# bytedance/particle-sfm

Hardware: AMD Instinct MI355X
Metric: trajectory-points/s (higher is better)
Workload: dtype f32 sampling + f64 positions; 1 GPU; configs[1]: synthetic 100x(1920x1080) flow pairs, sample_ratio=2, flow_check + chaining + occlusion + id assignment, 1 sequence per GPU; frames=101, height=1080, width=1920, trajectories=2073277, parallelism=sequence-per-gpu x1, world_size=1

## Files before the change

include/psfm.h:

```cpp
#ifndef PSFM_H_
#define PSFM_H_

#include <stddef.h>
#include <stdint.h>

#ifdef __cplusplus
extern "C" {
#endif

#define PSFM_VERSION 141

typedef enum psfm_status {
    PSFM_OK = 0,
    PSFM_ERR_ARG = 1,
    PSFM_ERR_HIP = 2,
    PSFM_ERR_CAPACITY = 3,
    PSFM_ERR_SOLVER = 4
} psfm_status;

typedef struct psfm_ctx psfm_ctx;

enum {
    PSFM_TERM_FUNCTION_TOL = 0,
    PSFM_TERM_PARAMETER_TOL = 1,
    PSFM_TERM_GRADIENT_TOL = 2,
    PSFM_TERM_MAX_ITER = 3,
    PSFM_TERM_MIN_RADIUS = 4,
    PSFM_TERM_FAILURE = 5
};

typedef struct psfm_solve_stats {
    int32_t iterations;
    int32_t successful_steps;
    int32_t termination;
    int32_t dogleg_nonGN;
    double initial_cost;
    double final_cost;
} psfm_solve_stats;

typedef struct psfm_track_info {
    int64_t n_traj;
    int64_t n_points;
    int64_t n_lanes_peak;
    int64_t lane_capacity;
    int64_t solver_iterations;
    int32_t n_solves;
    int32_t chain_mode;
} psfm_track_info;

const char* psfm_last_error(void);
int psfm_version(void);

int psfm_device_count(void);

psfm_status psfm_ctx_create(int device, psfm_ctx** out);
psfm_status psfm_ctx_destroy(psfm_ctx* ctx);

psfm_status psfm_ctx_set_capacity(psfm_ctx* ctx, double lane_factor, double traj_factor);

psfm_status psfm_ctx_set_chain_mode(psfm_ctx* ctx, int mode);

psfm_status psfm_ctx_set_motion_boundary(psfm_ctx* ctx, int enable, float thres);

psfm_status psfm_motion_boundary(psfm_ctx* ctx, const float* flows, int n, int h, int w, float thres, uint8_t* mb_out, void* stream);

psfm_status psfm_kill_map(psfm_ctx* ctx, const float* flows, const uint8_t* occ, int n, int h, int w, float thres, uint8_t* kill_out,
                          void* stream);

psfm_status psfm_ctx_set_solver(psfm_ctx* ctx, int mode, int k);
psfm_status psfm_solver_counters(psfm_ctx* ctx, int64_t* fused, int64_t* fused_redone, int64_t* chain, int32_t* k_now);

psfm_status psfm_ctx_set_resident_budget(psfm_ctx* ctx, int blocks);
psfm_status psfm_resident_capacity(psfm_ctx* ctx, int32_t* blocks);

psfm_status psfm_solver_launches(psfm_ctx* ctx, int64_t* resident, int64_t* giveups, int64_t* iterations);

psfm_status psfm_flow_check(psfm_ctx* ctx, const float* flows_f, const float* flows_b, int n_pairs, int h,
                            int w, float thres, uint8_t* occ_out, float* err_out, void* stream);

psfm_status psfm_load_flo_stack(psfm_ctx* ctx, const char* const* paths_host, int n, int h, int w, float* dst, int n_threads, void* stream);

psfm_status psfm_grid_sample(psfm_ctx* ctx, const float* map_hwc, int c, int h, int w, const double* xy,
                             int64_t n, float* out, void* stream);

psfm_status psfm_optimize_location(psfm_ctx* ctx, const double* uv12, const double* ref1, const double* ref2,
                                   const double* scale, const float* flow12, int64_t n, int w, int h,
                                   double* out, psfm_solve_stats* stats_host, void* stream);

psfm_status psfm_path_consistency_eval(psfm_ctx* ctx, const double* uv12, const double* ref1, const double* ref2,
                                       const double* scale, const float* flow12, int64_t n, int w, int h,
                                       double* residuals, double* jacobians, void* stream);

psfm_status psfm_sort_records(psfm_ctx* ctx, uint32_t* keys, int32_t* values, int64_t n, int end_bit, void* stream);

psfm_status psfm_sort_records64(psfm_ctx* ctx, uint64_t* keys, int32_t* values, int64_t n, int end_bit, void* stream);

psfm_status psfm_ctx_get_finalize_forms(psfm_ctx* ctx, int* sort_form, int* offsets_form);

psfm_status psfm_track(psfm_ctx* ctx, const float* flows, const uint8_t* occ, const float* flows_f2,
                       const uint8_t* occ_s2, int n_flows, int h, int w, int sample_ratio,
                       psfm_track_info* info_host, void* stream);

psfm_status psfm_connect(psfm_ctx* ctx, const float* flows_f, const float* flows_b, const float* flows_f2,
                         const float* flows_b2, int n_flows, int h, int w, float thres, int sample_ratio,
                         uint8_t* occ, uint8_t* occ_s2, psfm_track_info* info_host, void* stream);

psfm_status psfm_track_queries(psfm_ctx* ctx, const float* flows_f, const uint8_t* occ_f, const float* flows_b, const uint8_t* occ_b,
                               int n_flows, int h, int w, const double* q_xy, const int32_t* q_t, int64_t n_q,
                               psfm_track_info* info_host, void* stream);

psfm_status psfm_track_queries_optimize(psfm_ctx* ctx, const float* flows_f, const uint8_t* occ_f, const float* flows_f2,
                                        const uint8_t* occ_f2, const float* flows_b, const uint8_t* occ_b, const float* flows_b2,
                                        const uint8_t* occ_b2, int n_flows, int h, int w, const double* q_xy, const int32_t* q_t,
                                        int64_t n_q, psfm_track_info* info_host, void* stream);

psfm_status psfm_connect_batch(psfm_ctx* const* ctxs, int n_seq, const float* const* flows_f, const float* const* flows_b,
                               const float* const* flows_f2, const float* const* flows_b2, const int* n_flows, int h, int w,
                               float thres, int sample_ratio, psfm_track_info* infos_host, void* stream);

psfm_status psfm_result_device(psfm_ctx* ctx, const int32_t** birth, const int32_t** len,
                               const int64_t** off, const double** xy);

psfm_status psfm_result_copy(psfm_ctx* ctx, int32_t* birth_host, int32_t* len_host, int64_t* off_host,
                             double* xy_host, void* stream);

psfm_status psfm_result_solve_stats(psfm_ctx* ctx, psfm_solve_stats* stats_host, int32_t max_n,
                                    int32_t* n_out);

psfm_status psfm_result_filter(psfm_ctx* ctx, int traj_min_len, int64_t* n_traj_host, int64_t* n_points_host, void* stream);
psfm_status psfm_result_filtered_copy(psfm_ctx* ctx, int32_t* ids_host, int32_t* birth_host, int32_t* len_host,
                                      int64_t* off_host, double* xy_host, void* stream);

psfm_status psfm_window_sample(psfm_ctx* ctx, int frame0, int n_frames, int traj_min_len, int min_length,
                               int64_t max_num_tracks, uint64_t seed, int raw_h, int raw_w, int in_h, int in_w,
                               int64_t capacity, int32_t* ids_out, double* xy_raw, double* xy_norm, double* mask_absent,
                               int64_t* k_host, void* stream);

psfm_status psfm_traj_augment(psfm_ctx* ctx, const double* xy_norm, const double* mask_absent, const float* depth, int64_t k,
                              int n_frames, int h, int w, const float* kinv_host, float* out, void* stream);

int psfm_traj_encode_weight_count(void);
psfm_status psfm_traj_encode(psfm_ctx* ctx, const float* features, const double* mask_absent, const float* weights, int64_t k,
                             int n_frames, float* out, void* stream);

int psfm_traj_decode_weight_count(void);
size_t psfm_traj_decode_workspace_bytes(int64_t k);
psfm_status psfm_traj_decode(psfm_ctx* ctx, const float* encoding, const float* weights, int64_t k, void* workspace,
                             size_t workspace_bytes, float* logits, float* prob, uint8_t* pred, void* stream);

psfm_status psfm_traj_to_matches(psfm_ctx* ctx, int n_img, int sample_k, const uint8_t* labels_dev, int64_t* n_kp_host,
                                 int64_t* n_matches_host, int64_t* n_pairs_host, void* stream);
psfm_status psfm_matches_copy(psfm_ctx* ctx, int64_t* kp_off_host, double* kp_xy_host, int64_t* pair_key_host,
                              int64_t* pair_off_host, int64_t* pair_first_host, int32_t* rows_host, void* stream);

psfm_status psfm_labels_set(psfm_ctx* ctx, int64_t n_traj, int64_t n_points, const int32_t* ids, const int64_t* off,
                            const int32_t* frame_ids, const double* xy, const uint8_t* labels, void* stream);
psfm_status psfm_labels_begin(psfm_ctx* ctx, void* stream);
psfm_status psfm_labels_merge_window(psfm_ctx* ctx, int frame0, int n_frames, const int32_t* ids_dev, const uint8_t* pred_dev,
                                     int64_t k, void* stream);
psfm_status psfm_labels_finish(psfm_ctx* ctx, int64_t* n_traj_host, int64_t* n_points_host, void* stream);
psfm_status psfm_labels_device(psfm_ctx* ctx, const int32_t** ids, const int64_t** off, const int32_t** frame_ids, const double** xy,
                               const uint8_t** labels);
psfm_status psfm_labels_copy(psfm_ctx* ctx, int32_t* ids_out, int64_t* off_out, int32_t* frame_ids_out, double* xy_out,
                             uint8_t* labels_out, void* stream);
psfm_status psfm_labels_to_matches(psfm_ctx* ctx, int n_img, int sample_k, int remove_dynamic, int64_t* n_kp_host,
                                   int64_t* n_matches_host, int64_t* n_pairs_host, void* stream);

psfm_status psfm_matches_to_database(psfm_ctx* ctx, int n_img, const int32_t* db_id_host, const int32_t* db_pos_host,
                                     int64_t* n_pairs_kept_host, int64_t* n_rows_kept_host, void* stream);
psfm_status psfm_database_copy(psfm_ctx* ctx, float* kp_f32, int64_t* pair_id, int64_t* pair_key, int64_t* pair_off, uint32_t* rows,
                               void* stream);
int psfm_database_chunk_rows(void);
psfm_status psfm_database_compact_again(psfm_ctx* ctx, void* stream);

psfm_status psfm_sparse_depth(psfm_ctx* ctx, const double* obs_xy, const int64_t* obs_id, int64_t n_obs, const void* img_desc_host,
                              int n_img, const int64_t* pt_id_sorted, const int32_t* pt_row, const double* pt_xyz, int64_t n_pts,
                              double* depth_out, int64_t* missing_id_host, void* stream);
psfm_status psfm_sparse_depth_sort_ids(psfm_ctx* ctx, const int64_t* pt_id, int64_t n_pts, int64_t* pt_id_sorted, int32_t* pt_row,
                                       void* stream);
psfm_status psfm_ctx_set_sparse_depth(psfm_ctx* ctx, int64_t budget_bytes, int timing);
psfm_status psfm_ctx_get_sparse_depth_budget(psfm_ctx* ctx, int64_t* budget_bytes);
psfm_status psfm_sparse_depth_last_ms(psfm_ctx* ctx, double* ms3);
psfm_status psfm_colmap_points3d_count(const void* buf, uint64_t nbytes, uint64_t* n);
psfm_status psfm_colmap_points3d_scan(const void* buf, uint64_t nbytes, uint64_t* ids_out, double* xyz_out, double* err_out,
                                      uint64_t* track_len_out);

psfm_status psfm_depth_display(psfm_ctx* ctx, const double* depth, const void* img_desc_host, int n_img, double pc,
                               const uint8_t* table_host, const uint8_t* bad_rgba_host, uint8_t* rgba_out, int64_t* n_valid_out,
                               double* z_out, void* stream);
psfm_status psfm_ctx_set_depth_display(psfm_ctx* ctx, int timing);
psfm_status psfm_depth_display_last_ms(psfm_ctx* ctx, double* ms4);
int psfm_depth_display_chunk(void);

psfm_status psfm_traj_eval_counts(psfm_ctx* ctx, const int32_t* frame_ids, const double* xy, const uint8_t* labels, int64_t n_points,
                                  const uint8_t* masks_u8, const float* table_host, int n_frames, int h, int w, int64_t* counts_out,
                                  void* stream);
psfm_status psfm_traj_vote_labels(psfm_ctx* ctx, const double* xy, const double* mask_absent, const uint8_t* gts_u8, int64_t k,
                                  int n_frames, int h, int w, uint8_t* labels_out, void* stream);

psfm_status psfm_shard_begin(psfm_ctx* ctx, int n_flows, int h, int w, int sample_ratio, int64_t g0, int64_t g1, int optimize,
                             uint8_t* maps, int64_t map_pitch, void* stream);
psfm_status psfm_shard_step(psfm_ctx* ctx, const float* flow, const uint8_t* occ, int frame, void* stream);
psfm_status psfm_shard_solve_export(psfm_ctx* ctx, const float* flow01, const float* flow12, const float* flow02,
                                    const uint8_t* occ02, int frame, int kind, int k, double* sums_out, void* stream);
psfm_status psfm_shard_frame(psfm_ctx* ctx, const float* flow01, const float* flow12, const float* flow02, const uint8_t* occ,
                             const uint8_t* occ02, int frame, int k, double* sums_out, void* stream);
psfm_status psfm_shard_solve_control(psfm_ctx* ctx, int frame, int kind, int k, const double* totals, int32_t* done_host,
                                     int32_t* redo_host, psfm_solve_stats* stats_host, void* stream);
psfm_status psfm_shard_solve_control_async(psfm_ctx* ctx, int frame, int k, const double* totals, void* stream);
psfm_status psfm_shard_window_state(psfm_ctx* ctx, int f_lo, int f_hi, psfm_solve_stats* stats_host, int32_t* stalled_frame,
                                    void* stream);
psfm_status psfm_shard_solve_control_chain_async(psfm_ctx* ctx, int frame, int kind, const double* totals, void* stream);
psfm_status psfm_shard_solve_poll(psfm_ctx* ctx, int32_t* done_host, psfm_solve_stats* stats_host, void* stream);
psfm_status psfm_shard_solve_local(psfm_ctx* ctx, const float* flow01, const float* flow12, const float* flow02, const uint8_t* occ02,
                                   int frame, int unroll, void* stream);
psfm_status psfm_shard_solve_redo_local(psfm_ctx* ctx, const float* flow01, const float* flow12, const float* flow02,
                                        const uint8_t* occ02, int frame, int chain_stalled, psfm_solve_stats* stats_host, void* stream);
psfm_status psfm_shard_peer_area(psfm_ctx* ctx, void** area_dev, void* ipc_handle_64, void* stream);
psfm_status psfm_shard_peer_open(psfm_ctx* ctx, const void* ipc_handle_64, int peer_rank, void** mapped);
psfm_status psfm_shard_peer_epoch(psfm_ctx* ctx, uint32_t* last_epoch, int reset, void* stream);
psfm_status psfm_shard_peer_connect(psfm_ctx* ctx, int world, int rank, void* const* areas, const int32_t* n_blocks);
psfm_status psfm_shard_solve_blocks(psfm_ctx* ctx, int32_t* n_blocks);
psfm_status psfm_shard_solve_peer(psfm_ctx* ctx, const float* flow01, const float* flow12, const float* flow02, const uint8_t* occ02,
                                  int frame, uint32_t epoch, void* stream);

psfm_status psfm_shard_peek_stall(psfm_ctx* ctx, int32_t* stalled_frame);
psfm_status psfm_shard_solve_restore(psfm_ctx* ctx, int frame, void* stream);
psfm_status psfm_shard_solve_writeback(psfm_ctx* ctx, int frame, const psfm_solve_stats* stats, void* stream);
psfm_status psfm_shard_solve_record(psfm_ctx* ctx, const psfm_solve_stats* stats);
psfm_status psfm_shard_finish(psfm_ctx* ctx, psfm_track_info* info_host, void* stream);
psfm_status psfm_result_keys(psfm_ctx* ctx, int sample_ratio, int w, int64_t* keys_dev, void* stream);

psfm_status psfm_ctx_set_profiling(psfm_ctx* ctx, int enable);
psfm_status psfm_profile_get(psfm_ctx* ctx, int kind, double* total_ms, int64_t* launches);

#ifdef __cplusplus
}
#endif
#endif
```

particle-sfm_amd/build.py:

```python
import os
import subprocess
import sys
from concurrent.futures import ThreadPoolExecutor

HERE = os.path.dirname(os.path.abspath(__file__))
CSRC = os.path.join(HERE, "csrc")
OBJ = os.path.join(HERE, "build")
LIBDIR = os.path.join(HERE, "lib")
LIB = os.path.join(LIBDIR, "libpsfm_hip.so")
SOURCES = ["psfm_api.hip", "psfm_track.hip", "psfm_persist.hip", "psfm_finalize.hip", "psfm_sort.hip", "psfm_sort64.hip", "psfm_solver.hip", "psfm_solver_fused.hip", "psfm_solver_batch.hip", "psfm_window.hip", "psfm_matches.hip", "psfm_shard.hip", "psfm_batch.hip", "psfm_ingest.hip", "psfm_labels.hip", "psfm_augment.hip", "psfm_encoder.hip", "psfm_decoder.hip", "psfm_ground_truth.hip", "psfm_database.hip", "psfm_sparse_depth.hip", "psfm_motion_boundary.hip", "psfm_depth_display.hip", "psfm_query.hip", "psfm_query_pc.hip"]
HIPCC = os.environ.get("HIPCC", "/opt/rocm/bin/hipcc")
FLAGS = ["--offload-arch=gfx950", "-O3", "-std=c++17", "-fPIC", "-ffp-contract=off", "-fno-fast-math",
         "-Wall", "-Wno-unused-function", "-Wno-unused-result",
         "-mllvm", "-amdgpu-atomic-optimizer-strategy=None"]


def source_hash():
    import hashlib
    h = hashlib.sha256()
    files = sorted(os.path.join(CSRC, f) for f in os.listdir(CSRC) if f.endswith((".hip", ".h")))
    files.append(os.path.join(os.path.dirname(HERE), "include", "psfm.h"))
    for f in files:
        h.update(os.path.basename(f).encode())
        h.update(open(f, "rb").read())
    h.update(" ".join(FLAGS).encode())
    return h.hexdigest()[:16]


def _newer(target, deps):
    if not os.path.exists(target):
        return True
    t = os.path.getmtime(target)
    return any(os.path.getmtime(d) > t for d in deps)


def build(force=False, verbose=False):
    extra = os.environ.get("PSFM_EXTRA_FLAGS", "").split()
    if extra:
        FLAGS.extend(extra)
        force = True
    os.makedirs(OBJ, exist_ok=True)
    os.makedirs(LIBDIR, exist_ok=True)
    headers = [os.path.join(CSRC, f) for f in os.listdir(CSRC) if f.endswith(".h")]
    headers.append(os.path.join(os.path.dirname(HERE), "include", "psfm.h"))
    jobs, objs = [], []
    for src in SOURCES:
        s = os.path.join(CSRC, src)
        o = os.path.join(OBJ, src.replace(".hip", ".o"))
        objs.append(o)
        if force or _newer(o, [s] + headers):
            jobs.append([HIPCC] + FLAGS + ["-c", s, "-o", o])

    def run(cmd):
        if verbose:
            print(" ".join(cmd), flush=True)
        r = subprocess.run(cmd, stdout=subprocess.PIPE, stderr=subprocess.STDOUT, text=True)
        if r.returncode != 0:
            raise RuntimeError("hipcc failed:\n%s\n%s" % (" ".join(cmd), r.stdout))
        if verbose and r.stdout.strip():
            print(r.stdout)

    with ThreadPoolExecutor(max_workers=4) as ex:
        list(ex.map(run, jobs))
    if force or jobs or _newer(LIB, objs):
        run([HIPCC, "--offload-arch=gfx950", "-shared", "-fPIC", "-o", LIB] + objs)
    return LIB


if __name__ == "__main__":
    if "--source-hash" in sys.argv:
        print(source_hash())
    else:
        print(build(force="--force" in sys.argv, verbose=True))
```

particle-sfm_amd/csrc/psfm_api.hip:

```cpp
#include <stdarg.h>
#include <stdio.h>
#include <string.h>
#include <mutex>
#include <shared_mutex>
#include <atomic>
#include <chrono>
#include <stdlib.h>

#include "psfm_internal.h"

static thread_local char g_err[512] = "";
static std::shared_mutex g_dev_gate[16];
std::shared_mutex& psfm_device_gate(int device) { return g_dev_gate[device & 15]; }
static std::atomic<int> g_dev_waiters[16];
int psfm_gate_waiters(int device) { return g_dev_waiters[device & 15].load(std::memory_order_relaxed); }
void psfm_gate_waiters_add(int device, int d) { g_dev_waiters[device & 15].fetch_add(d, std::memory_order_relaxed); }
static int psfm_wants_persist(psfm_ctx* c, bool optimize, int h, int w, int ratio, bool fused)
{
    if (c->chain_mode == 1 || ratio < 1 || !psfm_frame_ok(h, w)) return 0;
    if (c->mb_enable && !optimize) return 0;
    if (optimize) return c->resident_budget > 0 ? 0 : 1;
    const int64_t G = (int64_t)((w + ratio - 1) / ratio) * ((h + ratio - 1) / ratio);
    const int64_t P = (int64_t)h * w;
    const int maxb = psfm_persist_max_blocks(c);
    if (maxb <= 0 || (G + 255) / 256 > maxb) return 0;
    if (c->chain_mode == 2) return 2;
    if (ratio < 2 || G < 100000) return 0;
    if (fused && (G < 400000 || P > 6 * G)) return 0;
    return 1;
}

void psfm_set_error(const char* fmt, ...)
{
    va_list ap;
    va_start(ap, fmt);
    vsnprintf(g_err, sizeof(g_err), fmt, ap);
    va_end(ap);
}

extern "C" const char* psfm_last_error(void) { return g_err; }
extern "C" int psfm_version(void) { return PSFM_VERSION; }

extern "C" int psfm_device_count(void)
{
    int n = 0;
    if (hipGetDeviceCount(&n) != hipSuccess) { (void)hipGetLastError(); return 0; }
    return n;
}

psfm_status PsfmBuf::ensure(size_t need)
{
    if (need <= bytes) return PSFM_OK;
    if (p) { (void)hipFree(p); p = nullptr; bytes = 0; }
    size_t want = (need + (size_t)(1 << 20) - 1) & ~((size_t)(1 << 20) - 1);
    hipError_t e = hipMalloc(&p, want);
    if (e != hipSuccess) {
        p = nullptr;
        psfm_set_error("hipMalloc(%zu bytes) failed: %s", want, hipGetErrorString(e));
        return PSFM_ERR_HIP;
    }
    bytes = want;
    return PSFM_OK;
}

void PsfmBuf::release()
{
    if (p) (void)hipFree(p);
    p = nullptr;
    bytes = 0;
}

hipEvent_t PsfmProfiler::get()
{
    if (!pool.empty()) { hipEvent_t e = pool.back(); pool.pop_back(); return e; }
    hipEvent_t e;
    (void)hipEventCreate(&e);
    return e;
}
void PsfmProfiler::begin(int kind, hipStream_t s)
{
    if (!enabled) return;
    Span sp; sp.kind = kind; sp.a = get(); sp.b = get();
    (void)hipEventRecord(sp.a, s);
    spans.push_back(sp);
}
void PsfmProfiler::kernel_span(int kind, hipEvent_t* a, hipEvent_t* b, bool always)
{
    if (!enabled || (!always && (calls++ % stride) != 0)) { *a = nullptr; *b = nullptr; return; }
    Span sp; sp.kind = kind; sp.a = get(); sp.b = get();
    spans.push_back(sp);
    *a = sp.a; *b = sp.b;
}
void PsfmProfiler::end(hipStream_t s)
{
    if (!enabled) return;
    (void)hipEventRecord(spans.back().b, s);
}
void PsfmProfiler::collect()
{
    for (auto& sp : spans) {
        float ms = 0.f;
        if (hipEventElapsedTime(&ms, sp.a, sp.b) == hipSuccess) { total_ms[sp.kind] += ms; launches[sp.kind]++; }
        pool.push_back(sp.a); pool.push_back(sp.b);
    }
    spans.clear();
}
void PsfmProfiler::reset()
{
    for (int k = 0; k < PSFM_PROF_KINDS; ++k) { total_ms[k] = 0; launches[k] = 0; }
}
void PsfmProfiler::destroy()
{
    collect();
    for (auto e : pool) (void)hipEventDestroy(e);
    pool.clear();
}

#define PSFM_CHECK_CTX(c)                                                     \
    do {                                                                      \
        if (!(c)) { psfm_set_error("ctx is NULL"); return PSFM_ERR_ARG; }     \
        PSFM_HIP(hipSetDevice((c)->device));                                  \
    } while (0)

extern "C" psfm_status psfm_ctx_create(int device, psfm_ctx** out)
{
    if (!out) { psfm_set_error("psfm_ctx_create: out is NULL"); return PSFM_ERR_ARG; }
    *out = nullptr;
    int n = 0;
    hipError_t e = hipGetDeviceCount(&n);
    if (e != hipSuccess || n <= 0) {
        (void)hipGetLastError();
        psfm_set_error("no HIP device available (%s); libpsfm_hip has no CPU fallback",
                       e != hipSuccess ? hipGetErrorString(e) : "device count 0");
        return PSFM_ERR_HIP;
    }
    if (device < 0 || device >= n) { psfm_set_error("device %d out of range [0,%d)", device, n); return PSFM_ERR_ARG; }
    PSFM_HIP(hipSetDevice(device));
    psfm_ctx* c = new psfm_ctx();
    c->device = device;
    c->host_pinned_bytes = 512 + sizeof(PsfmShard) * PSFM_NSHARD + 4096;
    e = hipHostMalloc(&c->host_pinned, c->host_pinned_bytes, hipHostMallocDefault);
    if (e != hipSuccess) { delete c; psfm_set_error("hipHostMalloc failed: %s", hipGetErrorString(e)); return PSFM_ERR_HIP; }
    *out = c;
    return PSFM_OK;
}

extern "C" psfm_status psfm_ctx_destroy(psfm_ctx* c)
{
    if (!c) return PSFM_OK;
    (void)hipSetDevice(c->device);
    PsfmBuf* bufs[] = {&c->log, &c->birth_frame, &c->birth_idx, &c->free_stack, &c->fin_keys, &c->fin_lanes,
                       &c->occupied, &c->counters, &c->shards, &c->survivors, &c->sort_keys, &c->sort_lanes, &c->sort_tmp,
                       &c->scan_tmp, &c->fin_marks, &c->res_birth, &c->res_len, &c->res_off, &c->res_xy, &c->sol_x, &c->sol_state,
                       &c->sol_partials, &c->sol_ctrl, &c->sol_misc, &c->sol_stats, &c->sol_fused, &c->sol_bar, &c->sol_list, &c->occ_own, &c->occ2_own,
                       &c->handoff, &c->seg_info, &c->seg_table, &c->persist_bar, &c->batch_tab, &c->batch_ws, &c->batch_fc, &c->win_ws, &c->flt_ids, &c->flt_birth, &c->flt_len, &c->flt_off, &c->flt_xy,
                       &c->mt_kp_off, &c->mt_q, &c->mt_pts, &c->mt_kp_ind, &c->mt_kp_xy, &c->mt_moff, &c->mt_keys, &c->mt_rows, &c->mt_gid, &c->mt_pairs,
                       &c->lb_state, &c->lb_first, &c->lb_flag, &c->lb_ws, &c->lb_ids, &c->lb_off, &c->lb_frames, &c->lb_xy, &c->lb_labels, &c->gt_flag, &c->kill,
                       &c->db_kp, &c->db_pairs, &c->db_rows, &c->db_ws, &c->sd_ws, &c->dd_ws, &c->dd_comp, &c->qr_ws};
    for (auto b : bufs) b->release();
    for (hipEvent_t e : c->sd_events) if (e) (void)hipEventDestroy(e);
    for (hipEvent_t e : c->dd_events) if (e) (void)hipEventDestroy(e);
    for (void*& q : c->peer_opened) { if (q) (void)hipIpcCloseMemHandle(q); q = nullptr; }
    c->peer_area.release();
    psfm_shard_abandon(c);
    c->prof.destroy();
    if (c->side_stream) (void)hipStreamDestroy(c->side_stream);
    if (c->redo_stream) (void)hipStreamDestroy(c->redo_stream);
    if (c->copy_stream) (void)hipStreamDestroy(c->copy_stream);
    if (c->copy_stream2) (void)hipStreamDestroy(c->copy_stream2);
    for (void* p : c->ingest_slots) (void)hipHostFree(p);
    for (hipEvent_t e : c->ingest_events) (void)hipEventDestroy(e);
    if (c->host_pinned) (void)hipHostFree(c->host_pinned);
    if (c->host_seg) (void)hipHostFree(c->host_seg);
    if (c->host_batch) (void)hipHostFree(c->host_batch);
    if (c->host_batch2) (void)hipHostFree(c->host_batch2);
    delete c;
    return PSFM_OK;
}

extern "C" psfm_status psfm_ctx_set_capacity(psfm_ctx* c, double lane_factor, double traj_factor)
{
    if (!c || !(lane_factor >= 1.0) || !(traj_factor >= 1.0)) { psfm_set_error("psfm_ctx_set_capacity: factors must be >= 1"); return PSFM_ERR_ARG; }
    c->lane_factor = lane_factor;
    c->traj_factor = traj_factor;
    return PSFM_OK;
}

extern "C" psfm_status psfm_ctx_set_chain_mode(psfm_ctx* c, int mode)
{
    if (!c || mode < 0 || mode > 2) { psfm_set_error("psfm_ctx_set_chain_mode: mode must be 0 (auto), 1 (per-frame launches) or 2 (persistent loop)"); return PSFM_ERR_ARG; }
    c->chain_mode = mode;
    return PSFM_OK;
}

extern "C" psfm_status psfm_ctx_set_solver(psfm_ctx* c, int mode, int k)
{
    if (!c || mode < 0 || mode > 2 || k < 0 || k > psfm_solve_kmax()) {
        psfm_set_error("psfm_ctx_set_solver: mode must be 0 (adaptive), 1 (launch chain) or 2 (fused solve), k in [0, %d]", psfm_solve_kmax());
        return PSFM_ERR_ARG;
    }
    c->solver_mode = mode;
    c->solver_K = k;
    return PSFM_OK;
}

extern "C" psfm_status psfm_solver_counters(psfm_ctx* c, int64_t* fused, int64_t* fused_redone, int64_t* chain, int32_t* k_now)
{
    if (!c) { psfm_set_error("ctx is NULL"); return PSFM_ERR_ARG; }
    if (fused) *fused = c->n_fused_ok;
    if (fused_redone) *fused_redone = c->n_fused_redone;
    if (chain) *chain = c->n_chain;
    if (k_now) *k_now = c->solve_K;
    return PSFM_OK;
}

extern "C" psfm_status psfm_ctx_set_resident_budget(psfm_ctx* c, int blocks)
{
    if (!c || blocks < 0) { psfm_set_error("psfm_ctx_set_resident_budget: blocks must be >= 0"); return PSFM_ERR_ARG; }
    c->resident_budget = blocks;
    return PSFM_OK;
}

extern "C" psfm_status psfm_resident_capacity(psfm_ctx* c, int32_t* blocks)
{
    PSFM_CHECK_CTX(c);
    if (blocks) *blocks = psfm_resident_blocks(c);
    return PSFM_OK;
}

extern "C" psfm_status psfm_solver_launches(psfm_ctx* c, int64_t* resident, int64_t* giveups, int64_t* iterations)
{
    if (!c) { psfm_set_error("ctx is NULL"); return PSFM_ERR_ARG; }
    if (resident) *resident = c->n_resident;
    if (giveups) *giveups = c->pc_giveups;
    if (iterations) *iterations = c->n_iter_launches;
    return PSFM_OK;
}

extern "C" psfm_status psfm_ctx_set_profiling(psfm_ctx* c, int enable)
{
    if (!c) { psfm_set_error("ctx is NULL"); return PSFM_ERR_ARG; }
    c->prof.enabled = enable != 0;
    c->prof.stride = enable > 1 ? enable : 1;
    c->prof.calls = 0;
    c->prof.collect();
    c->prof.reset();
    return PSFM_OK;
}

extern "C" psfm_status psfm_profile_get(psfm_ctx* c, int kind, double* total_ms, int64_t* launches)
{
    if (!c || kind < 0 || kind >= PSFM_PROF_KINDS) { psfm_set_error("psfm_profile_get: bad argument"); return PSFM_ERR_ARG; }
    if (total_ms) *total_ms = c->prof.total_ms[kind];
    if (launches) *launches = c->prof.launches[kind];
    return PSFM_OK;
}

extern "C" psfm_status psfm_flow_check(psfm_ctx* c, const float* flows_f, const float* flows_b, int n_pairs, int h, int w,
                                       float thres, uint8_t* occ_out, float* err_out, void* stream)
{
    PSFM_CHECK_CTX(c);
    PsfmGate gate(c->device, 0);
    if (n_pairs < 0 || !psfm_frame_ok(h, w) || (n_pairs > 0 && (!flows_f || !flows_b || !occ_out))) {
        psfm_set_error("psfm_flow_check: bad argument (n_pairs=%d h=%d w=%d)", n_pairs, h, w);
        return PSFM_ERR_ARG;
    }
    hipStream_t s = (hipStream_t)stream;
    c->prof.begin(PSFM_PROF_FLOW_CHECK, s);
    psfm_status st = psfm_launch_flow_check(flows_f, flows_b, n_pairs, h, w, thres, occ_out, err_out, s);
    c->prof.end(s);
    return st;
}

extern "C" psfm_status psfm_grid_sample(psfm_ctx* c, const float* map_hwc, int ch, int h, int w, const double* xy,
                                        int64_t n, float* out, void* stream)
{
    PSFM_CHECK_CTX(c);
    PsfmGate gate(c->device, 0);
    if ((ch != 1 && ch != 2) || !psfm_frame_ok(h, w) || n < 0 || (n > 0 && (!map_hwc || !xy || !out))) {
        psfm_set_error("psfm_grid_sample: bad argument (c=%d h=%d w=%d n=%lld)", ch, h, w, (long long)n);
        return PSFM_ERR_ARG;
    }
    return psfm_launch_grid_sample(map_hwc, ch, h, w, xy, n, out, (hipStream_t)stream);
}

extern "C" psfm_status psfm_optimize_location(psfm_ctx* c, const double* uv12, const double* ref1, const double* ref2,
                                              const double* scale, const float* flow12, int64_t n, int w, int h,
                                              double* out, psfm_solve_stats* stats_host, void* stream)
{
    PSFM_CHECK_CTX(c);
    PsfmGate gate(c->device, (c->chain_mode == 1 || c->resident_budget > 0) ? 0 : 1);
    c->pc_persist_ok = gate.exclusive || c->resident_budget > 0;
    c->pc_giveups = 0;
    c->n_resident = c->n_iter_launches = 0;
    if (n < 0 || !psfm_frame_ok(h, w) || (n > 0 && (!uv12 || !ref1 || !ref2 || !scale || !flow12 || !out))) {
        psfm_set_error("psfm_optimize_location: bad argument (n=%lld h=%d w=%d)", (long long)n, h, w);
        return PSFM_ERR_ARG;
    }
    psfm_solve_stats st;
    memset(&st, 0, sizeof(st));
    hipStream_t s = (hipStream_t)stream;
    c->prof.begin(PSFM_PROF_SOLVER, s);
    psfm_status rc = psfm_solve_batch(c, uv12, ref1, ref2, scale, flow12, n, w, h, out, &st, s);
    c->prof.end(s);
    if (stats_host) *stats_host = st;
    return rc;
}

extern "C" psfm_status psfm_path_consistency_eval(psfm_ctx* c, const double* uv12, const double* ref1, const double* ref2,
                                                  const double* scale, const float* flow12, int64_t n, int w, int h,
                                                  double* residuals, double* jacobians, void* stream)
{
    PSFM_CHECK_CTX(c);
    PsfmGate gate(c->device, 0);
    if (n < 0 || n > 0x3fffffff || !psfm_frame_ok(h, w) || (n > 0 && (!uv12 || !ref1 || !ref2 || !scale || !flow12 || (!residuals && !jacobians)))) {
        psfm_set_error("psfm_path_consistency_eval: bad argument (n=%lld h=%d w=%d)", (long long)n, h, w);
        return PSFM_ERR_ARG;
    }
    return psfm_launch_pc_eval(uv12, ref1, ref2, scale, flow12, n, w, h, residuals, jacobians, (hipStream_t)stream);
}

extern "C" psfm_status psfm_sort_records(psfm_ctx* c, uint32_t* keys, int32_t* values, int64_t n, int end_bit, void* stream)
{
    PSFM_CHECK_CTX(c);
    PsfmGate gate(c->device, 0);
    if (n < 0 || n >= (1ll << 31) || end_bit < 1 || end_bit > 32 || (n > 0 && (!keys || !values))) {
        psfm_set_error("psfm_sort_records: bad argument (n=%lld end_bit=%d)", (long long)n, end_bit);
        return PSFM_ERR_ARG;
    }
    if (n == 0) return PSFM_OK;
    hipStream_t s = (hipStream_t)stream;
    psfm_status st;
    if ((st = c->sort_keys.ensure(sizeof(unsigned long long) * (size_t)n * 2)) != PSFM_OK) return st;
    if ((st = c->sort_lanes.ensure(sizeof(int) * (size_t)n * 2)) != PSFM_OK) return st;
    const int64_t half = psfm_sort_pairs32_passes((unsigned)end_bit) % 2 == 0 ? 0 : n;
    unsigned* k0 = c->sort_keys.as<unsigned>();
    int* v0 = c->sort_lanes.as<int>();
    PSFM_HIP(hipMemcpyAsync(k0 + half, keys, sizeof(unsigned) * (size_t)n, hipMemcpyDeviceToDevice, s));
    PSFM_HIP(hipMemcpyAsync(v0 + half, values, sizeof(int) * (size_t)n, hipMemcpyDeviceToDevice, s));
    if ((st = psfm_sort_pairs32(c, k0, v0, k0 + n, v0 + n, n, (unsigned)end_bit, s)) != PSFM_OK) return st;
    PSFM_HIP(hipMemcpyAsync(keys, k0, sizeof(unsigned) * (size_t)n, hipMemcpyDeviceToDevice, s));
    PSFM_HIP(hipMemcpyAsync(values, v0, sizeof(int) * (size_t)n, hipMemcpyDeviceToDevice, s));
    return PSFM_OK;
}

extern "C" psfm_status psfm_sort_records64(psfm_ctx* c, uint64_t* keys, int32_t* values, int64_t n, int end_bit, void* stream)
{
    PSFM_CHECK_CTX(c);
    PsfmGate gate(c->device, 0);
    if (n < 0 || n >= (1ll << 31) || end_bit < 1 || end_bit > 64 || (n > 0 && (!keys || !values))) {
        psfm_set_error("psfm_sort_records64: bad argument (n=%lld end_bit=%d)", (long long)n, end_bit);
        return PSFM_ERR_ARG;
    }
    if (n == 0) return PSFM_OK;
    hipStream_t s = (hipStream_t)stream;
    psfm_status st;
    if ((st = c->sort_keys.ensure(sizeof(unsigned long long) * (size_t)n * 2)) != PSFM_OK) return st;
    if ((st = c->sort_lanes.ensure(sizeof(int) * (size_t)n * 2)) != PSFM_OK) return st;
    const int64_t half = psfm_sort_pairs64_passes((unsigned)end_bit) % 2 == 0 ? 0 : n;
    unsigned long long* k0 = c->sort_keys.as<unsigned long long>();
    int* v0 = c->sort_lanes.as<int>();
    PSFM_HIP(hipMemcpyAsync(k0 + half, keys, sizeof(unsigned long long) * (size_t)n, hipMemcpyDeviceToDevice, s));
    PSFM_HIP(hipMemcpyAsync(v0 + half, values, sizeof(int) * (size_t)n, hipMemcpyDeviceToDevice, s));
    if ((st = psfm_sort_pairs64(c, k0, v0, k0 + n, v0 + n, n, (unsigned)end_bit, s)) != PSFM_OK) return st;
    PSFM_HIP(hipMemcpyAsync(keys, k0, sizeof(unsigned long long) * (size_t)n, hipMemcpyDeviceToDevice, s));
    PSFM_HIP(hipMemcpyAsync(values, v0, sizeof(int) * (size_t)n, hipMemcpyDeviceToDevice, s));
    return PSFM_OK;
}

extern "C" psfm_status psfm_ctx_get_finalize_forms(psfm_ctx* c, int* sort_form, int* offsets_form)
{
    PSFM_CHECK_CTX(c);
    if (sort_form) *sort_form = c->fin_sort_form;
    if (offsets_form) *offsets_form = c->fin_offsets_form;
    return PSFM_OK;
}

psfm_status psfm_track_dims(psfm_ctx* c, int n_flows, int h, int w, int ratio, int64_t g_own, PsfmTrackDims& d)
{
    d.H = h; d.W = w; d.ratio = ratio; d.n_flows = n_flows;
    d.GW = (w + ratio - 1) / ratio; d.GH = (h + ratio - 1) / ratio;
    d.G = (int64_t)d.GW * d.GH;
    const int64_t Gown = g_own < 0 ? d.G : (g_own > 0 ? g_own : 1);
    d.cap = (int64_t)(c->lane_factor * (double)Gown);
    d.cap = ((d.cap + 255) / 256) * 256;
    const int64_t n_blocks = d.cap / 256;
    {
        const int64_t gb = (Gown + 255) / 256;
        d.nsh = (int)(gb < PSFM_NSHARD ? (gb > 0 ? gb : 1) : PSFM_NSHARD);
    }
    d.free_cap = (int)(((n_blocks + d.nsh - 1) / d.nsh) * 256) + 1024;
    const double tf = c->traj_factor > (double)n_flows / 8.0 ? c->traj_factor : (double)n_flows / 8.0;
    d.shard_cap = (int)(((int64_t)(tf * (double)Gown) + d.cap) / d.nsh) + 1024;
    d.traj_cap = (int64_t)d.shard_cap * PSFM_NSHARD;
    if (d.cap > 0x7fffffff / 2 || d.traj_cap > 0x7fffffff / 2) { psfm_set_error("psfm_track: grid too large"); return PSFM_ERR_ARG; }
    d.shift_b = 1; while ((1ll << d.shift_b) < d.G) ++d.shift_b;
    int tbits = 1; while ((1ll << tbits) < (long long)n_flows + 2) ++tbits;
    d.shift_d = d.shift_b + tbits;
    if (d.shift_d + tbits > 63) { psfm_set_error("psfm_track: key does not fit 64 bits"); return PSFM_ERR_ARG; }
    d.cw = (float)((double)(w - 1) / 2.0); d.ch = (float)((double)(h - 1) / 2.0);
    return PSFM_OK;
}

psfm_status psfm_track_alloc(psfm_ctx* c, const PsfmTrackDims& d)
{
    psfm_status st;
    const int n_flows = d.n_flows;
    if ((st = c->log.ensure(sizeof(double2) * (size_t)(n_flows + 1) * d.cap)) != PSFM_OK) return st;
    if ((st = c->birth_frame.ensure(sizeof(int) * d.cap)) != PSFM_OK) return st;
    if ((st = c->birth_idx.ensure(sizeof(int) * d.cap)) != PSFM_OK) return st;
    if ((st = c->free_stack.ensure(sizeof(int) * (size_t)d.free_cap * PSFM_NSHARD * 2)) != PSFM_OK) return st;
    if ((st = c->shards.ensure(sizeof(PsfmShard) * PSFM_NSHARD * 2)) != PSFM_OK) return st;
    if ((st = c->fin_keys.ensure(sizeof(unsigned long long) * d.traj_cap)) != PSFM_OK) return st;
    if ((st = c->fin_lanes.ensure(sizeof(int) * d.traj_cap)) != PSFM_OK) return st;
    if ((st = c->occupied.ensure((size_t)d.G * 3 + 8)) != PSFM_OK) return st;
    if ((st = c->counters.ensure(sizeof(PsfmCounters))) != PSFM_OK) return st;
    if ((st = c->survivors.ensure(sizeof(int) * (size_t)(n_flows + 1))) != PSFM_OK) return st;
    return PSFM_OK;
}

struct PsfmOccPipeline {
    int chunk = 0;
    std::vector<hipEvent_t> ready;
    std::vector<hipEvent_t> ready_s2;
    int waited = -1, waited_s2 = -1;
    psfm_status need(int pair, bool s2, hipStream_t s)
    {
        if (chunk <= 0) return PSFM_OK;
        std::vector<hipEvent_t>& ev = s2 ? ready_s2 : ready;
        int& w = s2 ? waited_s2 : waited;
        const int cidx = pair / chunk;
        while (w < cidx && w + 1 < (int)ev.size()) {
            ++w;
            PSFM_HIP(hipStreamWaitEvent(s, ev[w], 0));
        }
        return PSFM_OK;
    }
};

static psfm_status psfm_track_impl(psfm_ctx* c, const float* flows, const uint8_t* occ, const float* flows_f2,
                                   const uint8_t* occ_s2, int n_flows, int h, int w, int ratio, psfm_track_info* info,
                                   void* stream, PsfmOccPipeline* pipe, PsfmGate& gate,
                                   const float* fuse_flows_b = nullptr, float fuse_thres = 0.f, int64_t occ_pitch = 0)
{
    const bool device_is_ours = gate.exclusive;
    if (occ_pitch == 0) occ_pitch = (int64_t)h * w;
    PSFM_CHECK_CTX(c);
    psfm_shard_abandon(c);
    const bool optimize = flows_f2 != nullptr;
    if (n_flows < 1 || !psfm_frame_ok(h, w) || ratio < 1 || !flows || !occ || (optimize && !occ_s2 && n_flows > 1)) {
        psfm_set_error("psfm_track: bad argument (n_flows=%d h=%d w=%d ratio=%d)", n_flows, h, w, ratio);
        return PSFM_ERR_ARG;
    }
    if (ratio > 64) { psfm_set_error("psfm_track: sample_ratio %d > 64 unsupported", ratio); return PSFM_ERR_ARG; }
    hipStream_t s = (hipStream_t)stream;
    PsfmTrackDims d;
    psfm_status st;
    if ((st = psfm_track_dims(c, n_flows, h, w, ratio, -1, d)) != PSFM_OK) return st;
    const int64_t P = (int64_t)h * w;
    if ((st = psfm_track_alloc(c, d)) != PSFM_OK) return st;

    c->solve_stats.clear();
    c->res_n_traj = c->res_n_points = 0;
    c->res_n_flows = n_flows;
    c->res_is_query = false;
    c->pc_persist_ok = device_is_ours || c->resident_budget > 0;
    c->pc_giveups = 0;

    const bool mb = c->mb_enable;
    if (!optimize && c->chain_mode != 1 && !mb) {
        const int maxb = psfm_persist_max_blocks(c);
        const int64_t need_blocks = (d.G + 255) / 256;
        if (maxb > 0 && need_blocks <= maxb && device_is_ours) {
            PsfmTrackDims dp = d;
            int64_t nb = need_blocks <= 256 ? 2 * need_blocks + 4 : need_blocks + need_blocks / 4;
            dp.nblk = (int)(nb < maxb ? nb : maxb);
            if (fuse_flows_b) {
                const int64_t fc_blocks = (P + 1023) / 1024;
                const int64_t want = fc_blocks < maxb ? fc_blocks : maxb;
                if (want > dp.nblk) dp.nblk = (int)want;
            }
            dp.cap = (int64_t)dp.nblk * (256 + psfm_persist_guests());
            dp.nsh = dp.nblk < PSFM_NSHARD ? dp.nblk : PSFM_NSHARD;
            dp.free_cap = (int)(((dp.nblk + dp.nsh - 1) / dp.nsh) * 256) + 1024;
            dp.seg_cap = (int)(d.traj_cap / dp.nblk) + 64;
            dp.spill_cap = (int)(d.traj_cap / 8) + 4096;
            const int64_t fin_total = (int64_t)dp.nblk * dp.seg_cap + dp.spill_cap;
            if ((st = c->log.ensure(sizeof(double2) * (size_t)(n_flows + 1) * dp.cap)) != PSFM_OK) return st;
            if ((st = c->free_stack.ensure(sizeof(int) * (size_t)dp.free_cap * PSFM_NSHARD * 2)) != PSFM_OK) return st;
            if ((st = c->fin_keys.ensure(sizeof(unsigned long long) * fin_total)) != PSFM_OK) return st;
            if ((st = c->fin_lanes.ensure(sizeof(int) * fin_total)) != PSFM_OK) return st;
            if ((st = c->handoff.ensure((size_t)dp.nblk * 256 * 24)) != PSFM_OK) return st;
            if ((st = c->seg_info.ensure(sizeof(int) * 2 * (size_t)dp.nblk)) != PSFM_OK) return st;
            if ((st = c->persist_bar.ensure((size_t)(4 * PSFM_NSHARD + 1) * 128)) != PSFM_OK) return st;
            if (pipe && (st = pipe->need(n_flows - 1, false, s)) != PSFM_OK) return st;
            bool fallback = false;
            {
                const bool trace = getenv("PSFM_TRACE") != nullptr;
                const auto t1 = std::chrono::steady_clock::now();
                st = psfm_launch_chain_persist(c, dp, flows, occ, occ_pitch, fuse_flows_b, fuse_thres, s);
                if (st == PSFM_ERR_CAPACITY) {
                    fallback = true;
                    st = PSFM_OK;
                } else {
                    if (st != PSFM_OK) return st;
                    c->prof.begin(PSFM_PROF_FINALIZE, s);
                    st = psfm_finalize_persist(c, dp, &fallback, s);
                    c->prof.end(s);
                }
                if (trace) {
                    const auto t2 = std::chrono::steady_clock::now();
                    fprintf(stderr, "[psfm %p] persistent loop: launch+finalize %.2f ms, fallback %d, overflow %d\n", (void*)c,
                            std::chrono::duration<double, std::milli>(t2 - t1).count(), (int)fallback,
                            ((PsfmCounters*)c->host_pinned)->overflow);
                }
            }
            if (st != PSFM_OK) return st;
            if (!fallback) {
                PSFM_HIP(hipStreamSynchronize(s));
                c->prof.collect();
                if (info) {
                    memset(info, 0, sizeof(*info));
                    info->n_traj = c->res_n_traj;
                    info->n_points = c->res_n_points;
                    info->n_lanes_peak = ((PsfmCounters*)c->host_pinned)->n_lanes;
                    info->lane_capacity = dp.cap;
                    info->chain_mode = 2;
                }
                return PSFM_OK;
            }
            c->prof.collect();
        }
    }
    if (fuse_flows_b) {
        c->prof.begin(PSFM_PROF_FLOW_CHECK, s);
        for (int f = 0; f < n_flows; ++f)
            if ((st = psfm_launch_flow_check(flows + (size_t)f * P * 2, fuse_flows_b + (size_t)f * P * 2, 1, h, w, fuse_thres,
                                             const_cast<uint8_t*>(occ) + (size_t)f * occ_pitch, nullptr, s)) != PSFM_OK) return st;
        c->prof.end(s);
    }
    if (mb) {
        if ((st = c->kill.ensure((size_t)n_flows * (size_t)P)) != PSFM_OK) return st;
        if (pipe && (st = pipe->need(n_flows - 1, false, s)) != PSFM_OK) return st;
        if (occ_pitch != P) { psfm_set_error("psfm_track: motion boundary needs densely packed occlusion maps"); return PSFM_ERR_ARG; }
        if ((st = psfm_launch_motion_boundary(flows, occ, n_flows, h, w, c->mb_thres, c->kill.as<uint8_t>(), s)) != PSFM_OK) return st;
    }
    if ((st = psfm_launch_track_init(c, d, s)) != PSFM_OK) return st;
    int64_t total_iters = 0;
    static const int check_env = getenv("PSFM_CHECK_FRAMES") ? atoi(getenv("PSFM_CHECK_FRAMES")) : 0;
    const int PSFM_CHECK = check_env >= 2 ? check_env : 16;
    std::vector<psfm_solve_stats> hstats((size_t)n_flows + 1);
    int first_unchecked = 1;
    if (optimize) {
        if ((st = c->sol_stats.ensure(sizeof(psfm_solve_stats) * (size_t)(n_flows + 1))) != PSFM_OK) return st;
    }
    const char* unroll_env = getenv("PSFM_SOLVE_UNROLL");
    const int unroll_fixed = unroll_env ? (atoi(unroll_env) < 1 ? 1 : atoi(unroll_env)) : 0;
    c->n_fused_ok = c->n_fused_redone = c->n_chain = 0;
    c->n_resident = c->n_iter_launches = 0;
    if (optimize && (st = psfm_solve_prepare(c, d, s)) != PSFM_OK) return st;
    static const bool merge = !(getenv("PSFM_MERGE_FRAME") && atoi(getenv("PSFM_MERGE_FRAME")) == 0);
    const bool seq_env = !(getenv("PSFM_SEQ") && atoi(getenv("PSFM_SEQ")) == 0);
    bool seq_ok = optimize && merge && seq_env && unroll_fixed == 0 && !mb;
    int launch_id = 0;
    int idle_windows = 0;
    bool pc_in_step = true;
    int* hpc = (int*)((char*)c->host_pinned + 320);
    PsfmCounters* dctr = c->counters.as<PsfmCounters>();

    auto checkpoint = [&](int f_hi, bool fused_now, bool seq, int* f_next) -> psfm_status {
        PsfmCounters* hc = (PsfmCounters*)c->host_pinned;
        PSFM_HIP(hipMemcpyAsync(hc, c->counters.p, sizeof(PsfmCounters), hipMemcpyDeviceToHost, s));
        PSFM_HIP(hipMemcpyAsync(hstats.data() + first_unchecked, c->sol_stats.as<psfm_solve_stats>() + first_unchecked,
                                sizeof(psfm_solve_stats) * (size_t)(f_hi - first_unchecked + 1), hipMemcpyDeviceToHost, s));
        PSFM_HIP(hipStreamSynchronize(s));
        if (gate.yield_exclusive()) c->pc_persist_ok = c->resident_budget > 0;
        if ((hc->overflow & 7) != 0 || hc->n_lanes > d.cap) {
            psfm_set_error("capacity exceeded: lanes used %d of %lld, overflow bits %d (frame %d of %d); raise psfm_ctx_set_capacity",
                           hc->n_lanes, (long long)d.cap, hc->overflow, hc->pc_frame, n_flows);
            return PSFM_ERR_CAPACITY;
        }
        const int stalled = hc->stall ? hc->stall - 1 : -1;
        int last_ok = f_hi;
        if (seq) {
            const int pcf = hc->pc_frame < n_flows ? hc->pc_frame : n_flows;
            last_ok = pcf - 1;
        }
        if (stalled >= 0) {
            const int fs = stalled;
            psfm_solve_stats ss;
            memset(&ss, 0, sizeof(ss));
            const int k_used = c->solver_K > 0 ? c->solver_K : c->solve_K;
            psfm_status st2 = psfm_solve_frame_resume(c, d, flows + (size_t)(fs - 1) * P * 2, flows + (size_t)fs * P * 2,
                                                      flows_f2 + (size_t)(fs - 1) * P * 2, occ_s2 + (size_t)(fs - 1) * P, fs, &ss,
                                                      (fused_now && !seq && c->solver_K == 0 && k_used < psfm_solve_kmax())
                                                          ? (k_used + 2 < psfm_solve_kmax() ? k_used + 2 : psfm_solve_kmax()) : 0,
                                                      !fused_now, s);
            if (st2 != PSFM_OK) return st2;
            hstats[fs] = ss;
            last_ok = fs;
            pc_in_step = false;
        }
        int max_it = 0, n_solved = 0, n_unclean = 0, k_need = 2;
        for (int k = first_unchecked; k <= last_ok; ++k) {
            if (hstats[k].termination >= 0) {
                c->solve_stats.push_back(hstats[k]);
                total_iters += hstats[k].iterations;
                const psfm_solve_stats& q = hstats[k];
                const bool clean = q.dogleg_nonGN == 0 && q.termination != PSFM_TERM_FAILURE &&
                                   (q.iterations == q.successful_steps + 1 ||
                                    (q.termination == PSFM_TERM_GRADIENT_TOL && q.iterations == q.successful_steps)) &&
                                   q.successful_steps + 1 <= psfm_solve_kmax();
                ++n_solved;
                if (!clean) ++n_unclean;
                else if (q.successful_steps + 1 > k_need) k_need = q.successful_steps + 1;
                if (!fused_now) ++c->n_chain;
                else if (k == stalled) ++c->n_fused_redone;
                else ++c->n_fused_ok;
            }
            if (hstats[k].iterations > max_it) max_it = hstats[k].iterations;
        }
        if (n_solved > 0) {
            c->solve_mode = (n_unclean * 8 > n_solved) ? 1 : 0;
            if (seq) {
                int hist[16] = {0};
                for (int k = first_unchecked; k <= last_ok; ++k)
                    if (hstats[k].termination >= 0) ++hist[hstats[k].successful_steps + 1 < 15 ? hstats[k].successful_steps + 1 : 15];
                int best = 2;
                for (int q = 2; q <= psfm_solve_kmax(); ++q) if (hist[q] > hist[best]) best = q;
                c->solve_K = best;
            } else {
                c->solve_K = k_need > c->solve_K ? k_need : c->solve_K - (c->solve_K - k_need + 1) / 2;
            }
        }
        int want = max_it + 1;
        want = want < 4 ? 4 : (want > 64 ? 64 : want);
        c->solve_unroll = want > c->solve_unroll ? want : c->solve_unroll - (c->solve_unroll - want + 1) / 2;
        first_unchecked = last_ok + 1;
        *f_next = last_ok + 1;
        return PSFM_OK;
    };

    int f = 0;
    while (f < n_flows) {
        const bool fused_now = c->solver_mode == 2 || (c->solver_mode == 0 && c->solve_mode == 0);
        if (seq_ok && fused_now && f >= 1) {
            const int k_now = c->solver_K > 0 ? c->solver_K : c->solve_K;
// ... 215 lines not shown
```

particle-sfm_amd/csrc/psfm_finalize.hip:

```cpp
#include <cstring>
#include <stdio.h>
#include <rocprim/device/device_radix_sort.hpp>
#include <rocprim/device/device_scan.hpp>

#include "psfm_device.h"
#include "psfm_finalize_plan.h"
#include "psfm_internal.h"

#define PSFM_BLOCK 256

__device__ __forceinline__ void psfm_collect_alive_body(
    const int* __restrict__ birth_frame, const int* __restrict__ birth_idx, PsfmCounters* __restrict__ ctr,
    PsfmShard* __restrict__ shards, unsigned long long* __restrict__ fin_keys, int* __restrict__ fin_lanes, int cap,
    int shard_cap, int last_time, int shift_b, int shift_d)
{
    __shared__ int s_cnt[PSFM_BLOCK / PSFM_WAVE];
    __shared__ int s_base;
    const int n_lanes = min(ctr->n_lanes, cap);
    if ((int)(blockIdx.x * PSFM_BLOCK) >= n_lanes) return;
    const int i = blockIdx.x * PSFM_BLOCK + threadIdx.x;
    int bf = -1;
    if (i < n_lanes) bf = birth_frame[i];
    const bool pending = bf <= -2;
    const bool alive = (bf >= 0) | pending;
    const int my_last = pending ? last_time - 1 : last_time;
    if (pending) bf = -2 - bf;
    const unsigned long long am = __ballot(alive);
    const int lane = psfm_lane_id(), wave = threadIdx.x / PSFM_WAVE;
    if (lane == 0) s_cnt[wave] = __popcll(am);
    __syncthreads();
    const int shard = blockIdx.x % PSFM_NSHARD;
    if (threadIdx.x == 0) {
        int tot = 0;
        for (int w = 0; w < PSFM_BLOCK / PSFM_WAVE; ++w) tot += s_cnt[w];
        s_base = tot > 0 ? atomicAdd(&shards[shard].fin_cnt, tot) : 0;
    }
    __syncthreads();
    if (alive) {
        int r = s_base + psfm_rank_in(am);
        for (int w = 0; w < wave; ++w) r += s_cnt[w];
        if (r < shard_cap) {
            const int64_t o = (int64_t)shard * shard_cap + r;
            fin_keys[o] = ((unsigned long long)my_last << shift_d) | ((unsigned long long)bf << shift_b) |
                          (unsigned long long)birth_idx[i];
            fin_lanes[o] = i;
        } else {
            atomicOr(&ctr->overflow, 2);
        }
    }
}

__global__ __launch_bounds__(PSFM_BLOCK) void psfm_collect_alive_kernel(
    const int* __restrict__ birth_frame, const int* __restrict__ birth_idx, PsfmCounters* __restrict__ ctr,
    PsfmShard* __restrict__ shards, unsigned long long* __restrict__ fin_keys, int* __restrict__ fin_lanes, int cap,
    int shard_cap, int last_time, int shift_b, int shift_d)
{
    psfm_collect_alive_body(birth_frame, birth_idx, ctr, shards, fin_keys, fin_lanes, cap, shard_cap, last_time, shift_b, shift_d);
}

__global__ __launch_bounds__(PSFM_BLOCK) void psfm_compact_shards_kernel(
    const unsigned long long* __restrict__ fin_keys, const int* __restrict__ fin_lanes, int shard_cap,
    PsfmShardOffsets so, unsigned long long* __restrict__ keys, int* __restrict__ lanes, PsfmKeyFmt fmt)
{
    const int shard = blockIdx.y;
    const int n = so.count[shard];
    for (int i = blockIdx.x * PSFM_BLOCK + threadIdx.x; i < n; i += gridDim.x * PSFM_BLOCK) {
        psfm_put_key(keys, so.start[shard] + i, fin_keys[(int64_t)shard * shard_cap + i], fmt);
        lanes[so.start[shard] + i] = fin_lanes[(int64_t)shard * shard_cap + i];
    }
}

__global__ __launch_bounds__(PSFM_BLOCK) void psfm_decode_kernel(const void* __restrict__ keys, int64_t n, PsfmKeyFmt fmt,
                                                                 int* __restrict__ birth, int* __restrict__ len, int64_t* __restrict__ len64)
{
    const int64_t i = (int64_t)blockIdx.x * PSFM_BLOCK + threadIdx.x;
    if (i > n) return;
    if (i == n) { len64[i] = 0; return; }
    int last, b, idx;
    psfm_key_fields(keys, i, fmt.use32, fmt.shift_b, fmt.shift_d, &last, &b, &idx);
    birth[i] = b;
    len[i] = last - b + 1;
    len64[i] = (int64_t)(last - b + 1);
}

#define PSFM_PLAN_BLOCK 1024
struct PsfmPlan {
    const int* gstart; const int64_t* goff;
    const void* keys; int use32, shift_b, shift_d;
    int* birth_w; int* len_w; int64_t* off_w;
};

__global__ __launch_bounds__(PSFM_BLOCK) void psfm_group_bounds_kernel(const void* __restrict__ keys, int64_t n, int use32, int shift_b,
                                                                       int shift_d, int* __restrict__ gstart)
{
    const int64_t i = (int64_t)blockIdx.x * PSFM_BLOCK + threadIdx.x;
    if (i >= n) return;
    const int g = psfm_key_group(keys, i, use32, shift_b, shift_d);
    const int gp = i > 0 ? psfm_key_group(keys, i - 1, use32, shift_b, shift_d) : -1;
    if (g != gp) gstart[g] = (int)i;
}

__global__ __launch_bounds__(PSFM_PLAN_BLOCK) void psfm_group_plan_kernel(int* __restrict__ marks, int* __restrict__ gstart,
                                                                          int64_t* __restrict__ goff, int ng, int64_t n,
                                                                          int64_t* __restrict__ off_n)
{
    __shared__ int s_g[PSFM_PLAN_MAX_GROUPS];
    __shared__ int s_wmin[PSFM_PLAN_BLOCK / PSFM_WAVE];
    __shared__ long long s_wsum[PSFM_PLAN_BLOCK / PSFM_WAVE];
    constexpr int NW = PSFM_PLAN_BLOCK / PSFM_WAVE;
    constexpr int INF = 0x7fffffff;
    const int tid = threadIdx.x, lane = tid & (PSFM_WAVE - 1), wave = tid / PSFM_WAVE;
    for (int k = tid; k < ng; k += PSFM_PLAN_BLOCK) {
        const int v = marks[k];
        s_g[k] = v;
        gstart[k] = v;
        if (v >= 0) marks[k] = -1;
    }
    __syncthreads();
    const int per = (ng + PSFM_PLAN_BLOCK - 1) / PSFM_PLAN_BLOCK;
    const int g0 = min(tid * per, ng), g1 = min(g0 + per, ng);
    int first = INF;
    for (int g = g1 - 1; g >= g0; --g) if (s_g[g] >= 0) first = s_g[g];
    int sm = first;
#pragma unroll
    for (int o = 1; o < PSFM_WAVE; o <<= 1) {
        const int v = __shfl_down(sm, o);
        if (lane + o < PSFM_WAVE && v < sm) sm = v;
    }
    if (lane == 0) s_wmin[wave] = sm;
    int nxt = __shfl_down(sm, 1);
    if (lane == PSFM_WAVE - 1) nxt = INF;
    __syncthreads();
    for (int w = wave + 1; w < NW; ++w) nxt = min(nxt, s_wmin[w]);
    if (nxt == INF) nxt = (int)n;
    int last = 0, birth = 0;
    if (g0 < g1) psfm_tri_invert((unsigned)g0, &last, &birth);
    for (int g = g1 - 1; g >= g0; --g) {
        const int st = s_g[g];
        if (st >= 0) { s_g[g] = nxt - st; nxt = st; } else s_g[g] = 0;
    }
    long long pts = 0;
    {
        int l = last, b = birth;
        for (int g = g0; g < g1; ++g) {
            pts += (long long)s_g[g] * (long long)(l - b + 1);
            if (++b > l) { ++l; b = 0; }
        }
    }
    long long inc = pts;
#pragma unroll
    for (int o = 1; o < PSFM_WAVE; o <<= 1) {
        const long long v = __shfl_up(inc, o);
        if (lane >= o) inc += v;
    }
    if (lane == PSFM_WAVE - 1) s_wsum[wave] = inc;
    __syncthreads();
    long long base = 0, total = 0;
    for (int w = 0; w < NW; ++w) { const long long v = s_wsum[w]; if (w < wave) base += v; total += v; }
    long long run = base + inc - pts;
    {
// ... 71 lines not shown
    const int64_t col = s_lane[j];
    const int bj = s_birth[j];
    double2 r[NLD];
#pragma unroll
    for (int u = 0; u < NLD; ++u) {
        const int t = q + u * (PSFM_BLOCK / TILE_J);
        r[u] = t < lj ? log[(int64_t)(bj + t) * cap + col] : make_double2(0.0, 0.0);
    }
    if (tid < TILE_J) s_off[tid] = id0 + tid < n ? psfm_track_offset(pl, off, id0 + tid, hb, hl) : 0;
    for (int k0 = 0; k0 < maxlen; k0 += TILE_K) {
#pragma unroll
        for (int u = 0; u < NLD; ++u) tile[j][q + u * (PSFM_BLOCK / TILE_J)] = r[u];
        __syncthreads();
        if (k0 + TILE_K < maxlen) {
#pragma unroll
            for (int u = 0; u < NLD; ++u) {
                const int t = k0 + TILE_K + q + u * (PSFM_BLOCK / TILE_J);
                r[u] = t < lj ? log[(int64_t)(bj + t) * cap + col] : make_double2(0.0, 0.0);
            }
        }
        const int kk = tid & (TILE_K - 1);
        for (int jj = tid / TILE_K; jj < TILE_J; jj += PSFM_BLOCK / TILE_K) {
            const int t = k0 + kk;
            if (t < s_len[jj]) out[s_off[jj] + t] = tile[jj][kk];
        }
        __syncthreads();
    }
}

__global__ __launch_bounds__(PSFM_BLOCK) void psfm_gather_kernel(const double2* __restrict__ log, int64_t cap,
                                                                 const int* __restrict__ lanes,
                                                                 const int* __restrict__ birth,
                                                                 const int* __restrict__ len,
                                                                 const int64_t* __restrict__ off, int64_t n,
                                                                 double2* __restrict__ out, PsfmPlan pl)
{
    psfm_gather_body(log, cap, lanes, birth, len, off, n, out, pl);
}

__global__ __launch_bounds__(PSFM_BLOCK) void psfm_gather_delta_kernel(const float2* __restrict__ dlog, int64_t cap,
                                                                       const int* __restrict__ lanes,
                                                                       const int* __restrict__ birth,
                                                                       const int* __restrict__ len,
                                                                       const int64_t* __restrict__ off, int64_t n,
                                                                       const void* __restrict__ keys, int use32, int shift_b,
                                                                       int GW, int ratio, double2* __restrict__ out, PsfmPlan pl)
{
    __shared__ float2 dtile[TILE_J][TILE_K + 1];
    __shared__ double2 tile[TILE_J][TILE_K + 1];
    __shared__ double2 s_pos[TILE_J];
    __shared__ int s_lane[TILE_J], s_birth[TILE_J], s_len[TILE_J];
    __shared__ int64_t s_off[TILE_J];
    __shared__ int s_maxlen;
    const int tid = threadIdx.x;
    const int64_t id0 = (int64_t)blockIdx.x * TILE_J;
    int hb = 0, hl = 0;
    if (tid == 0) s_maxlen = 0;
    __syncthreads();
    if (tid < TILE_J) {
        const int64_t id = id0 + tid;
        const bool ok = id < n;
        int b = 0, l = 0, idx = -1;
        const int my_lane = ok ? lanes[id] : 0;
        if (ok) psfm_track_header(pl, birth, len, id, &b, &l, &idx);
        hb = b; hl = l;
        s_lane[tid] = my_lane;
        s_birth[tid] = b;
        s_len[tid] = l;
        if (ok) {
            atomicMax(&s_maxlen, l);
            if (idx < 0) idx = psfm_key_idx(psfm_key_at(keys, id, use32), shift_b);
            const int gy = idx / GW, gx = idx - gy * GW;
            s_pos[tid] = make_double2((double)(gx * ratio), (double)(gy * ratio));
        }
    }
    __syncthreads();
    const int maxlen = s_maxlen;
    const int j = tid & (TILE_J - 1);
    const int q = tid / TILE_J;
    constexpr int NLD = TILE_K * TILE_J / PSFM_BLOCK;
    const int lj = s_len[j];
    const int64_t col = s_lane[j];
    const int bj = s_birth[j];
    float2 r[NLD];
#pragma unroll
    for (int u = 0; u < NLD; ++u) {
        const int t = q + u * (PSFM_BLOCK / TILE_J);
        r[u] = (t >= 1 && t < lj) ? dlog[(int64_t)(bj + t - 1) * cap + col] : make_float2(0.f, 0.f);
    }
    if (tid < TILE_J) s_off[tid] = id0 + tid < n ? psfm_track_offset(pl, off, id0 + tid, hb, hl) : 0;
    for (int k0 = 0; k0 < maxlen; k0 += TILE_K) {
#pragma unroll
        for (int u = 0; u < NLD; ++u) dtile[j][q + u * (PSFM_BLOCK / TILE_J)] = r[u];
        __syncthreads();
        if (k0 + TILE_K < maxlen) {
#pragma unroll
            for (int u = 0; u < NLD; ++u) {
                const int t = k0 + TILE_K + q + u * (PSFM_BLOCK / TILE_J);
                r[u] = (t < lj) ? dlog[(int64_t)(bj + t - 1) * cap + col] : make_float2(0.f, 0.f);
            }
        }
        if (tid < TILE_J) {
            double2 pos = s_pos[tid];
            const int l = s_len[tid];
            float2 f[TILE_K];
#pragma unroll
            for (int k = 0; k < TILE_K; ++k) f[k] = dtile[tid][k];
#pragma unroll
            for (int k = 0; k < TILE_K; ++k) {
                const int t = k0 + k;
                if (t >= 1 && t < l) { pos.x = pos.x + (double)f[k].x; pos.y = pos.y + (double)f[k].y; }
                tile[tid][k] = pos;
            }
            s_pos[tid] = pos;
        }
        __syncthreads();
        const int kk = tid & (TILE_K - 1);
        for (int jj = tid / TILE_K; jj < TILE_J; jj += PSFM_BLOCK / TILE_K) {
            const int t = k0 + kk;
            if (t < s_len[jj]) out[s_off[jj] + t] = tile[jj][kk];
        }
        __syncthreads();
    }
}

static PsfmFinForm psfm_form_of(const PsfmTrackDims& d, int64_t n, int n_seq = 0)
{
    static const int sort_on = getenv("PSFM_FIN_SORT") ? atoi(getenv("PSFM_FIN_SORT")) : 1;
    static const int plan_on = getenv("PSFM_FIN_PLAN") ? atoi(getenv("PSFM_FIN_PLAN")) : 1;
    return psfm_fin_form(d.shift_b, d.shift_d, d.n_flows, n_seq > 0 ? n_seq : 1, n, sort_on, plan_on, n_seq > 0 ? 0 : 1);
}

struct PsfmFinDst { unsigned long long* keys; int* lanes; };
static PsfmFinDst psfm_compact_dst(psfm_ctx* c, const PsfmFinForm& f, int64_t n)
{
    const int64_t half = f.first_half ? 0 : n;
    return {f.fmt.use32 ? (unsigned long long*)(c->sort_keys.as<unsigned>() + half) : c->sort_keys.as<unsigned long long>() + half,
            c->sort_lanes.as<int>() + half};
}

template <class K>
static psfm_status psfm_rocprim_sort(psfm_ctx* c, int64_t n, unsigned end_bit, size_t scan_bytes, hipStream_t s)
{
    K* k_out = c->sort_keys.as<K>(), *k_in = k_out + n;
    int* l_out = c->sort_lanes.as<int>(), *l_in = l_out + n;
    size_t tmp_bytes = 0;
    psfm_status st;
    PSFM_HIP(rocprim::radix_sort_pairs(nullptr, tmp_bytes, k_in, k_out, l_in, l_out, (size_t)n, 0u, end_bit, s));
    if ((st = c->sort_tmp.ensure(tmp_bytes > scan_bytes ? tmp_bytes : scan_bytes)) != PSFM_OK) return st;
    PSFM_HIP(rocprim::radix_sort_pairs(c->sort_tmp.p, tmp_bytes, k_in, k_out, l_in, l_out, (size_t)n, 0u, end_bit, s));
    return PSFM_OK;
}

static psfm_status psfm_sort_records(psfm_ctx* c, const PsfmFinForm& f, int64_t n, size_t* scan_bytes, hipStream_t s)
{
    psfm_status st;
    PSFM_HIP(rocprim::exclusive_scan(nullptr, *scan_bytes, (int64_t*)nullptr, (int64_t*)nullptr, (int64_t)0,
                                     (size_t)(n + 1), rocprim::plus<int64_t>(), s));
    c->fin_sort_form = 0; c->fin_offsets_form = 0;
    if (f.sort_form == 3) {
        st = f.fmt.use32 ? psfm_rocprim_sort<unsigned>(c, n, f.end_bit, *scan_bytes, s) : psfm_rocprim_sort<unsigned long long>(c, n, f.end_bit, *scan_bytes, s);
    } else {
        int* l_out = c->sort_lanes.as<int>();
        if ((st = c->sort_tmp.ensure(*scan_bytes)) != PSFM_OK) return st;
        if (f.fmt.use32) st = psfm_sort_pairs32(c, c->sort_keys.as<unsigned>(), l_out, c->sort_keys.as<unsigned>() + n, l_out + n, n, f.end_bit, s);
        else st = psfm_sort_pairs64(c, c->sort_keys.as<unsigned long long>(), l_out, c->sort_keys.as<unsigned long long>() + n, l_out + n, n, f.end_bit, s);
    }
    if (st != PSFM_OK) return st;
    c->fin_sort_form = f.sort_form;
    return PSFM_OK;
}

static psfm_status psfm_host_seg_ensure(psfm_ctx* c, size_t need, size_t slack)
{
    if (c->host_seg_bytes >= need) return PSFM_OK;
    if (c->host_seg) (void)hipHostFree(c->host_seg);
    c->host_seg = nullptr; c->host_seg_bytes = 0;
    PSFM_HIP(hipHostMalloc(&c->host_seg, need + slack, hipHostMallocDefault));
    c->host_seg_bytes = need + slack;
    return PSFM_OK;
}

static psfm_status psfm_finalize_sorted(psfm_ctx* c, const PsfmTrackDims& d, const PsfmFinForm& f, int64_t n, int64_t npts, bool delta_log,
                                        hipStream_t s)
{
    psfm_status st;
    size_t scan_bytes = 0;
    if ((st = psfm_sort_records(c, f, n, &scan_bytes, s)) != PSFM_OK) return st;
    if ((st = c->res_birth.ensure(sizeof(int) * n)) != PSFM_OK) return st;
    if ((st = c->res_len.ensure(sizeof(int) * n)) != PSFM_OK) return st;
    if ((st = c->res_off.ensure(sizeof(int64_t) * (n + 1))) != PSFM_OK) return st;
    const long long ng = f.ng;
    const PsfmKeyFmt fmt = f.fmt;
    PsfmPlan pl;
    pl.gstart = nullptr; pl.goff = nullptr; pl.keys = (const void*)c->sort_keys.p; pl.use32 = fmt.use32; pl.shift_b = d.shift_b; pl.shift_d = d.shift_d;
    pl.birth_w = c->res_birth.as<int>(); pl.len_w = c->res_len.as<int>(); pl.off_w = c->res_off.as<int64_t>();
    if (f.offsets_form == 1) {
        if ((st = c->scan_tmp.ensure((sizeof(int64_t) + sizeof(int)) * (size_t)ng)) != PSFM_OK) return st;
        int64_t* goff = c->scan_tmp.as<int64_t>();
        int* gstart = (int*)(goff + ng);
        const void* had = c->fin_marks.p;
        if ((st = c->fin_marks.ensure(sizeof(int) * (size_t)PSFM_PLAN_MAX_GROUPS)) != PSFM_OK) return st;
        if (!c->fin_marks_clean || had != c->fin_marks.p)
            PSFM_HIP(hipMemsetAsync(c->fin_marks.p, 0xff, sizeof(int) * (size_t)PSFM_PLAN_MAX_GROUPS, s));
        c->fin_marks_clean = false;
        hipLaunchKernelGGL(psfm_group_bounds_kernel, dim3((unsigned)((n + PSFM_BLOCK - 1) / PSFM_BLOCK)), dim3(PSFM_BLOCK), 0, s,
                           (const void*)c->sort_keys.p, n, fmt.use32, d.shift_b, d.shift_d, c->fin_marks.as<int>());
        hipLaunchKernelGGL(psfm_group_plan_kernel, dim3(1), dim3(PSFM_PLAN_BLOCK), 0, s, c->fin_marks.as<int>(), gstart, goff, (int)ng, n,
                           c->res_off.as<int64_t>() + n);
        PSFM_HIP(hipGetLastError());
        c->fin_marks_clean = true;
        c->fin_offsets_form = 1;
        pl.gstart = gstart; pl.goff = goff;
    } else {
        c->fin_offsets_form = 3;
        if ((st = c->scan_tmp.ensure(sizeof(int64_t) * (n + 1))) != PSFM_OK) return st;
        hipLaunchKernelGGL(psfm_decode_kernel, dim3((unsigned)((n + 1 + PSFM_BLOCK - 1) / PSFM_BLOCK)), dim3(PSFM_BLOCK), 0, s,
                           (const void*)c->sort_keys.p, n, fmt, c->res_birth.as<int>(), c->res_len.as<int>(), c->scan_tmp.as<int64_t>());
        PSFM_HIP(hipGetLastError());
        PSFM_HIP(rocprim::exclusive_scan(c->sort_tmp.p, scan_bytes, c->scan_tmp.as<int64_t>(), c->res_off.as<int64_t>(),
                                         (int64_t)0, (size_t)(n + 1), rocprim::plus<int64_t>(), s));
    }
    c->res_n_points = npts;
    if ((st = c->res_xy.ensure(sizeof(double2) * (size_t)(npts > 0 ? npts : 1))) != PSFM_OK) return st;
    if (delta_log)
        hipLaunchKernelGGL(psfm_gather_delta_kernel, dim3((unsigned)((n + TILE_J - 1) / TILE_J)), dim3(PSFM_BLOCK), 0, s,
                           c->log.as<float2>(), d.cap, c->sort_lanes.as<int>(), c->res_birth.as<int>(),
                           c->res_len.as<int>(), c->res_off.as<int64_t>(), n, (const void*)c->sort_keys.p, fmt.use32,
                           d.shift_b, d.GW, d.ratio, c->res_xy.as<double2>(), pl);
    else
        hipLaunchKernelGGL(psfm_gather_kernel, dim3((unsigned)((n + TILE_J - 1) / TILE_J)), dim3(PSFM_BLOCK), 0, s,
                           c->log.as<double2>(), d.cap, c->sort_lanes.as<int>(), c->res_birth.as<int>(),
                           c->res_len.as<int>(), c->res_off.as<int64_t>(), n, c->res_xy.as<double2>(), pl);
    PSFM_HIP(hipGetLastError());
    return PSFM_OK;
}

psfm_status psfm_finalize(psfm_ctx* c, const PsfmTrackDims& d, hipStream_t s)
{
    PsfmCounters* ctr = c->counters.as<PsfmCounters>();
    PsfmShard* shards = c->shards.as<PsfmShard>();
    hipLaunchKernelGGL(psfm_collect_alive_kernel, dim3((unsigned)((d.cap + PSFM_BLOCK - 1) / PSFM_BLOCK)), dim3(PSFM_BLOCK),
                       0, s, c->birth_frame.as<int>(), c->birth_idx.as<int>(), ctr, shards,
                       c->fin_keys.as<unsigned long long>(), c->fin_lanes.as<int>(), (int)d.cap, d.shard_cap,
                       d.n_flows, d.shift_b, d.shift_d);
    PSFM_HIP(hipGetLastError());
    PsfmCounters* hc = (PsfmCounters*)c->host_pinned;
    PsfmShard* hs = psfm_host_shards(c);
    PSFM_HIP(hipMemcpyAsync(hc, ctr, sizeof(PsfmCounters), hipMemcpyDeviceToHost, s));
    PSFM_HIP(hipMemcpyAsync(hs, shards, sizeof(PsfmShard) * PSFM_NSHARD, hipMemcpyDeviceToHost, s));
    PSFM_HIP(hipStreamSynchronize(s));
    PsfmShardOffsets so;
    int fin_cnt[PSFM_NSHARD];
    int64_t n = 0, npts = 0;
    for (int k = 0; k < PSFM_NSHARD; ++k) { npts += hs[k].points; fin_cnt[k] = hs[k].fin_cnt; }
    const bool over = psfm_shard_offsets(fin_cnt, d.shard_cap, &so, &n) || hc->overflow != 0;
    if (over || hc->n_lanes > d.cap) {
        psfm_set_error("capacity exceeded: lanes used %d of %lld, trajectory records %lld of %lld (%d shards); "
                       "raise psfm_ctx_set_capacity", hc->n_lanes, (long long)d.cap, (long long)n,
                       (long long)d.traj_cap, PSFM_NSHARD);
        return PSFM_ERR_CAPACITY;
    }
    c->res_n_traj = n;
    c->res_n_points = 0;
    if (n == 0) return PSFM_OK;
    psfm_status st;
    if ((st = c->sort_keys.ensure(sizeof(unsigned long long) * n * 2)) != PSFM_OK) return st;
    if ((st = c->sort_lanes.ensure(sizeof(int) * n * 2)) != PSFM_OK) return st;
    const PsfmFinForm f = psfm_form_of(d, n);
    const PsfmFinDst dst = psfm_compact_dst(c, f, n);
    hipLaunchKernelGGL(psfm_compact_shards_kernel, dim3(64, PSFM_NSHARD), dim3(PSFM_BLOCK), 0, s,
                       c->fin_keys.as<unsigned long long>(), c->fin_lanes.as<int>(), d.shard_cap, so, dst.keys, dst.lanes, f.fmt);
    PSFM_HIP(hipGetLastError());
    return psfm_finalize_sorted(c, d, f, n, npts, false, s);
}

__global__ __launch_bounds__(PSFM_BLOCK) void psfm_compact_segments_kernel(
    const unsigned long long* __restrict__ fin_keys, const int* __restrict__ fin_lanes, const int2* __restrict__ seg_info, int nblk,
    int seg_cap, const PsfmCounters* __restrict__ ctr, int spill_cap, unsigned long long* __restrict__ keys, int* __restrict__ lanes,
    PsfmKeyFmt fmt)
{
    __shared__ long long s_part[PSFM_BLOCK / PSFM_WAVE];
    const int b = blockIdx.x, tid = threadIdx.x;
    long long mine = 0;
    for (int k = tid; k < b; k += PSFM_BLOCK) mine += seg_info[k].x;
#pragma unroll
    for (int o = 32; o > 0; o >>= 1) mine += __shfl_down(mine, o);
    if ((tid & (PSFM_WAVE - 1)) == 0) s_part[tid / PSFM_WAVE] = mine;
    __syncthreads();
    long long dst = 0;
    for (int w = 0; w < PSFM_BLOCK / PSFM_WAVE; ++w) dst += s_part[w];
    const int count = b < nblk ? seg_info[b].x : min(ctr->spill_cnt, spill_cap);
    const long long src = (long long)b * seg_cap;
    for (int i0 = 0; i0 < count; i0 += 4 * PSFM_BLOCK) {
        unsigned long long k[4];
        int l[4];
#pragma unroll
        for (int u = 0; u < 4; ++u) {
            const int i = i0 + u * PSFM_BLOCK + tid;
            k[u] = i < count ? fin_keys[src + i] : 0ull;
            l[u] = i < count ? fin_lanes[src + i] : 0;
        }
#pragma unroll
        for (int u = 0; u < 4; ++u) {
            const int i = i0 + u * PSFM_BLOCK + tid;
            if (i < count) {
                psfm_put_key(keys, dst + i, k[u], fmt);
                lanes[dst + i] = l[u];
            }
        }
    }
}

psfm_status psfm_finalize_persist(psfm_ctx* c, const PsfmTrackDims& d, bool* fallback, hipStream_t s)
{
    *fallback = false;
    const int nseg = d.nblk + 1;
    psfm_status st;
    if ((st = psfm_host_seg_ensure(c, sizeof(int2) * (size_t)d.nblk, 0)) != PSFM_OK) return st;
    int2* hinfo = (int2*)c->host_seg;
    PsfmCounters* hc = (PsfmCounters*)c->host_pinned;
    PSFM_HIP(hipMemcpyAsync(hc, c->counters.p, sizeof(PsfmCounters), hipMemcpyDeviceToHost, s));
    PSFM_HIP(hipMemcpyAsync(hinfo, c->seg_info.p, sizeof(int2) * (size_t)d.nblk, hipMemcpyDeviceToHost, s));
    PSFM_HIP(hipStreamSynchronize(s));
    if (hc->pad[0]) fprintf(stderr, "psfm persist check: site %d index %d\n", hc->pad[0], hc->pad[1]);
    if (hc->overflow & (4 | 8)) {
        *fallback = true;
        return PSFM_OK;
    }
    int64_t n = 0, npts = 0;
    for (int b = 0; b < d.nblk; ++b) {
        n += hinfo[b].x;
        npts += hinfo[b].y;
    }
    const int spilled = hc->spill_cnt < d.spill_cap ? hc->spill_cnt : d.spill_cap;
    n += spilled;
    if (hc->overflow != 0) {
        psfm_set_error("capacity exceeded (persistent loop): overflow bits %d, trajectory records %lld (%d spilled of %d); "
                       "raise psfm_ctx_set_capacity", hc->overflow, (long long)n, hc->spill_cnt, d.spill_cap);
        return PSFM_ERR_CAPACITY;
    }
    c->res_n_traj = n;
    c->res_n_points = 0;
    if (n == 0) return PSFM_OK;
    if ((st = c->sort_keys.ensure(sizeof(unsigned long long) * n * 2)) != PSFM_OK) return st;
    if ((st = c->sort_lanes.ensure(sizeof(int) * n * 2)) != PSFM_OK) return st;
    const PsfmFinForm f = psfm_form_of(d, n);
    const PsfmFinDst dst = psfm_compact_dst(c, f, n);
    hipLaunchKernelGGL(psfm_compact_segments_kernel, dim3((unsigned)nseg), dim3(PSFM_BLOCK), 0, s,
                       c->fin_keys.as<unsigned long long>(), c->fin_lanes.as<int>(), (const int2*)c->seg_info.as<int2>(), d.nblk, d.seg_cap,
                       (const PsfmCounters*)c->counters.as<PsfmCounters>(), d.spill_cap, dst.keys, dst.lanes, f.fmt);
    PSFM_HIP(hipGetLastError());
    return psfm_finalize_sorted(c, d, f, n, npts, true, s);
}

struct PsfmFinSeq {
    const int* birth_frame; const int* birth_idx; PsfmCounters* ctr; PsfmShard* shards;
    unsigned long long* fin_keys; int* fin_lanes;
    const double2* log; int64_t cap;
    int shard_cap, last_time;
    int64_t rec_start, n;
    int* res_birth; int* res_len; int64_t* res_off; double2* res_xy;
};

__global__ __launch_bounds__(PSFM_BLOCK) void psfm_collect_alive_batch_kernel(const PsfmFinSeq* __restrict__ T, int shift_b, int shift_d)
{
    const PsfmFinSeq& q = T[blockIdx.y];
    psfm_collect_alive_body(q.birth_frame, q.birth_idx, q.ctr, q.shards, q.fin_keys, q.fin_lanes, (int)q.cap, q.shard_cap, q.last_time,
                            shift_b, shift_d);
}

__global__ __launch_bounds__(PSFM_WAVE) void psfm_batch_counts_kernel(const PsfmFinSeq* __restrict__ T, long long* __restrict__ counts)
{
    const PsfmFinSeq& q = T[blockIdx.x];
    const int k = threadIdx.x;
    static_assert(PSFM_NSHARD == PSFM_WAVE, "one lane per shard");
    const int fc = q.shards[k].fin_cnt;
    long long n = fc > q.shard_cap ? q.shard_cap : fc;
    long long pts = q.shards[k].points;
    int over = fc > q.shard_cap ? 1 : 0;
#pragma unroll
    for (int o = 32; o > 0; o >>= 1) { n += __shfl_down(n, o); pts += __shfl_down(pts, o); over |= __shfl_down(over, o); }
    if (k == 0) {
        counts[blockIdx.x * 4 + 0] = n;
        counts[blockIdx.x * 4 + 1] = pts;
        counts[blockIdx.x * 4 + 2] = (long long)(q.ctr->overflow | (over ? 2 : 0));
        counts[blockIdx.x * 4 + 3] = (long long)q.ctr->n_lanes;
    }
}

__global__ __launch_bounds__(PSFM_BLOCK) void psfm_compact_shards_batch_kernel(const PsfmFinSeq* __restrict__ T, unsigned long long* __restrict__ keys,
                                                                               int* __restrict__ lanes, PsfmKeyFmt fmt, int seq_shift)
{
    __shared__ int s_cnt[PSFM_NSHARD];
    const int shard = blockIdx.y, seq = blockIdx.z;
    const PsfmFinSeq& q = T[seq];
    if (threadIdx.x < PSFM_NSHARD) { const int fc = q.shards[threadIdx.x].fin_cnt; s_cnt[threadIdx.x] = fc > q.shard_cap ? q.shard_cap : fc; }
    __syncthreads();
    int64_t start = q.rec_start;
    for (int k = 0; k < shard; ++k) start += s_cnt[k];
    const int n = s_cnt[shard];
    for (int i = blockIdx.x * PSFM_BLOCK + threadIdx.x; i < n; i += gridDim.x * PSFM_BLOCK) {
        psfm_put_key(keys, start + i, q.fin_keys[(int64_t)shard * q.shard_cap + i], fmt, seq, seq_shift);
        lanes[start + i] = q.fin_lanes[(int64_t)shard * q.shard_cap + i];
    }
}

__global__ __launch_bounds__(PSFM_BLOCK) void psfm_decode_batch_kernel(const PsfmFinSeq* __restrict__ T, const void* __restrict__ keys, int64_t n,
                                                                       PsfmKeyFmt fmt, int seq_shift, int64_t* __restrict__ len64)
{
    const int64_t i = (int64_t)blockIdx.x * PSFM_BLOCK + threadIdx.x;
    if (i > n) return;
    if (i == n) { len64[i] = 0; return; }
    int seq, last, b, idx;
    const unsigned long long k = psfm_batch_split(psfm_key_at(keys, i, fmt.use32), fmt.use32, seq_shift, &seq);
    if (fmt.use32) psfm_key32_fields((unsigned)k, fmt.shift_b, &last, &b, &idx);
    else psfm_key64_fields(k, fmt.shift_b, fmt.shift_d, &last, &b, &idx);
    const PsfmFinSeq& q = T[seq];
    const int64_t local = i - q.rec_start;
    q.res_birth[local] = b;
    q.res_len[local] = last - b + 1;
    len64[i] = (int64_t)(last - b + 1);
}

__global__ __launch_bounds__(PSFM_BLOCK) void psfm_offsets_batch_kernel(const PsfmFinSeq* __restrict__ T, const int64_t* __restrict__ scan)
{
    const PsfmFinSeq& q = T[blockIdx.y];
    const int64_t i = (int64_t)blockIdx.x * PSFM_BLOCK + threadIdx.x;
    if (i > q.n) return;
    q.res_off[i] = scan[q.rec_start + i] - scan[q.rec_start];
}

__global__ __launch_bounds__(PSFM_BLOCK) void psfm_gather_batch_kernel(const PsfmFinSeq* __restrict__ T, const int* __restrict__ lanes)
{
    const PsfmFinSeq& q = T[blockIdx.y];
    if ((int64_t)blockIdx.x * TILE_J >= q.n) return;
    PsfmPlan none; none.gstart = nullptr;
    psfm_gather_body(q.log, q.cap, lanes + q.rec_start, q.res_birth, q.res_len, q.res_off, q.n, q.res_xy, none);
}

psfm_status psfm_finalize_batch(psfm_ctx* own, psfm_ctx* const* ctxs, const PsfmTrackDims* dims, int n_seq, hipStream_t s)
{
    if (n_seq < 1 || n_seq > PSFM_BATCH_MAX) { psfm_set_error("psfm_finalize_batch: bad batch size %d", n_seq); return PSFM_ERR_ARG; }
    psfm_status st;
    const size_t tbytes = sizeof(PsfmFinSeq) * (size_t)n_seq, cbytes = sizeof(long long) * 4 * (size_t)n_seq;
    if ((st = psfm_host_seg_ensure(own, tbytes + cbytes, 4096)) != PSFM_OK) return st;
    if ((st = own->seg_table.ensure(tbytes + cbytes)) != PSFM_OK) return st;
    PsfmFinSeq* hT = (PsfmFinSeq*)own->host_seg;
    long long* hcnt = (long long*)((char*)own->host_seg + tbytes);
    PsfmFinSeq* dT = own->seg_table.as<PsfmFinSeq>();
    long long* dcnt = (long long*)((char*)own->seg_table.p + tbytes);
    int64_t cap_max = 0;
    PsfmTrackDims dk = dims[0];
    for (int i = 0; i < n_seq; ++i) {
        const PsfmTrackDims& d = dims[i];
        psfm_ctx* c = ctxs[i];
        if (d.shift_b != dk.shift_b || d.shift_d != dk.shift_d) { psfm_set_error("psfm_finalize_batch: sequences with different key formats"); return PSFM_ERR_ARG; }
        if (d.n_flows > dk.n_flows) dk.n_flows = d.n_flows;
        memset(&hT[i], 0, sizeof(PsfmFinSeq));
        hT[i].birth_frame = c->birth_frame.as<int>(); hT[i].birth_idx = c->birth_idx.as<int>();
        hT[i].ctr = c->counters.as<PsfmCounters>(); hT[i].shards = c->shards.as<PsfmShard>();
        hT[i].fin_keys = c->fin_keys.as<unsigned long long>(); hT[i].fin_lanes = c->fin_lanes.as<int>();
        hT[i].log = c->log.as<double2>(); hT[i].cap = d.cap;
        hT[i].shard_cap = d.shard_cap; hT[i].last_time = d.n_flows;
        if (d.cap > cap_max) cap_max = d.cap;
    }
    PSFM_HIP(hipMemcpyAsync(dT, hT, tbytes, hipMemcpyHostToDevice, s));
    hipLaunchKernelGGL(psfm_collect_alive_batch_kernel, dim3((unsigned)((cap_max + PSFM_BLOCK - 1) / PSFM_BLOCK), (unsigned)n_seq), dim3(PSFM_BLOCK),
                       0, s, dT, dk.shift_b, dk.shift_d);
    hipLaunchKernelGGL(psfm_batch_counts_kernel, dim3((unsigned)n_seq), dim3(PSFM_WAVE), 0, s, dT, dcnt);
    PSFM_HIP(hipGetLastError());
    PSFM_HIP(hipMemcpyAsync(hcnt, dcnt, cbytes, hipMemcpyDeviceToHost, s));
    PSFM_HIP(hipStreamSynchronize(s));
    int64_t N = 0, n_max = 0;
    for (int i = 0; i < n_seq; ++i) {
        psfm_ctx* c = ctxs[i];
        const int64_t n = hcnt[4 * i + 0], npts = hcnt[4 * i + 1];
        PsfmCounters* hc = (PsfmCounters*)c->host_pinned;
        hc->n_lanes = (int)hcnt[4 * i + 3]; hc->overflow = (int)hcnt[4 * i + 2];
        if (hcnt[4 * i + 2] != 0 || hcnt[4 * i + 3] > dims[i].cap) {
            psfm_set_error("capacity exceeded (sequence %d of the batch): lanes used %lld of %lld, trajectory records %lld of %lld, overflow bits %lld; "
                           "raise psfm_ctx_set_capacity", i, hcnt[4 * i + 3], (long long)dims[i].cap, (long long)n, (long long)dims[i].traj_cap,
                           hcnt[4 * i + 2]);
            return PSFM_ERR_CAPACITY;
        }
        c->res_n_traj = n;
        c->res_n_points = npts;
        hT[i].rec_start = N; hT[i].n = n;
        N += n;
        if (n > n_max) n_max = n;
        if ((st = c->res_birth.ensure(sizeof(int) * (size_t)(n > 0 ? n : 1))) != PSFM_OK) return st;
        if ((st = c->res_len.ensure(sizeof(int) * (size_t)(n > 0 ? n : 1))) != PSFM_OK) return st;
        if ((st = c->res_off.ensure(sizeof(int64_t) * (size_t)(n + 1))) != PSFM_OK) return st;
        if ((st = c->res_xy.ensure(sizeof(double2) * (size_t)(npts > 0 ? npts : 1))) != PSFM_OK) return st;
        hT[i].res_birth = c->res_birth.as<int>(); hT[i].res_len = c->res_len.as<int>();
        hT[i].res_off = c->res_off.as<int64_t>(); hT[i].res_xy = c->res_xy.as<double2>();
    }
    PSFM_HIP(hipMemcpyAsync(dT, hT, tbytes, hipMemcpyHostToDevice, s));
    if (N == 0) {
        for (int i = 0; i < n_seq; ++i) PSFM_HIP(hipMemsetAsync(ctxs[i]->res_off.p, 0, sizeof(int64_t), s));
// ... 28 lines not shown
```

particle-sfm_amd/csrc/psfm_internal.h:

```cpp
#pragma once
#include <hip/hip_runtime.h>
#include <stdint.h>
#include <shared_mutex>
#include <string>
#include <vector>

#include "../../include/psfm.h"

#define PSFM_MAX_PEERS 8

void psfm_set_error(const char* fmt, ...);

#define PSFM_HIP(expr)                                                                          \
    do {                                                                                        \
        hipError_t e_ = (expr);                                                                 \
        if (e_ != hipSuccess) {                                                                 \
            psfm_set_error("%s failed: %s (%s:%d)", #expr, hipGetErrorString(e_), __FILE__, __LINE__); \
            return PSFM_ERR_HIP;                                                                \
        }                                                                                       \
    } while (0)

static inline bool psfm_frame_ok(int h, int w) { return h >= 2 && w >= 2 && (int64_t)h * (int64_t)w * 8 < ((int64_t)1 << 32); }

std::shared_mutex& psfm_device_gate(int device);
int psfm_gate_waiters(int device);
void psfm_gate_waiters_add(int device, int d);
struct PsfmGate {
    std::shared_mutex& m;
    int device;
    bool exclusive = false;
    PsfmGate(int dev, int want_exclusive ) : m(psfm_device_gate(dev)), device(dev)
    {
        if (want_exclusive == 2) { m.lock(); exclusive = true; }
        else if (want_exclusive == 1 && m.try_lock()) exclusive = true;
        else if (!m.try_lock_shared()) {
            psfm_gate_waiters_add(device, 1);
            m.lock_shared();
            psfm_gate_waiters_add(device, -1);
        }
    }
    bool yield_exclusive()
    {
        if (!exclusive || psfm_gate_waiters(device) <= 0) return false;
        m.unlock();
        exclusive = false;
        m.lock_shared();
        return true;
    }
    ~PsfmGate() { if (exclusive) m.unlock(); else m.unlock_shared(); }
    PsfmGate(const PsfmGate&) = delete;
    PsfmGate& operator=(const PsfmGate&) = delete;
};

struct PsfmBuf {
    void* p = nullptr;
    size_t bytes = 0;
    psfm_status ensure(size_t need);
    void release();
    template <class T> T* as() const { return (T*)p; }
};

struct PsfmCounters {
    int n_lanes;
    int overflow;
    int stall;
    int abort;
    int spill_cnt;
    int sel;
    int n_lanes_snap[2];
    int pc_frame, pc_phase, pc_owner, solve_K;
    int pad[4];
};

#define PSFM_NSHARD 64
struct PsfmShard {
    int fin_cnt;
    unsigned points;
    int pad0[30];
    int free_top;
    int pad1[31];
};

enum { PSFM_PROF_FLOW_CHECK = 0, PSFM_PROF_CHAIN = 1, PSFM_PROF_RESPAWN = 2, PSFM_PROF_SOLVER = 3,
       PSFM_PROF_FINALIZE = 4, PSFM_PROF_KINDS = 5 };

struct PsfmProfiler {
    bool enabled = false;
    int stride = 1;
    int64_t calls = 0;
    struct Span { int kind; hipEvent_t a, b; };
    std::vector<Span> spans;
    std::vector<hipEvent_t> pool;
    double total_ms[PSFM_PROF_KINDS] = {0};
    int64_t launches[PSFM_PROF_KINDS] = {0};
    hipEvent_t get();
    void begin(int kind, hipStream_t s);
    void kernel_span(int kind, hipEvent_t* a, hipEvent_t* b, bool always = false);
    void end(hipStream_t s);
    void collect();
    void reset();
    void destroy();
};

struct PsfmSolveCtrl;

struct PsfmTrackDims;

struct psfm_ctx {
    int device = 0;
    double lane_factor = 2.0, traj_factor = 8.0;
    PsfmBuf log;
    PsfmBuf birth_frame;
    PsfmBuf birth_idx;
    PsfmBuf free_stack;
    PsfmBuf fin_keys;
    PsfmBuf fin_lanes;
    PsfmBuf occupied;
    PsfmBuf counters;
    PsfmBuf shards;
    PsfmBuf survivors;
    PsfmBuf handoff;
    PsfmBuf seg_info;
    PsfmBuf seg_table;
    PsfmBuf persist_bar;
    int persist_max_blocks = -1;
    int chain_mode = 0;
    bool mb_enable = false;
    float mb_thres = 0.02f;
    PsfmBuf kill;
    void* host_seg = nullptr;
    size_t host_seg_bytes = 0;
    PsfmBuf sort_keys, sort_lanes, sort_tmp, scan_tmp;
    PsfmBuf fin_marks;
    bool fin_marks_clean = false;
    int fin_sort_form = 0, fin_offsets_form = 0;
    PsfmBuf res_birth, res_len, res_off, res_xy;
    int64_t res_n_traj = 0, res_n_points = 0;
    int res_n_flows = 0;
    bool res_is_query = false;
    PsfmBuf qr_ws;
    PsfmBuf sol_x, sol_state, sol_partials, sol_ctrl, sol_misc, sol_stats, sol_fused, sol_bar;
    PsfmBuf sol_list;
    int pc_persist_blocks[4] = {-1, -1, -1, -1};
    bool pc_persist_ok = false;
    int resident_budget = 0;
    unsigned pc_epoch = 0;
    PsfmBuf peer_area;
    unsigned peer_epoch = 0;
    int peer_world = 0, peer_rank = 0;
    int peer_L[PSFM_MAX_PEERS] = {0};
    void* peer_lead[PSFM_MAX_PEERS] = {nullptr};
    void* peer_opened[PSFM_MAX_PEERS] = {nullptr};
    int pc_giveups = 0;
    int solve_K = 4;
    int solve_mode = 0;
    int solver_mode = 0, solver_K = 0;
    int64_t n_fused_ok = 0, n_fused_redone = 0, n_chain = 0;
    int64_t n_resident = 0, n_iter_launches = 0;
    PsfmTrackDims* shard_dims = nullptr;
    bool shard_optimize = false;
    int solve_unroll = 6;
    PsfmBuf occ_own, occ2_own;
    PsfmBuf batch_tab, batch_ws, batch_fc;
    void* host_batch = nullptr;
    size_t host_batch_bytes = 0;
    void* host_batch2 = nullptr;
    size_t host_batch2_bytes = 0;
    int64_t batch_notrim_shape = 0;
    PsfmBuf win_ws;
    PsfmBuf flt_ids, flt_birth, flt_len, flt_off, flt_xy;
    int64_t flt_n_traj = 0, flt_n_points = 0;
    PsfmBuf mt_kp_off, mt_q, mt_pts, mt_kp_ind, mt_kp_xy, mt_moff, mt_keys, mt_rows, mt_gid, mt_pairs;
    int64_t mt_n_kp = 0, mt_n_m = 0, mt_n_pairs = 0;
    int mt_n_img = 0;
    uint64_t res_gen = 0;
    uint64_t lb_gen = 0;
    bool lb_active = false, lb_finished = false;
    int64_t lb_rows = 0;
    PsfmBuf lb_state, lb_first, lb_flag;
    PsfmBuf lb_ws;
    PsfmBuf lb_ids, lb_off, lb_frames, lb_xy, lb_labels;
    int64_t lb_n_traj = 0, lb_n_points = 0;
    PsfmBuf db_kp, db_pairs, db_rows, db_ws;
    int64_t db_n_kp = 0, db_n_pairs = 0, db_n_rows = 0, db_cap = 0;
    int db_n_img = 0;
    bool db_valid = false;
    bool db_src_live = false;
    PsfmBuf sd_ws;
    int64_t sd_budget = 1ll << 30;
    bool sd_timing = false;
    hipEvent_t sd_events[4] = {nullptr, nullptr, nullptr, nullptr};
    double sd_ms[3] = {0.0, 0.0, 0.0};
    PsfmBuf dd_ws, dd_comp;
    bool dd_timing = false;
    hipEvent_t dd_events[6] = {nullptr, nullptr, nullptr, nullptr, nullptr, nullptr};
    double dd_ms[4] = {0.0, 0.0, 0.0, 0.0};
    PsfmBuf gt_flag;
    hipStream_t side_stream = nullptr;
    hipStream_t copy_stream = nullptr;
    hipStream_t copy_stream2 = nullptr;
    std::vector<void*> ingest_slots;
    std::vector<hipEvent_t> ingest_events;
    size_t ingest_slot_bytes = 0;
    hipStream_t redo_stream = nullptr;
    std::vector<psfm_solve_stats> solve_stats;
    PsfmProfiler prof;
    void* host_pinned = nullptr;
    size_t host_pinned_bytes = 0;
};
static inline PsfmShard* psfm_host_shards(const psfm_ctx* c) { return (PsfmShard*)((char*)c->host_pinned + 512); }
static inline PsfmSolveCtrl* psfm_host_solve_ctrl(const psfm_ctx* c) { return (PsfmSolveCtrl*)(psfm_host_shards(c) + PSFM_NSHARD); }

psfm_status psfm_launch_flow_check(const float* ff, const float* fb, int n_pairs, int h, int w, float thres,
                                   uint8_t* occ, float* err, hipStream_t s);
psfm_status psfm_launch_flow_check_bg(const float* ff, const float* fb, int n_pairs, int h, int w, float thres, uint8_t* occ,
                                      int n_blocks, hipStream_t s);
psfm_status psfm_launch_grid_sample(const float* map, int c, int h, int w, const double* xy, int64_t n,
                                    float* out, hipStream_t s);

struct PsfmTrackDims {
    int H, W, ratio, GW, GH, n_flows;
    int64_t G, cap, traj_cap;
    int shard_cap;
    int free_cap;
    int nsh = PSFM_NSHARD;
    int shift_b, shift_d;
    float cw, ch;
    int nblk = 0, seg_cap = 0, spill_cap = 0;
    int64_t g0 = 0, Gband = 0, shard_pitch = 0;
    uint8_t* shard_maps = nullptr;
};

psfm_status psfm_track_dims(psfm_ctx* c, int n_flows, int h, int w, int ratio, int64_t g_own, PsfmTrackDims& d);
psfm_status psfm_track_alloc(psfm_ctx* c, const PsfmTrackDims& d);
psfm_status psfm_launch_track_init(psfm_ctx* c, const PsfmTrackDims& d, hipStream_t s);
psfm_status psfm_launch_chain_step(psfm_ctx* c, const PsfmTrackDims& d, const float* flow, const uint8_t* occ,
                                   int frame, bool optimize, hipStream_t s);

psfm_status psfm_launch_motion_boundary(const float* flows, const uint8_t* occ, int n, int h, int w, float thres, uint8_t* out, hipStream_t s);
psfm_status psfm_launch_chain_step_mb(psfm_ctx* c, const PsfmTrackDims& d, const float* flow, const uint8_t* kill, int frame, bool optimize,
                                      hipStream_t s);

psfm_status psfm_query_refuse(psfm_ctx* c, const char* who, const double* q_xy, const int32_t* q_t, unsigned Q, int n_flows,
                              unsigned long long* first_bad, hipStream_t s);
psfm_status psfm_query_finish(psfm_ctx* c, const int32_t* q_t, const int* len_f, const int* len_b, unsigned Q, int n_flows, int64_t* bsum,
                              int64_t* n_points, hipStream_t s);

#define PSFM_BATCH_MAX 64
struct PsfmBatchSeq;
struct PsfmFcSeq { const float* ff; const float* fb; uint8_t* occ; int n_pairs; int pad; };
bool psfm_flow_check_batch_ok(int h, int w, const void* ff, const void* fb, const void* occ);
psfm_status psfm_launch_flow_check_batch(const PsfmFcSeq* tab_dev, int n_seq, int pair0, int n_pairs, int h, int w, float thres, hipStream_t s);
void psfm_batch_fill_seq(psfm_ctx* c, const PsfmTrackDims& d, const float* flows, const uint8_t* occ, int64_t occ_pitch, PsfmBatchSeq* row);
psfm_status psfm_launch_track_init_batch(const PsfmBatchSeq* tab_dev, int n_seq, int64_t cap_max, hipStream_t s);
psfm_status psfm_launch_chain_step_batch(psfm_ctx* owner, const PsfmBatchSeq* tab_dev, int n_seq, int ratio, int64_t cap_max, int frame,
                                         bool optimize, hipStream_t s);
size_t psfm_batch_seq_opt_bytes(void);
psfm_status psfm_batch_fill_seq_opt(psfm_ctx* c, const PsfmTrackDims& d, const float* flows, const uint8_t* occ, int64_t occ_pitch,
                                    const float* flows_f2, const uint8_t* occ_s2, void* row_host, hipStream_t s);
psfm_status psfm_launch_seq_batch(psfm_ctx* owner, const void* tab_dev, int n_seq, int ratio, int64_t cap_max, int n_launches, int launch_id0,
                                  hipStream_t s);
psfm_status psfm_launch_flush_batch(const void* tab_dev, int n_seq, int64_t cap_max, hipStream_t s);
psfm_status psfm_launch_batch_set_pc(const void* tab_dev, const int (*v)[4], int n_seq, hipStream_t s);
size_t psfm_batch_pack_row_bytes(int win);
psfm_status psfm_launch_batch_pack(const void* tab_dev, const int* lo, int n_seq, int win, char* out_dev, hipStream_t s);
psfm_status psfm_finalize_batch(psfm_ctx* own, psfm_ctx* const* ctxs, const PsfmTrackDims* dims, int n_seq, hipStream_t s);

struct PsfmMatchSrc {
    int64_t k = 0, n_pts = 0;
    const int64_t* off = nullptr; const int* birth = nullptr; const int* frames = nullptr;
    const double2* xy = nullptr; const uint8_t* labels = nullptr;
    const char* who = "psfm_traj_to_matches";
};
psfm_status psfm_match_tables(psfm_ctx* c, const PsfmMatchSrc& src, int n_img, int sample_k, int64_t* n_kp_host, int64_t* n_matches_host,
                              int64_t* n_pairs_host, hipStream_t s);

int psfm_persist_max_blocks(psfm_ctx* c);
int psfm_persist_guests(void);
psfm_status psfm_launch_chain_persist(psfm_ctx* c, const PsfmTrackDims& d, const float* flows, const uint8_t* occ,
                                      int64_t occ_pitch, const float* flows_b, float thres, hipStream_t s);

psfm_status psfm_finalize(psfm_ctx* c, const PsfmTrackDims& d, hipStream_t s);
int psfm_sort_pairs32_passes(unsigned end_bit);
int psfm_sort_pairs64_passes(unsigned end_bit);
psfm_status psfm_sort_pairs64(psfm_ctx* c, unsigned long long* k_half0, int* v_half0, unsigned long long* k_half1, int* v_half1, int64_t n, unsigned end_bit, hipStream_t s);
psfm_status psfm_sort_pairs32(psfm_ctx* c, unsigned* k_half0, int* v_half0, unsigned* k_half1, int* v_half1, int64_t n, unsigned end_bit, hipStream_t s);
psfm_status psfm_finalize_persist(psfm_ctx* c, const PsfmTrackDims& d, bool* fallback, hipStream_t s);

psfm_status psfm_solve_frame_enqueue(psfm_ctx* c, const PsfmTrackDims& d, const float* flow01, const float* flow12,
                                     const float* flow02, const uint8_t* occ02, int frame, int unroll, hipStream_t s);
psfm_status psfm_solve_frame_resume(psfm_ctx* c, const PsfmTrackDims& d, const float* flow01, const float* flow12,
                                    const float* flow02, const uint8_t* occ02, int frame, psfm_solve_stats* st,
                                    int try_fused_k, bool chain_stalled, hipStream_t s);
psfm_status psfm_solve_frame_fused(psfm_ctx* c, const PsfmTrackDims& d, const float* flow01, const float* flow12,
                                   const float* flow02, const uint8_t* occ02, int frame, int K, hipStream_t s);
psfm_status psfm_launch_frame(psfm_ctx* c, const PsfmTrackDims& d, const float* flow01, const float* flow12, const float* flow02,
                              const uint8_t* occ, const uint8_t* occ02, int frame, int K, hipStream_t s, double* export_sums = nullptr);
psfm_status psfm_launch_seq(psfm_ctx* c, const PsfmTrackDims& d, const float* flows, const uint8_t* occ, int64_t occ_pitch,
                            const float* flows_f2, const uint8_t* occ_s2, int n_launches, int launch_id0, hipStream_t s);
psfm_status psfm_solve_flush(psfm_ctx* c, const PsfmTrackDims& d, int frame, hipStream_t s);
psfm_status psfm_solve_prepare(psfm_ctx* c, const PsfmTrackDims& d, hipStream_t s);
int psfm_solve_kmax(void);
int psfm_resident_blocks(psfm_ctx* c);
void psfm_shard_abandon(psfm_ctx* c);
psfm_status psfm_solve_export(psfm_ctx* c, const PsfmTrackDims& d, const float* flow01, const float* flow12, const float* flow02,
                              const uint8_t* occ02, int frame, int kind, int K, double* sums_out, hipStream_t s);
psfm_status psfm_solve_control(psfm_ctx* c, const PsfmTrackDims& d, int frame, int kind, int K, const double* totals, hipStream_t s,
                               int* stall_host = nullptr);
psfm_status psfm_solve_state(psfm_ctx* c, int* done, int* stall, psfm_solve_stats* st, hipStream_t s);
psfm_status psfm_solve_restore(psfm_ctx* c, const PsfmTrackDims& d, int frame, hipStream_t s);
psfm_status psfm_solve_writeback(psfm_ctx* c, const PsfmTrackDims& d, int frame, hipStream_t s);
size_t psfm_peer_area_bytes(void);
size_t psfm_peer_lead_offset(void);
int psfm_peer_leaders(int n_blocks);
int psfm_solve_blocks(psfm_ctx* c, const PsfmTrackDims& d);
psfm_status psfm_solve_frame_enqueue_peer(psfm_ctx* c, const PsfmTrackDims& d, const float* flow01, const float* flow12,
                                          const float* flow02, const uint8_t* occ02, int frame, unsigned epoch, hipStream_t s);
psfm_status psfm_launch_pc_eval(const double* uv12, const double* ref1, const double* ref2, const double* scale, const float* flow12,
                                int64_t n, int w, int h, double* res, double* jac, hipStream_t s);
psfm_status psfm_solve_batch(psfm_ctx* c, const double* uv12, const double* ref1, const double* ref2,
                             const double* scale, const float* flow12, int64_t n, int w, int h, double* out,
                             psfm_solve_stats* st, hipStream_t s);
```

particle-sfm_amd/csrc/psfm_persist.hip:

```cpp
#include <hip/hip_ext.h>
#include <stdlib.h>

#include "psfm_internal.h"
#include "psfm_chain.h"

#define PP_BLOCK 256
#define PP_NW (PP_BLOCK / PSFM_WAVE)
#define PP_PROBE 8
#ifndef PP_PRE_WAVES
#define PP_PRE_WAVES 4
#endif
#ifndef PP_KEEP
#define PP_KEEP 0
#endif
#ifndef PP_FC_AHEAD
#define PP_FC_AHEAD 4
#endif
#ifndef PP_FC_PAIRS
#define PP_FC_PAIRS 1
#endif
#define PP_GUESTS 32
#ifndef PP_WHATIF
#define PP_WHATIF 0
#endif
#ifndef PP_WAVES_N
#define PP_WAVES_N 8
#endif
#define PP_WAVES __attribute__((amdgpu_waves_per_eu(PP_WAVES_N, PP_WAVES_N)))

#ifdef PSFM_PERSIST_CHECK
#define PP_CHK(idx, lim, code) (((idx) >= 0 && (idx) < (lim)) ? true : (atomicCAS(&psfm_cold()->ctr->pad[0], 0, (code)), atomicMax(&psfm_cold()->ctr->pad[1], (int)(idx)), false))
#else
#define PP_CHK(idx, lim, code) true
#endif
#ifndef PP_COH_MARKS
#define PP_COH_MARKS true
#endif
#define PP_POOLED (-1)
#define PP_PEND (-2)
#define PP_DIED (-3)

struct PsfmPersistArgs {
    const float2* flows; uint8_t* occ;
    const float2* flows_b; float t2; int fc; int fc_xcd_per;
    int xcd_per;
    int64_t occ_pitch; PsfmFastDiv wdiv;
    int H, W; float cw, ch, rcw, rch;
    int ratio, GW, GH, G;
    float2* dlog; int cap;
    uint8_t* maps;
    unsigned long long* handoff;
    unsigned* bar;
    int n_flows;
    int nblk;
    PsfmFastDiv gwdiv, rdiv;
};
#define PP_SURV ((2 * PSFM_NSHARD + 1) * 32)

struct PsfmPersistCold {
    int cap_main;
    int cap;
    PsfmCounters* ctr;
    PsfmShard* shards;
    int* free_stack; int free_cap; int nsh;
    unsigned long long* fin_keys; int* fin_lanes;
    int seg_cap; int spill_base; int spill_cap;
    int2* seg_info;
    int shift_b, shift_d;
    int spin_limit;
};
struct PsfmPersistKernarg { PsfmPersistArgs hot; PsfmPersistCold cold; };

typedef const __attribute__((address_space(4))) PsfmPersistArgs* PsfmHotPtr;
typedef const __attribute__((address_space(4))) PsfmPersistCold* PsfmColdPtr;
__device__ __forceinline__ PsfmHotPtr psfm_hot()
{
    const __attribute__((address_space(4))) char* k = (const __attribute__((address_space(4))) char*)__builtin_amdgcn_kernarg_segment_ptr();
    asm volatile("" : "+s"(k));
    return (PsfmHotPtr)(k + offsetof(PsfmPersistKernarg, hot));
}
#define PA psfm_hot()
__device__ __forceinline__ int psfm_bid()
{
    int b = (int)blockIdx.x;
    asm volatile("" : "+s"(b));
    return b;
}
#define PP_BID psfm_bid()
#define PP_SHARD (psfm_bid() & (PSFM_NSHARD - 1))
template <class P> __device__ __forceinline__ PsfmFastDiv psfm_fd(P p)
{
    PsfmFastDiv f;
    f.m = p->m; f.sh1 = p->sh1; f.sh2 = p->sh2; f.d = 0u;
    return f;
}
__device__ __forceinline__ PsfmColdPtr psfm_cold()
{
    const __attribute__((address_space(4))) char* k = (const __attribute__((address_space(4))) char*)__builtin_amdgcn_kernarg_segment_ptr();
    asm volatile("" : "+s"(k));
    return (PsfmColdPtr)(k + offsetof(PsfmPersistKernarg, cold));
}

struct PsfmFrameView {
    const float2* flow; const uint8_t* occ;
    int H, W; float cw, ch, rcw, rch;
};
struct PsfmMarksView {
    int ratio, GW, GH;
    uint8_t* blocked_cur; uint8_t stamp_cur;
    PsfmFastDiv rdiv;
    float2* slab;
};

__device__ __forceinline__ PsfmFrameView psfm_frame_view(int t)
{
    const PsfmHotPtr a = psfm_hot();
    PsfmFrameView v;
    v.H = a->H; v.W = a->W; v.cw = a->cw; v.ch = a->ch; v.rcw = a->rcw; v.rch = a->rch;
    v.flow = a->flows + (size_t)t * ((size_t)v.H * v.W); v.occ = a->occ + (size_t)t * a->occ_pitch;
    return v;
}
template <int R>
__device__ __forceinline__ PsfmMarksView psfm_marks_view(int t)
{
    const PsfmHotPtr a = psfm_hot();
    PsfmMarksView m;
    m.ratio = R > 0 ? R : a->ratio; m.GW = a->GW; m.GH = a->GH;
    if (R > 0) { m.rdiv.m = 0u; m.rdiv.sh1 = 0; m.rdiv.sh2 = 0; m.rdiv.d = 0u; }
    else m.rdiv = psfm_fd(&a->rdiv);
    m.blocked_cur = a->maps + (size_t)(t % 3) * a->G; m.stamp_cur = 1;
    m.slab = a->dlog + (size_t)t * a->cap;
    return m;
}

__device__ __forceinline__ void psfm_put_record(int slot, unsigned long long key, int lane)
{
    const PsfmColdPtr c = psfm_cold();
    const int seg_cap = c->seg_cap;
    int64_t o;
    if (slot < seg_cap) {
        o = (int64_t)PP_BID * seg_cap + slot;
    } else {
        PsfmCounters* ctr = c->ctr;
        const int q = atomicAdd(&ctr->spill_cnt, 1);
        if (q >= c->spill_cap) { atomicOr(&ctr->overflow, 2); return; }
        o = (int64_t)c->spill_base + q;
    }
    if (!PP_CHK(lane, c->cap, 6)) return;
    c->fin_keys[o] = key;
    c->fin_lanes[o] = lane;
}
__device__ __forceinline__ unsigned long long psfm_cold_key(int last_time, int bf, int idx)
{
    const PsfmColdPtr c = psfm_cold();
    return psfm_key(last_time, bf, idx, c->shift_b, c->shift_d);
}

__device__ __forceinline__ int psfm_record_slot(int* s_rec_cnt, bool dead)
{
    const unsigned long long dm = __ballot(dead);
    if (dm == 0ull) return 0;
    int base = 0;
    if (psfm_lane_id() == (int)__builtin_ctzll(dm)) base = atomicAdd(s_rec_cnt, __popcll(dm));
    base = __shfl(base, (int)__builtin_ctzll(dm));
    return base + psfm_rank_in(dm);
}

#ifdef PSFM_TIMELINE
__device__ unsigned long long g_pp_tl[2 * 4096 * 8];
__device__ int g_pp_st[4096 * 8];
__device__ int g_pp_tl_frame = -1;
#define PP_TL(k) do { if ((unsigned)(t - g_pp_tl_frame) < 2u && tid == 0) g_pp_tl[((t - g_pp_tl_frame) * 4096 + blockIdx.x) * 8 + (k)] = __builtin_amdgcn_s_memrealtime(); } while (0)
extern "C" int psfm_debug_persist_timeline(int frame, unsigned long long* out_host, int n_blocks)
{
    if (out_host && n_blocks < 0) return hipMemcpyFromSymbol(out_host, HIP_SYMBOL(g_pp_st), (size_t)(-n_blocks) * 32) != hipSuccess;
    if (out_host) return hipMemcpyFromSymbol(out_host, HIP_SYMBOL(g_pp_tl), (size_t)2 * 4096 * 64) != hipSuccess;
    return hipMemcpyToSymbol(HIP_SYMBOL(g_pp_tl_frame), &frame, sizeof(int)) != hipSuccess;
}
#else
#define PP_TL(k) do {} while (0)
#endif

__device__ __forceinline__ void psfm_bar_arrive(int shard, int k, int lane)
{
    int last = 0;
    asm volatile("" : "+s"(k));
    if (lane == 0) {
        const int nblk = PA->nblk;
        const unsigned members = (unsigned)((nblk - shard + PSFM_NSHARD - 1) / PSFM_NSHARD);
        const unsigned old = __hip_atomic_fetch_add(PA->bar + shard * 32, 1u, __ATOMIC_RELAXED, __HIP_MEMORY_SCOPE_AGENT);
        if (old + 1 == members * (unsigned)(k + 1)) {
            const unsigned nsh = (unsigned)(nblk < PSFM_NSHARD ? nblk : PSFM_NSHARD);
            const unsigned o2 = __hip_atomic_fetch_add(PA->bar + 64 * 32, 1u, __ATOMIC_RELAXED, __HIP_MEMORY_SCOPE_AGENT);
            if (o2 + 1 == nsh * (unsigned)(k + 1)) last = 1;
        }
    }
    last = __builtin_amdgcn_readfirstlane(last);
    if (last) psfm_coh_st(PA->bar + (65 + lane) * 32, (unsigned)(k + 1));
}
__device__ __forceinline__ bool psfm_bar_wait(int shard, int k)
{
    const unsigned* flag = PA->bar + (65 + shard) * 32;
    int n = 0;
    while (psfm_coh_ld(flag) < (unsigned)(k + 1)) {
        __builtin_amdgcn_s_sleep(1);
        if (++n > psfm_cold()->spin_limit) { PsfmCounters* ctr = psfm_cold()->ctr; atomicOr(&ctr->overflow, 8); psfm_coh_st(&ctr->abort, 1); return false; }
        if ((n & 127) == 0 && psfm_coh_ld(&psfm_cold()->ctr->abort)) return false;
    }
// ... 44 lines not shown
}

struct PsfmEntry { int kind, ex, host; };

template <int R>
__global__ __launch_bounds__(PP_BLOCK) PP_WAVES void psfm_chain_persist_kernel(PsfmPersistKernarg)
{
    __shared__ int s_births[PP_NW], s_adopt[PP_NW], s_pend[PP_NW];
    __shared__ int s_new_g[PP_BLOCK];
    __shared__ int s_ad_tid[PP_BLOCK];
    __shared__ int s_pend_tid[PP_BLOCK];
    __shared__ double2 s_xp[PP_BLOCK];
    __shared__ int s_xg[PP_BLOCK];
    __shared__ int s_xf[PP_BLOCK];
    __shared__ int s_gi[PP_BLOCK];
    __shared__ int s_npts[PP_BLOCK];
    __shared__ int s_seg_start[PP_PROBE + 1], s_seg_end[PP_PROBE + 1];
    __shared__ int s_nseg, s_base_free, s_ok, s_alive_any[2], s_rec_cnt, s_done;
    __shared__ double2 s_gp[PP_GUESTS];
    __shared__ int s_gbf[PP_GUESTS];
    __shared__ int s_ggi[PP_GUESTS];
    __shared__ int s_glive[PP_GUESTS], s_gfree[PP_GUESTS], s_nglive, s_ngfree;

    int tid = threadIdx.x;
    int L = psfm_vblock() * PP_BLOCK + tid;
    const int ratio = R > 0 ? R : PA->ratio;

    int bf = PP_POOLED;
    double2 p = make_double2(0.0, 0.0);
    s_gi[tid] = L;
    s_npts[tid] = 0;
    if (L < PA->G) {
        const PsfmHotPtr a = psfm_hot();
        const int gy = (int)psfm_fastdiv((unsigned)L, psfm_fd(&a->gwdiv)), gx = L - gy * a->GW;
        p = make_double2((double)(gx * ratio), (double)(gy * ratio));
        bf = 0;
        s_npts[tid] = 1;
    }
    s_xf[tid] = 0;
    if (tid < PP_GUESTS) s_gbf[tid] = -1;
    if (tid == 0) { s_rec_cnt = 0; s_alive_any[0] = 0; s_alive_any[1] = 0; s_done = 0; }
    int fc_next = 0;
    if (PA->fc) {
        for (; fc_next < 2 && fc_next < PA->n_flows; ++fc_next) psfm_fc_slice(fc_next, tid);
        __builtin_amdgcn_s_waitcnt(0);
    }
    __syncthreads();
    if (tid / PSFM_WAVE == PP_NW - 1) psfm_bar_arrive(PP_SHARD, 0, tid & (PSFM_WAVE - 1));
    if (PA->fc) {
        if (tid == 0) s_ok = psfm_bar_wait(PP_SHARD, 0) ? 1 : 0;
        __syncthreads();
        if (!s_ok) return;
    }

    for (int t = 0; t < PA->n_flows; ++t) {
        asm volatile("" : "+v"(tid));
        L = psfm_vblock() * PP_BLOCK + tid;
        const int lane = tid & (PSFM_WAVE - 1), wave = tid / PSFM_WAVE;
        PsfmFrameView v = psfm_frame_view(t);
        const int cur = t & 1, prev = cur ^ 1;

        PP_TL(0);
        const bool live = bf >= 0;
        bool any_alive = false;
        int npts = 0;
        auto own_step = [&](const PsfmFrameView& vs, int s, const PsfmStepLoads& ld, bool mine, bool& alive_any) {
            PsfmStep s1;
            s1.alive = true;
            if (mine) s1 = psfm_step_finish(vs, p, ld);
            const int slot1 = psfm_record_slot(&s_rec_cnt, !s1.alive);
            if (mine) {
                if (s1.alive) {
                    const PsfmMarksView m = psfm_marks_view<R>(s);
                    if (PP_CHK(L, PA->cap, 1)) m.slab[L] = s1.flow;
                    psfm_block_grid<R, PP_COH_MARKS>(m, (int)s1.next.x, (int)s1.next.y);
                    p = s1.next;
                    alive_any = true;
                    ++npts;
                } else {
                    psfm_put_record(slot1, psfm_cold_key(s, bf, s_gi[tid]), L);
                    bf = PP_DIED;
                    p = make_double2(0.0, 0.0);
                }
            }
        };
        PsfmStepLoads l1 = psfm_step_issue(v, p);

        auto do_E = [&]() { own_step(v, t, l1, live, any_alive); };
        const bool e_first = wave < PP_PRE_WAVES;
        if (e_first) do_E();

        if (PA->fc) {
            const PsfmHotPtr a = psfm_hot();
            const unsigned* flag = a->bar + (65 + PP_SHARD) * 32;
            const int nf = a->n_flows, fc_lim = t + PP_FC_AHEAD < nf ? t + PP_FC_AHEAD : nf;
            while (fc_next < fc_lim) {
                if (__builtin_amdgcn_readfirstlane((int)psfm_coh_ld(flag)) >= t + 1 || (PP_WHATIF & 32)) break;
                psfm_fc_slice(fc_next, tid);
                ++fc_next;
            }
        }
        if (tid == 0) s_ok = (PP_WHATIF & 4) ? 1 : (psfm_bar_wait(PP_SHARD, t) ? 1 : 0);
        __syncthreads();
        if (!s_ok) return;

#ifndef PP_NO_SETPRIO
        __builtin_amdgcn_s_setprio(3);
#endif
        PP_TL(1);
        const bool poll = t > 0 && bf == PP_POOLED && !(PP_WHATIF & 8);
        const PsfmHotPtr ac = psfm_hot();
        const int G = ac->G;
        const bool gridpt = t > 0 && L < G && !(PP_WHATIF & 8);
        uint8_t* map_prev = ac->maps + (size_t)((t + 2) % 3) * G;
        unsigned sv = 0, byte = 0;
        unsigned long long h0 = 0, h1 = 0, h2 = ~0ull;
        if (t > 0 && PP_BID == 0 && tid < PSFM_NSHARD) sv = psfm_coh_ld(ac->bar + PP_SURV + (prev * PSFM_NSHARD + tid) * 32);
        if (gridpt) byte = psfm_coh_ld(map_prev + L);
        if (poll) {
            const unsigned long long* h = ac->handoff + (size_t)L * 3;
            h0 = psfm_coh_ld(h); h1 = psfm_coh_ld(h + 1); h2 = psfm_coh_ld(h + 2);
        }

        v = psfm_frame_view(t);
        if (!e_first) do_E();

        const unsigned long long svm = __ballot(sv == (unsigned)t);
        bool birth = false;
        if (gridpt) {
            if (byte != 0) psfm_coh_st(map_prev + L, (uint8_t)0);
            birth = byte == 0;
            if (L == 0 && svm == 0ull) {
                const int r0 = R > 0 ? R : PA->ratio;
                birth = ((0 + 1) * (0 + 1) + 0 * 0) > r0 * r0;
            }
            if (PP_WHATIF & 1) birth = false;
        }
        bool adopted = false;
        if (poll) {
            const int tag = (int)(h2 >> 32);
            if ((tag >> 1) == t - 1 && !(PP_WHATIF & 1)) {
                if (tag & 1) {
                    adopted = true;
                    s_xp[tid] = make_double2(__longlong_as_double((long long)h0), __longlong_as_double((long long)h1));
                    s_xg[tid] = (int)(unsigned)h2;
                } else {
                    bf = PP_PEND;
                }
            }
        }
        const bool pend = bf == PP_PEND;
        if (bf == PP_DIED) bf = PP_PEND;
        const unsigned long long bm = __ballot(birth), am = __ballot(adopted), pm = __ballot(pend);
        if (lane == 0) { s_births[wave] = __popcll(bm); s_adopt[wave] = __popcll(am); s_pend[wave] = __popcll(pm); }
        if (birth) s_new_g[wave * PSFM_WAVE + psfm_rank_in(bm)] = L;
        if (adopted) s_ad_tid[wave * PSFM_WAVE + psfm_rank_in(am)] = tid;
        if (pend) s_pend_tid[wave * PSFM_WAVE + psfm_rank_in(pm)] = tid;
        if (wave == 0) {
            const int gb = tid < PP_GUESTS ? s_gbf[tid] : -1;
            const bool gl = gb >= 0, gf = (tid < PP_GUESTS) & (gb < 0);
            const unsigned long long glm = __ballot(gl), gfm = __ballot(gf);
            if (lane == 0) { s_nglive = __popcll(glm); s_ngfree = __popcll(gfm); }
            if (gl) s_glive[psfm_rank_in(glm)] = tid;
            if (gf) s_gfree[psfm_rank_in(gfm)] = tid;
        }
        __syncthreads();

        PP_TL(2);
        int nb = 0, nad = 0, npd = 0, my_pend_before = 0;
#pragma unroll
        for (int w = 0; w < PP_NW; ++w) {
            if (w == wave) my_pend_before = npd;
            nb += s_births[w]; nad += s_adopt[w]; npd += s_pend[w];
        }
        const int matched = nb < npd ? nb : npd;
        const int ngl = s_nglive;
        const int gmatched = (nb - matched) < s_ngfree ? (nb - matched) : s_ngfree;
        const int n2 = nb + nad + ngl;
        const int t_frame = t, nb_f = __builtin_amdgcn_readfirstlane(nb), nad_f = __builtin_amdgcn_readfirstlane(nad), npd_f = __builtin_amdgcn_readfirstlane(npd),
                  matched_f = __builtin_amdgcn_readfirstlane(matched), gmatched_f = __builtin_amdgcn_readfirstlane(gmatched);

        for (int base = 0; base == 0 || base < n2; base += PP_BLOCK) {
            int t = t_frame, nb = nb_f, nad = nad_f, npd = npd_f, matched = matched_f, gmatched = gmatched_f;
            asm volatile("" : "+s"(t), "+s"(nb), "+s"(nad), "+s"(npd), "+s"(matched), "+s"(gmatched));
            const int cur = t & 1, prev = cur ^ 1;
            const int k = base + tid;
            PsfmEntry e;
            e.kind = 0; e.ex = -1; e.host = -1;
            if (k < nb) {
                int before = 0, pb = 0;
#pragma unroll
                for (int w = 0; w < PP_NW; ++w) {
                    const int c = s_births[w], pc = s_pend[w];
                    if (k >= before && k < before + c) e.ex = s_new_g[w * PSFM_WAVE + (k - before)];
                    if (k >= pb && k < pb + pc) e.host = s_pend_tid[w * PSFM_WAVE + (k - pb)];
                    before += c; pb += pc;
                }
                e.kind = 1;
            } else if (k < nb + nad) {
                const int kk = k - nb;
                int before = 0;
#pragma unroll
                for (int w = 0; w < PP_NW; ++w) {
                    const int c = s_adopt[w];
                    if (kk >= before && kk < before + c) e.ex = s_ad_tid[w * PSFM_WAVE + (kk - before)];
                    before += c;
                }
                e.kind = 2;
            } else if (k < n2) {
                e.ex = s_glive[k - nb - nad];
                e.kind = 3;
            }
            PsfmStepLoads l2 = {};
            if (e.kind != 0) {
                double2 q;
                if (e.kind == 1) {
                    const PsfmHotPtr a = psfm_hot();
                    const int gy = (int)psfm_fastdiv((unsigned)e.ex, psfm_fd(&a->gwdiv)), gx = e.ex - gy * a->GW;
                    q = make_double2((double)(gx * ratio), (double)(gy * ratio));
                } else if (e.kind == 2) {
                    q = s_xp[e.ex];
                } else {
                    q = s_gp[e.ex];
                }
                l2 = psfm_step_issue(v, q);
            }
#ifdef PSFM_TIMELINE
            if (base == 0 && tid == 0 && t == g_pp_tl_frame) {
                int* st = g_pp_st + PP_BID * 8;
                st[0] = nb; st[1] = nad; st[2] = npd; st[3] = ngl; st[4] = s_ngfree; st[5] = nb - matched - gmatched; st[6] = npd - matched - PP_KEEP;
            }
#endif
            if (base == 0 && tid == 0) {
                const PsfmColdPtr c = psfm_cold();
                const int nsh = c->nsh, free_cap = c->free_cap;
                PsfmShard* sh_pop = c->shards + cur * PSFM_NSHARD;
                PsfmShard* sh_push = c->shards + prev * PSFM_NSHARD;
                int need = nb - matched - gmatched;
                const int n_push = npd - matched - PP_KEEP;
                int bfree = 0;
                const int fsh = PP_BID % nsh;
                if (n_push > 0) bfree = atomicAdd(&sh_push[fsh].free_top, n_push);
                int nseg = 0, done = 0;
                for (int rd = 0; rd < PP_PROBE / 4 && need > 0; ++rd) {
                    const int q4 = need >> 2, r4 = need & 3;
                    int sh[4], ask[4], old[4];
#pragma unroll
                    for (int j = 0; j < 4; ++j) {
                        sh[j] = (fsh + (rd * 4 + j) * 7) % nsh;
                        ask[j] = q4 + (j < r4 ? 1 : 0);
                        old[j] = ask[j] > 0 ? atomicSub(&sh_pop[sh[j]].free_top, ask[j]) : 0;
                    }
#pragma unroll
                    for (int j = 0; j < 4; ++j) {
                        const int take = old[j] < 0 ? 0 : (old[j] > ask[j] ? ask[j] : old[j]);
                        if (take < ask[j]) atomicAdd(&sh_pop[sh[j]].free_top, ask[j] - take);
                        if (take > 0) {
                            s_seg_start[nseg] = sh[j] * free_cap + old[j] - 1;
                            done += take;
                            s_seg_end[nseg] = done;
                            ++nseg;
                            need -= take;
                        }
                    }
                }
                s_base_free = bfree;
                if (need > 0) {
                    const int base_new = atomicAdd(&c->ctr->n_lanes, need);
                    s_seg_start[nseg] = -(base_new + 1);
                    done += need;
                    s_seg_end[nseg] = done;
                    ++nseg;
                }
                s_nseg = nseg;
            }
            PP_TL(3);
            __syncthreads();
            PP_TL(4);

            if (base == 0) {
                if (pend) {
                    const int r = my_pend_before + psfm_rank_in(pm);
                    if (r >= matched + PP_KEEP) {
                        const PsfmColdPtr c = psfm_cold();
                        const int free_cap = c->free_cap;
                        int* free_push = c->free_stack + (size_t)prev * free_cap * PSFM_NSHARD;
                        const int fpos = s_base_free + (r - matched - PP_KEEP);
                        if (fpos < free_cap && PP_CHK(fpos, free_cap, 7)) psfm_coh_st(free_push + (size_t)(PP_BID % c->nsh) * free_cap + fpos, L);
                        else atomicOr(&c->ctr->overflow, 1);
                        bf = PP_POOLED;
                    }
                }
            }
            psfm_step_pin<true>(l2);
            asm volatile("" : "+v"(e.ex));
            if (e.kind != 0) {
                double2 q;
                int bfk, gik, col, gs = -1;
                if (e.kind == 1) {
                    const PsfmHotPtr a = psfm_hot();
                    const int gy = (int)psfm_fastdiv((unsigned)e.ex, psfm_fd(&a->gwdiv)), gx = e.ex - gy * a->GW;
                    q = make_double2((double)(gx * ratio), (double)(gy * ratio));
                    bfk = t; gik = e.ex;
                    if (k < matched) {
                        col = psfm_vblock() * PP_BLOCK + e.host;
                    } else if (k < matched + gmatched) {
                        gs = s_gfree[k - matched];
                        col = psfm_cold()->cap_main + PP_BID * PP_GUESTS + gs;
                    } else {
                        const PsfmColdPtr c = psfm_cold();
                        const int* free_pop = c->free_stack + (size_t)cur * c->free_cap * PSFM_NSHARD;
                        const int qq = k - matched - gmatched;
                        int j = 0, pv = 0;
                        while (j < s_nseg - 1 && qq >= s_seg_end[j]) { pv = s_seg_end[j]; ++j; }
                        const int st = s_seg_start[j];
                        if (st >= 0) (void)PP_CHK(st - (qq - pv), 2 * c->free_cap * PSFM_NSHARD, 9);
                        col = st >= 0 ? psfm_coh_ld(free_pop + (st - (qq - pv))) : (-(st + 1) + (qq - pv));
                        if (col >= c->cap_main) col = -1;
                    }
                } else if (e.kind == 2) {
                    q = s_xp[e.ex];
                    bfk = t - 1; gik = s_xg[e.ex];
                    col = psfm_vblock() * PP_BLOCK + e.ex;
                } else {
                    q = s_gp[e.ex];
                    bfk = s_gbf[e.ex]; gik = s_ggi[e.ex];
                    col = psfm_cold()->cap_main + PP_BID * PP_GUESTS + e.ex;
                }
                if (col >= 0) {
                    (void)PP_CHK(col, PA->cap, 2);
                    const PsfmStep s2 = psfm_step_finish(v, q, l2);
                    if (e.kind == 1) ++npts;
                    if (s2.alive) {
                        const PsfmMarksView m = psfm_marks_view<R>(t);
                        if (PP_CHK(col, PA->cap, 3)) m.slab[col] = s2.flow;
                        psfm_block_grid<R, PP_COH_MARKS>(m, (int)s2.next.x, (int)s2.next.y);
                        any_alive = true;
                        ++npts;
                    } else {
                        const int slot = atomicAdd(&s_rec_cnt, 1);
                        psfm_put_record(slot, psfm_cold_key(t, bfk, gik), col);
                    }
                    if (e.kind == 1) {
                        const bool popped = k >= matched + gmatched;
                        const int nf = PA->n_flows;
                        if (popped && s2.alive && t == nf - 1) {
                            const int slot = atomicAdd(&s_rec_cnt, 1);
                            psfm_put_record(slot, psfm_cold_key(nf, t, e.ex), col);
                        }
                        if (k < matched) {
                            s_xp[e.host] = s2.next; s_xg[e.host] = e.ex; s_xf[e.host] = s2.alive ? 1 : 2;
                        } else if (gs >= 0) {
                            if (s2.alive) { s_gp[gs] = s2.next; s_ggi[gs] = e.ex; s_gbf[gs] = t; }
                        } else if (PP_CHK(col, psfm_cold()->cap_main, 8)) {
                            unsigned long long* h = PA->handoff + (size_t)col * 3;
                            psfm_coh_st(h, (unsigned long long)__double_as_longlong(s2.next.x));
                            psfm_coh_st(h + 1, (unsigned long long)__double_as_longlong(s2.next.y));
                            psfm_coh_st(h + 2, (unsigned long long)(unsigned)e.ex |
                                                   ((unsigned long long)(unsigned)(2 * t + (s2.alive ? 1 : 0)) << 32));
                        }
                    } else if (e.kind == 2) {
                        if (s2.alive) s_xp[e.ex] = s2.next;
                        s_xf[e.ex] = s2.alive ? 3 : 2;
                    } else {
                        if (s2.alive) s_gp[e.ex] = s2.next;
                        else s_gbf[e.ex] = -1;
                    }
                } else {
                    atomicOr(&psfm_cold()->ctr->overflow, 4);
                }
            }
        }
        PP_TL(5);
        asm volatile("" : "+s"(t), "+v"(tid));
        if (npts) s_npts[tid] += npts;
        const unsigned long long alm = __ballot(any_alive);
        if (lane == 0 && alm != 0ull) s_alive_any[t & 1] = 1;
        __syncthreads();
        {
            const int f = s_xf[tid];
            if (f != 0) {
                s_xf[tid] = 0;
                if (f != 2) {
                    bf = f == 3 ? t - 1 : t;
                    s_gi[tid] = s_xg[tid];
                    p = s_xp[tid];
                } else {
                    bf = PP_PEND;
                }
            }
        }
        if (tid == 0 && s_alive_any[t & 1]) { psfm_coh_st(PA->bar + PP_SURV + ((t & 1) * PSFM_NSHARD + PP_SHARD) * 32, (unsigned)(t + 1)); s_alive_any[t & 1] = 0; }
        if (PA->fc) {
            const int nf = PA->n_flows, need = t + 3 < nf ? t + 3 : nf;
            if (!(PP_WHATIF & 16)) for (; fc_next < need; ++fc_next) psfm_fc_slice(fc_next, tid);
        }
        if (!(PP_WHATIF & 2)) asm volatile("s_waitcnt vmcnt(0) lgkmcnt(0)" ::: "memory");
        PP_TL(6);
        {
            int last_wave = 0;
            if (lane == 0) last_wave = atomicAdd(&s_done, 1) == PP_NW - 1 ? 1 : 0;
            last_wave = __builtin_amdgcn_readfirstlane(last_wave);
            if (last_wave) {
                if (lane == 0) s_done = 0;
                PP_TL(7);
                psfm_bar_arrive(PP_SHARD, t + 1, lane);
            }
        }
#ifndef PP_NO_SETPRIO
        __builtin_amdgcn_s_setprio(0);
#endif
    }

    const int lane = tid & (PSFM_WAVE - 1), wave = tid / PSFM_WAVE;
    {
        const int nf = PA->n_flows;
        const bool alive = bf >= 0;
        const int slot = psfm_record_slot(&s_rec_cnt, alive);
        if (alive) psfm_put_record(slot, psfm_cold_key(nf, bf, s_gi[tid]), L);
        if (tid < PP_GUESTS && s_gbf[tid] >= 0) {
            const int gslot = atomicAdd(&s_rec_cnt, 1);
            psfm_put_record(gslot, psfm_cold_key(nf, s_gbf[tid], s_ggi[tid]),
                            psfm_cold()->cap_main + PP_BID * PP_GUESTS + tid);
        }
    }
    {
        __shared__ int s_pts[PP_NW];
        int w = s_npts[tid];
#pragma unroll
        for (int o = 32; o > 0; o >>= 1) w += __shfl_down(w, o);
        if (lane == 0) s_pts[wave] = w;
        __syncthreads();
        if (tid == 0) {
            int tot = 0;
            for (int j = 0; j < PP_NW; ++j) tot += s_pts[j];
            const int c = s_rec_cnt;
            const PsfmColdPtr cold = psfm_cold();
            const int seg_cap = cold->seg_cap;
            cold->seg_info[PP_BID] = make_int2(c < seg_cap ? c : seg_cap, tot);
        }
    }
}

__global__ __launch_bounds__(256) void psfm_persist_init_kernel(PsfmCounters* ctr, PsfmShard* shards, int G,
                                                                unsigned long long* maps64, size_t n_maps64,
                                                                unsigned long long* bar64, size_t n_bar64,
                                                                unsigned long long* handoff, size_t n_handoff)
{
    const size_t i = (size_t)blockIdx.x * 256 + threadIdx.x, stride = (size_t)gridDim.x * 256;
    if (i == 0) { ctr->n_lanes = G; ctr->overflow = 0; ctr->stall = 0; ctr->abort = 0; ctr->spill_cnt = 0; ctr->pad[0] = 0; ctr->pad[1] = 0; }
    if (i < 2 * PSFM_NSHARD) { shards[i].fin_cnt = 0; shards[i].free_top = 0; shards[i].points = 0u; }
    for (size_t k = i; k < n_maps64; k += stride) maps64[k] = 0ull;
    for (size_t k = i; k < n_bar64; k += stride) bar64[k] = 0ull;
    for (size_t k = i; k < n_handoff; k += stride) handoff[k] = ~0ull;
}

int psfm_persist_guests(void) { return PP_GUESTS; }

int psfm_persist_max_blocks(psfm_ctx* c)
{
    if (c->persist_max_blocks >= 0) return c->persist_max_blocks;
    int cus = 0;
    c->persist_max_blocks = 0;
    if (hipDeviceGetAttribute(&cus, hipDeviceAttributeMultiprocessorCount, c->device) != hipSuccess) {
        (void)hipGetLastError();
        return 0;
    }
    int per_cu = 1 << 30;
    const void* inst[4] = {(const void*)psfm_chain_persist_kernel<0>, (const void*)psfm_chain_persist_kernel<1>,
                           (const void*)psfm_chain_persist_kernel<2>, (const void*)psfm_chain_persist_kernel<4>};
    for (int k = 0; k < 4; ++k) {
        int v = 0;
        if (hipOccupancyMaxActiveBlocksPerMultiprocessor(&v, inst[k], PP_BLOCK, 0) != hipSuccess) {
            (void)hipGetLastError();
            return 0;
        }
        per_cu = v < per_cu ? v : per_cu;
    }
    if (per_cu > 8) per_cu = 8;
    c->persist_max_blocks = per_cu * cus;
    return c->persist_max_blocks;
}

psfm_status psfm_launch_chain_persist(psfm_ctx* c, const PsfmTrackDims& d, const float* flows, const uint8_t* occ,
                                      int64_t occ_pitch, const float* flows_b, float thres, hipStream_t s)
{
    const size_t bar_bytes = (size_t)(4 * PSFM_NSHARD + 1) * 128;
    {
        const size_t n_maps64 = ((size_t)d.G * 3 + 7) / 8, n_bar64 = bar_bytes / 8, n_handoff = (size_t)d.nblk * PP_BLOCK * 3;
        hipLaunchKernelGGL(psfm_persist_init_kernel, dim3(1024), dim3(256), 0, s, c->counters.as<PsfmCounters>(),
                           c->shards.as<PsfmShard>(), (int)d.G, c->occupied.as<unsigned long long>(), n_maps64,
                           c->persist_bar.as<unsigned long long>(), n_bar64, c->handoff.as<unsigned long long>(), n_handoff);
    }
    PsfmPersistKernarg ka;
    PsfmPersistArgs& a = ka.hot;
    PsfmPersistCold& k = ka.cold;
    a.flows = (const float2*)flows; a.occ = const_cast<uint8_t*>(occ);
    a.occ_pitch = occ_pitch;
    a.flows_b = (const float2*)flows_b; a.t2 = psfm_sq_threshold(thres); a.fc = flows_b != nullptr;
    {
        static const int xcd_on = getenv("PSFM_FC_XCD") ? atoi(getenv("PSFM_FC_XCD")) : 1;
        const int64_t nch = ((int64_t)d.H * d.W + 1023) / 1024;
        a.fc_xcd_per = xcd_on && nch >= 64 ? (int)((nch + 7) / 8) : 0;
    }
    {
        static const int pp_xcd = getenv("PSFM_PP_XCD") ? atoi(getenv("PSFM_PP_XCD")) : 1;
        const int64_t gb = (d.G + PP_BLOCK - 1) / PP_BLOCK;
        const int per = (int)((gb + 7) / 8);
        a.xcd_per = (pp_xcd && gb >= 64 && 8 * per <= d.nblk) ? per : 0;
    }
    a.wdiv = psfm_fastdiv_make((unsigned)d.W);
    a.H = d.H; a.W = d.W; a.cw = d.cw; a.ch = d.ch; a.rcw = psfm_rcp_host(d.cw); a.rch = psfm_rcp_host(d.ch);
    a.ratio = d.ratio; a.GW = d.GW; a.GH = d.GH; a.G = (int)d.G;
    a.dlog = c->log.as<float2>(); a.cap = k.cap = (int)d.cap; k.cap_main = d.nblk * PP_BLOCK;
    a.maps = c->occupied.as<uint8_t>();
    k.ctr = c->counters.as<PsfmCounters>();
    k.shards = c->shards.as<PsfmShard>();
    k.free_stack = c->free_stack.as<int>(); k.free_cap = d.free_cap; k.nsh = d.nsh;
    a.handoff = c->handoff.as<unsigned long long>();
    k.fin_keys = c->fin_keys.as<unsigned long long>(); k.fin_lanes = c->fin_lanes.as<int>();
    k.seg_cap = d.seg_cap; k.spill_base = d.nblk * d.seg_cap; k.spill_cap = d.spill_cap;
    k.seg_info = c->seg_info.as<int2>();
    a.bar = c->persist_bar.as<unsigned>();
    a.n_flows = d.n_flows; a.nblk = d.nblk; k.shift_b = d.shift_b; k.shift_d = d.shift_d;
    a.gwdiv = psfm_fastdiv_make((unsigned)d.GW); a.rdiv = psfm_fastdiv_make((unsigned)d.ratio);
    k.spin_limit = 1 << 18;
    if (const char* e = getenv("PSFM_PERSIST_SPIN_LIMIT")) k.spin_limit = atoi(e);
    hipEvent_t e0 = nullptr, e1 = nullptr;
    c->prof.kernel_span(PSFM_PROF_CHAIN, &e0, &e1, true);
    const dim3 grid((unsigned)d.nblk), block(PP_BLOCK);
    const bool coop = getenv("PSFM_PERSIST_COOP") && atoi(getenv("PSFM_PERSIST_COOP")) != 0;
    const void* fn = d.ratio == 1 ? (const void*)psfm_chain_persist_kernel<1> : d.ratio == 2 ? (const void*)psfm_chain_persist_kernel<2>
                   : d.ratio == 4 ? (const void*)psfm_chain_persist_kernel<4> : (const void*)psfm_chain_persist_kernel<0>;
    if (coop) {
        void* kargs[] = {(void*)&ka};
        if (e0) PSFM_HIP(hipEventRecord(e0, s));
        const hipError_t le = hipLaunchCooperativeKernel(fn, grid, block, kargs, 0, s);
        if (le != hipSuccess) {
            (void)hipGetLastError();
            psfm_set_error("cooperative launch of the persistent frame loop refused: %s", hipGetErrorString(le));
            return PSFM_ERR_CAPACITY;
        }
        if (e1) PSFM_HIP(hipEventRecord(e1, s));
        return PSFM_OK;
    }
    switch (d.ratio) {
        case 1: hipExtLaunchKernelGGL(psfm_chain_persist_kernel<1>, grid, block, 0, s, e0, e1, 0, ka); break;
        case 2: hipExtLaunchKernelGGL(psfm_chain_persist_kernel<2>, grid, block, 0, s, e0, e1, 0, ka); break;
        case 4: hipExtLaunchKernelGGL(psfm_chain_persist_kernel<4>, grid, block, 0, s, e0, e1, 0, ka); break;
        default: hipExtLaunchKernelGGL(psfm_chain_persist_kernel<0>, grid, block, 0, s, e0, e1, 0, ka); break;
    }
    PSFM_HIP(hipGetLastError());
    return PSFM_OK;
}
```

particle-sfm_amd/point_trajectory/_hip.py:

```python
import ctypes
import os

_PKG = os.path.dirname(os.path.dirname(os.path.abspath(__file__)))
LIB_PATH = os.environ.get("PSFM_HIP_LIB", os.path.join(_PKG, "lib", "libpsfm_hip.so"))

PSFM_OK, PSFM_ERR_ARG, PSFM_ERR_HIP, PSFM_ERR_CAPACITY, PSFM_ERR_SOLVER = 0, 1, 2, 3, 4
PROF_KINDS = {"flow_check": 0, "chain_step": 1, "respawn": 2, "solver": 3, "finalize": 4}

EXPORTS = [
    "psfm_last_error", "psfm_version", "psfm_device_count", "psfm_ctx_create", "psfm_ctx_destroy",
    "psfm_ctx_set_capacity", "psfm_flow_check", "psfm_grid_sample", "psfm_optimize_location", "psfm_track",
    "psfm_connect",
    "psfm_result_device", "psfm_result_copy", "psfm_result_solve_stats", "psfm_ctx_set_profiling",
    "psfm_profile_get", "psfm_ctx_set_chain_mode", "psfm_window_sample", "psfm_result_filter", "psfm_result_filtered_copy",
    "psfm_ctx_set_solver", "psfm_solver_counters", "psfm_traj_to_matches", "psfm_matches_copy",
    "psfm_shard_begin", "psfm_shard_step", "psfm_shard_solve_export", "psfm_shard_solve_control", "psfm_shard_solve_restore",
    "psfm_shard_solve_writeback", "psfm_shard_solve_record", "psfm_shard_finish", "psfm_result_keys",
    "psfm_shard_solve_control_async", "psfm_shard_window_state", "psfm_shard_peek_stall", "psfm_shard_frame",
    "psfm_shard_solve_control_chain_async", "psfm_shard_solve_poll", "psfm_shard_solve_local", "psfm_shard_solve_redo_local", "psfm_connect_batch", "psfm_solver_launches", "psfm_ctx_set_resident_budget", "psfm_resident_capacity", "psfm_load_flo_stack",
    "psfm_path_consistency_eval", "psfm_sort_records", "psfm_sort_records64", "psfm_ctx_get_finalize_forms",
    "psfm_shard_peer_area", "psfm_shard_peer_epoch", "psfm_shard_peer_open", "psfm_shard_peer_connect", "psfm_shard_solve_blocks", "psfm_shard_solve_peer",
    "psfm_labels_begin", "psfm_labels_merge_window", "psfm_labels_finish", "psfm_labels_device", "psfm_labels_copy", "psfm_labels_to_matches",
    "psfm_traj_augment", "psfm_traj_encode_weight_count", "psfm_traj_encode",
    "psfm_traj_decode_weight_count", "psfm_traj_decode_workspace_bytes", "psfm_traj_decode",
    "psfm_traj_eval_counts", "psfm_traj_vote_labels",
    "psfm_labels_set", "psfm_matches_to_database", "psfm_database_copy", "psfm_database_chunk_rows",
    "psfm_database_compact_again",
    "psfm_sparse_depth", "psfm_sparse_depth_sort_ids", "psfm_ctx_set_sparse_depth", "psfm_ctx_get_sparse_depth_budget",
    "psfm_sparse_depth_last_ms", "psfm_colmap_points3d_count", "psfm_colmap_points3d_scan",
    "psfm_ctx_set_motion_boundary", "psfm_motion_boundary", "psfm_kill_map",
    "psfm_depth_display", "psfm_ctx_set_depth_display", "psfm_depth_display_last_ms", "psfm_depth_display_chunk",
    "psfm_track_queries", "psfm_track_queries_optimize",
]


class SolveStats(ctypes.Structure):
    _fields_ = [("iterations", ctypes.c_int32), ("successful_steps", ctypes.c_int32),
                ("termination", ctypes.c_int32), ("dogleg_nonGN", ctypes.c_int32),
                ("initial_cost", ctypes.c_double), ("final_cost", ctypes.c_double)]

    def as_dict(self):
        return {k: getattr(self, k) for k, _ in self._fields_}


class TrackInfo(ctypes.Structure):
    _fields_ = [("n_traj", ctypes.c_int64), ("n_points", ctypes.c_int64), ("n_lanes_peak", ctypes.c_int64),
                ("lane_capacity", ctypes.c_int64), ("solver_iterations", ctypes.c_int64),
                ("n_solves", ctypes.c_int32), ("chain_mode", ctypes.c_int32)]

    def as_dict(self):
        return {k: getattr(self, k) for k, _ in self._fields_}


class PsfmError(RuntimeError):
    def __init__(self, status, msg):
        super().__init__("libpsfm_hip status %d: %s" % (status, msg))
        self.status = status


_lib = None


def lib():
    global _lib
    if _lib is not None:
        return _lib
    if not os.path.exists(LIB_PATH):
        raise RuntimeError(
            "libpsfm_hip.so not found at %s -- build it with `python particle-sfm_amd/build.py` "
            "(the HIP extension is mandatory, there is no CPU fallback)" % LIB_PATH)
    import torch
    L = ctypes.CDLL(LIB_PATH)
    vp, i32, i64, f32, f64 = ctypes.c_void_p, ctypes.c_int, ctypes.c_int64, ctypes.c_float, ctypes.c_double
    L.psfm_last_error.restype = ctypes.c_char_p
    L.psfm_last_error.argtypes = []
    L.psfm_version.restype = i32
    L.psfm_device_count.restype = i32
    L.psfm_ctx_create.argtypes = [i32, ctypes.POINTER(vp)]
    L.psfm_ctx_destroy.argtypes = [vp]
    L.psfm_ctx_set_capacity.argtypes = [vp, f64, f64]
    L.psfm_load_flo_stack.argtypes = [vp, ctypes.POINTER(ctypes.c_char_p), i32, i32, i32, vp, i32, vp]
    L.psfm_flow_check.argtypes = [vp, vp, vp, i32, i32, i32, f32, vp, vp, vp]
    L.psfm_grid_sample.argtypes = [vp, vp, i32, i32, i32, vp, i64, vp, vp]
    L.psfm_optimize_location.argtypes = [vp, vp, vp, vp, vp, vp, i64, i32, i32, vp, ctypes.POINTER(SolveStats), vp]
    L.psfm_path_consistency_eval.argtypes = [vp, vp, vp, vp, vp, vp, i64, i32, i32, vp, vp, vp]
    L.psfm_sort_records.argtypes = [vp, vp, vp, i64, i32, vp]
    L.psfm_sort_records64.argtypes = [vp, vp, vp, i64, i32, vp]
    L.psfm_ctx_get_finalize_forms.argtypes = [vp, ctypes.POINTER(ctypes.c_int32), ctypes.POINTER(ctypes.c_int32)]
    L.psfm_track.argtypes = [vp, vp, vp, vp, vp, i32, i32, i32, i32, ctypes.POINTER(TrackInfo), vp]
    L.psfm_connect.argtypes = [vp, vp, vp, vp, vp, i32, i32, i32, f32, i32, vp, vp, ctypes.POINTER(TrackInfo), vp]
    L.psfm_connect_batch.argtypes = [ctypes.POINTER(vp), i32, ctypes.POINTER(vp), ctypes.POINTER(vp), ctypes.POINTER(vp), ctypes.POINTER(vp),
                                     ctypes.POINTER(i32), i32, i32, f32, i32, ctypes.POINTER(TrackInfo), vp]
    L.psfm_track_queries.argtypes = [vp, vp, vp, vp, vp, i32, i32, i32, vp, vp, i64, ctypes.POINTER(TrackInfo), vp]
    L.psfm_track_queries_optimize.argtypes = [vp, vp, vp, vp, vp, vp, vp, vp, vp, i32, i32, i32, vp, vp, i64, ctypes.POINTER(TrackInfo), vp]
    L.psfm_result_device.argtypes = [vp, ctypes.POINTER(vp), ctypes.POINTER(vp), ctypes.POINTER(vp), ctypes.POINTER(vp)]
    L.psfm_result_copy.argtypes = [vp, vp, vp, vp, vp, vp]
    L.psfm_result_solve_stats.argtypes = [vp, ctypes.POINTER(SolveStats), i32, ctypes.POINTER(ctypes.c_int32)]
    L.psfm_ctx_set_profiling.argtypes = [vp, i32]
    L.psfm_ctx_set_chain_mode.argtypes = [vp, i32]
    L.psfm_ctx_set_solver.argtypes = [vp, i32, i32]
    L.psfm_ctx_set_motion_boundary.argtypes = [vp, i32, f32]
    L.psfm_motion_boundary.argtypes = [vp, vp, i32, i32, i32, f32, vp, vp]
    L.psfm_kill_map.argtypes = [vp, vp, vp, i32, i32, i32, f32, vp, vp]
    L.psfm_solver_counters.argtypes = [vp, ctypes.POINTER(i64), ctypes.POINTER(i64), ctypes.POINTER(i64), ctypes.POINTER(ctypes.c_int32)]
    L.psfm_ctx_set_resident_budget.argtypes = [vp, i32]
    L.psfm_resident_capacity.argtypes = [vp, ctypes.POINTER(ctypes.c_int32)]
    L.psfm_solver_launches.argtypes = [vp, ctypes.POINTER(i64), ctypes.POINTER(i64), ctypes.POINTER(i64)]
    L.psfm_result_filter.argtypes = [vp, i32, ctypes.POINTER(i64), ctypes.POINTER(i64), vp]
    L.psfm_result_filtered_copy.argtypes = [vp, vp, vp, vp, vp, vp, vp]
    L.psfm_window_sample.argtypes = [vp, i32, i32, i32, i32, i64, ctypes.c_uint64, i32, i32, i32, i32, i64, vp, vp, vp, vp,
                                     ctypes.POINTER(i64), vp]
    L.psfm_traj_augment.argtypes = [vp, vp, vp, vp, i64, i32, i32, i32, vp, vp, vp]
    L.psfm_traj_encode_weight_count.argtypes = []
    L.psfm_traj_encode.argtypes = [vp, vp, vp, vp, i64, i32, vp, vp]
    L.psfm_traj_decode_weight_count.argtypes = []
    L.psfm_traj_decode_workspace_bytes.argtypes = [i64]
    L.psfm_traj_decode.argtypes = [vp, vp, vp, i64, vp, ctypes.c_size_t, vp, vp, vp, vp]
    L.psfm_traj_eval_counts.argtypes = [vp, vp, vp, vp, i64, vp, vp, i32, i32, i32, vp, vp]
    L.psfm_traj_vote_labels.argtypes = [vp, vp, vp, vp, i64, i32, i32, i32, vp, vp]
    L.psfm_traj_to_matches.argtypes = [vp, i32, i32, vp, ctypes.POINTER(i64), ctypes.POINTER(i64), ctypes.POINTER(i64), vp]
    L.psfm_matches_copy.argtypes = [vp, vp, vp, vp, vp, vp, vp, vp]
    L.psfm_labels_begin.argtypes = [vp, vp]
    L.psfm_labels_merge_window.argtypes = [vp, i32, i32, vp, vp, i64, vp]
    L.psfm_labels_finish.argtypes = [vp, ctypes.POINTER(i64), ctypes.POINTER(i64), vp]
    L.psfm_labels_device.argtypes = [vp, ctypes.POINTER(vp), ctypes.POINTER(vp), ctypes.POINTER(vp), ctypes.POINTER(vp), ctypes.POINTER(vp)]
    L.psfm_labels_copy.argtypes = [vp, vp, vp, vp, vp, vp, vp]
    L.psfm_labels_to_matches.argtypes = [vp, i32, i32, i32, ctypes.POINTER(i64), ctypes.POINTER(i64), ctypes.POINTER(i64), vp]
    L.psfm_labels_set.argtypes = [vp, i64, i64, vp, vp, vp, vp, vp, vp]
    L.psfm_matches_to_database.argtypes = [vp, i32, vp, vp, ctypes.POINTER(i64), ctypes.POINTER(i64), vp]
    L.psfm_database_copy.argtypes = [vp, vp, vp, vp, vp, vp, vp]
    L.psfm_database_chunk_rows.argtypes = []
    L.psfm_database_compact_again.argtypes = [vp, vp]
    L.psfm_sparse_depth.argtypes = [vp, vp, vp, i64, vp, i32, vp, vp, vp, i64, vp, ctypes.POINTER(i64), vp]
    L.psfm_sparse_depth_sort_ids.argtypes = [vp, vp, i64, vp, vp, vp]
    L.psfm_ctx_set_sparse_depth.argtypes = [vp, i64, i32]
    L.psfm_ctx_get_sparse_depth_budget.argtypes = [vp, ctypes.POINTER(i64)]
    L.psfm_sparse_depth_last_ms.argtypes = [vp, ctypes.POINTER(f64)]
    L.psfm_depth_display.argtypes = [vp, vp, vp, i32, f64, vp, vp, vp, vp, vp, vp]
    L.psfm_ctx_set_depth_display.argtypes = [vp, i32]
    L.psfm_depth_display_last_ms.argtypes = [vp, ctypes.POINTER(f64)]
    L.psfm_depth_display_chunk.argtypes = []
    L.psfm_colmap_points3d_count.argtypes = [vp, ctypes.c_uint64, ctypes.POINTER(ctypes.c_uint64)]
    L.psfm_colmap_points3d_scan.argtypes = [vp, ctypes.c_uint64, vp, vp, vp, vp]
    L.psfm_shard_begin.argtypes = [vp, i32, i32, i32, i32, i64, i64, i32, vp, i64, vp]
    L.psfm_shard_step.argtypes = [vp, vp, vp, i32, vp]
    L.psfm_shard_solve_export.argtypes = [vp, vp, vp, vp, vp, i32, i32, i32, vp, vp]
    L.psfm_shard_frame.argtypes = [vp, vp, vp, vp, vp, vp, i32, i32, vp, vp]
    L.psfm_shard_solve_control.argtypes = [vp, i32, i32, i32, vp, ctypes.POINTER(ctypes.c_int32), ctypes.POINTER(ctypes.c_int32),
                                           ctypes.POINTER(SolveStats), vp]
    L.psfm_shard_solve_control_async.argtypes = [vp, i32, i32, vp, vp]
    L.psfm_shard_solve_control_chain_async.argtypes = [vp, i32, i32, vp, vp]
    L.psfm_shard_solve_poll.argtypes = [vp, ctypes.POINTER(ctypes.c_int32), ctypes.POINTER(SolveStats), vp]
    L.psfm_shard_solve_local.argtypes = [vp, vp, vp, vp, vp, i32, i32, vp]
    L.psfm_shard_peer_area.argtypes = [vp, ctypes.POINTER(vp), vp, vp]
    L.psfm_shard_peer_open.argtypes = [vp, vp, i32, ctypes.POINTER(vp)]
    L.psfm_shard_peer_epoch.argtypes = [vp, ctypes.POINTER(ctypes.c_uint32), i32, vp]
    L.psfm_shard_peer_connect.argtypes = [vp, i32, i32, ctypes.POINTER(vp), ctypes.POINTER(ctypes.c_int32)]
    L.psfm_shard_solve_blocks.argtypes = [vp, ctypes.POINTER(ctypes.c_int32)]
    L.psfm_shard_solve_peer.argtypes = [vp, vp, vp, vp, vp, i32, ctypes.c_uint32, vp]
    L.psfm_shard_solve_redo_local.argtypes = [vp, vp, vp, vp, vp, i32, i32, ctypes.POINTER(SolveStats), vp]
    L.psfm_shard_window_state.argtypes = [vp, i32, i32, ctypes.POINTER(SolveStats), ctypes.POINTER(ctypes.c_int32), vp]
    L.psfm_shard_peek_stall.argtypes = [vp, ctypes.POINTER(ctypes.c_int32)]
    L.psfm_shard_solve_restore.argtypes = [vp, i32, vp]
    L.psfm_shard_solve_writeback.argtypes = [vp, i32, ctypes.POINTER(SolveStats), vp]
    L.psfm_shard_solve_record.argtypes = [vp, ctypes.POINTER(SolveStats)]
    L.psfm_shard_finish.argtypes = [vp, ctypes.POINTER(TrackInfo), vp]
    L.psfm_result_keys.argtypes = [vp, i32, i32, vp, vp]
    L.psfm_profile_get.argtypes = [vp, i32, ctypes.POINTER(f64), ctypes.POINTER(i64)]
    for name in EXPORTS:
        if name != "psfm_last_error":
            getattr(L, name).restype = i32
    L.psfm_traj_decode_workspace_bytes.restype = ctypes.c_size_t
    _lib = L
    return L


def check(status):
    if status != PSFM_OK:
        raise PsfmError(status, lib().psfm_last_error().decode("utf-8", "replace"))


class Context:

    def __init__(self, device=0):
        self._h = ctypes.c_void_p()
        check(lib().psfm_ctx_create(int(device), ctypes.byref(self._h)))
        self.device = int(device)
        self.resident_budget = 0

    @property
    def handle(self):
        return self._h

    def set_capacity(self, lane_factor, traj_factor):
        check(lib().psfm_ctx_set_capacity(self._h, float(lane_factor), float(traj_factor)))

    def set_chain_mode(self, mode):
        check(lib().psfm_ctx_set_chain_mode(self._h, int(mode)))

    def set_motion_boundary(self, enable, thres=0.02):
        check(lib().psfm_ctx_set_motion_boundary(self._h, int(bool(enable)), float(thres)))

    def set_solver(self, mode, k=0):
        check(lib().psfm_ctx_set_solver(self._h, int(mode), int(k)))

    def set_resident_budget(self, blocks):
        check(lib().psfm_ctx_set_resident_budget(self._h, int(blocks)))
        self.resident_budget = int(blocks)

    def resident_capacity(self):
        n = ctypes.c_int32()
        check(lib().psfm_resident_capacity(self._h, ctypes.byref(n)))
        return int(n.value)

    def solver_counters(self):
        a, b, c_, k = ctypes.c_int64(), ctypes.c_int64(), ctypes.c_int64(), ctypes.c_int32()
        check(lib().psfm_solver_counters(self._h, ctypes.byref(a), ctypes.byref(b), ctypes.byref(c_), ctypes.byref(k)))
        out = {"fused": a.value, "fused_redone": b.value, "chain": c_.value, "k": k.value}
        r, g, it = ctypes.c_int64(), ctypes.c_int64(), ctypes.c_int64()
        check(lib().psfm_solver_launches(self._h, ctypes.byref(r), ctypes.byref(g), ctypes.byref(it)))
        out.update({"resident_launches": r.value, "resident_giveups": g.value, "iteration_launches": it.value})
        return out

    def finalize_forms(self):
        a, b = ctypes.c_int32(), ctypes.c_int32()
        check(lib().psfm_ctx_get_finalize_forms(self._h, ctypes.byref(a), ctypes.byref(b)))
        return {"sort": int(a.value), "offsets": int(b.value)}

    def set_sparse_depth(self, budget_bytes=1 << 30, timing=False):
        check(lib().psfm_ctx_set_sparse_depth(self._h, int(budget_bytes), int(bool(timing))))

    def sparse_depth_ms(self):
        ms = (ctypes.c_double * 3)()
        check(lib().psfm_sparse_depth_last_ms(self._h, ms))
        return {"fill_ms": ms[0], "winner_ms": ms[1], "store_ms": ms[2]}

    def set_depth_display(self, timing=False):
        check(lib().psfm_ctx_set_depth_display(self._h, int(bool(timing))))

    def depth_display_ms(self):
        ms = (ctypes.c_double * 4)()
        check(lib().psfm_depth_display_last_ms(self._h, ms))
        return {"count_ms": ms[0], "compact_ms": ms[1], "select_ms": ms[2], "colour_ms": ms[3]}

    def set_profiling(self, enable):
        check(lib().psfm_ctx_set_profiling(self._h, int(enable)))

    def profile(self):
        out = {}
        for name, k in PROF_KINDS.items():
            ms, n = ctypes.c_double(), ctypes.c_int64()
            check(lib().psfm_profile_get(self._h, k, ctypes.byref(ms), ctypes.byref(n)))
            out[name] = {"total_ms": ms.value, "launches": n.value}
        return out

    def close(self):
        if self._h:
            lib().psfm_ctx_destroy(self._h)
            self._h = ctypes.c_void_p()

    def __del__(self):
        try:
            self.close()
        except Exception:
            pass


_contexts = {}
_contexts_lock = __import__("threading").Lock()


def context(device=None):
    import threading
    import torch
    if not torch.cuda.is_available():
        raise RuntimeError("point_trajectory (MI355X build) needs a HIP device: torch.cuda.is_available() is False "
                           "and there is no CPU fallback")
    if device is None:
        device = torch.cuda.current_device()
    device = int(device)
    key = (device, threading.get_ident())
    with _contexts_lock:
        ctx = _contexts.get(key)
    if ctx is None:
        ctx = Context(device)
        with _contexts_lock:
            _contexts[key] = ctx
    return ctx


def batch_contexts(n, device=None):
    import threading
    first = context(device)
    out = [first]
    for k in range(1, int(n)):
        key = (first.device, threading.get_ident(), "batch", k)
        with _contexts_lock:
            ctx = _contexts.get(key)
        if ctx is None:
            ctx = Context(first.device)
            with _contexts_lock:
                _contexts[key] = ctx
        out.append(ctx)
    return out


def release_thread_contexts():
    import threading
    tid = threading.get_ident()
    with _contexts_lock:
        mine = [_contexts.pop(k) for k in [k for k in _contexts if k[1] == tid]]
    for ctx in mine:
        ctx.close()


def current_stream_ptr(device=None):
    import torch
    return ctypes.c_void_p(torch.cuda.current_stream(device).cuda_stream)


def ptr(t):
    if t is None:
        return ctypes.c_void_p(0)
    return ctypes.c_void_p(t.data_ptr())
```

Measured before the change: 22.05 billion trajectory-points/s.

## Place finalize records directly via per-frame birth bitmasks and single-digit sort

The persistent tracking kernel now records, for each frame, a per-wave ballot bitmask of which grid points gave birth to a trajectory. At finalize, a scan over these masks yields each record's exact placement offset, so records are written in place instead of being compacted. A one-pass 8-bit digit scatter sort, keyed on the trajectory's last frame, replaces the general radix sort. This is meant to cut the compaction and multi-pass sort cost, in exchange for extra global writes in the hot persistent loop and a new table allocation. It is gated on specific form conditions and can be disabled with an environment variable.

```diff
diff --git a/include/psfm.h b/include/psfm.h
--- a/include/psfm.h
+++ b/include/psfm.h
@@ -96,6 +96,8 @@
 psfm_status psfm_sort_records64(psfm_ctx* ctx, uint64_t* keys, int32_t* values, int64_t n, int end_bit, void* stream);
 
 psfm_status psfm_ctx_get_finalize_forms(psfm_ctx* ctx, int* sort_form, int* offsets_form);
+
+psfm_status psfm_ctx_get_finalize_placed(psfm_ctx* ctx, int* placed);
 
 psfm_status psfm_track(psfm_ctx* ctx, const float* flows, const uint8_t* occ, const float* flows_f2,
                        const uint8_t* occ_s2, int n_flows, int h, int w, int sample_ratio,
diff --git a/particle-sfm_amd/build.py b/particle-sfm_amd/build.py
--- a/particle-sfm_amd/build.py
+++ b/particle-sfm_amd/build.py
@@ -8,7 +8,7 @@
 OBJ = os.path.join(HERE, "build")
 LIBDIR = os.path.join(HERE, "lib")
 LIB = os.path.join(LIBDIR, "libpsfm_hip.so")
-SOURCES = ["psfm_api.hip", "psfm_track.hip", "psfm_persist.hip", "psfm_finalize.hip", "psfm_sort.hip", "psfm_sort64.hip", "psfm_solver.hip", "psfm_solver_fused.hip", "psfm_solver_batch.hip", "psfm_window.hip", "psfm_matches.hip", "psfm_shard.hip", "psfm_batch.hip", "psfm_ingest.hip", "psfm_labels.hip", "psfm_augment.hip", "psfm_encoder.hip", "psfm_decoder.hip", "psfm_ground_truth.hip", "psfm_database.hip", "psfm_sparse_depth.hip", "psfm_motion_boundary.hip", "psfm_depth_display.hip", "psfm_query.hip", "psfm_query_pc.hip"]
+SOURCES = ["psfm_api.hip", "psfm_track.hip", "psfm_persist.hip", "psfm_finalize.hip", "psfm_place.hip", "psfm_sort.hip", "psfm_sort64.hip", "psfm_solver.hip", "psfm_solver_fused.hip", "psfm_solver_batch.hip", "psfm_window.hip", "psfm_matches.hip", "psfm_shard.hip", "psfm_batch.hip", "psfm_ingest.hip", "psfm_labels.hip", "psfm_augment.hip", "psfm_encoder.hip", "psfm_decoder.hip", "psfm_ground_truth.hip", "psfm_database.hip", "psfm_sparse_depth.hip", "psfm_motion_boundary.hip", "psfm_depth_display.hip", "psfm_query.hip", "psfm_query_pc.hip"]
 HIPCC = os.environ.get("HIPCC", "/opt/rocm/bin/hipcc")
 FLAGS = ["--offload-arch=gfx950", "-O3", "-std=c++17", "-fPIC", "-ffp-contract=off", "-fno-fast-math",
          "-Wall", "-Wno-unused-function", "-Wno-unused-result",
diff --git a/particle-sfm_amd/csrc/psfm_api.hip b/particle-sfm_amd/csrc/psfm_api.hip
--- a/particle-sfm_amd/csrc/psfm_api.hip
+++ b/particle-sfm_amd/csrc/psfm_api.hip
@@ -153,7 +153,7 @@
                        &c->occupied, &c->counters, &c->shards, &c->survivors, &c->sort_keys, &c->sort_lanes, &c->sort_tmp,
                        &c->scan_tmp, &c->fin_marks, &c->res_birth, &c->res_len, &c->res_off, &c->res_xy, &c->sol_x, &c->sol_state,
                        &c->sol_partials, &c->sol_ctrl, &c->sol_misc, &c->sol_stats, &c->sol_fused, &c->sol_bar, &c->sol_list, &c->occ_own, &c->occ2_own,
-                       &c->handoff, &c->seg_info, &c->seg_table, &c->persist_bar, &c->batch_tab, &c->batch_ws, &c->batch_fc, &c->win_ws, &c->flt_ids, &c->flt_birth, &c->flt_len, &c->flt_off, &c->flt_xy,
+                       &c->handoff, &c->place_tab, &c->seg_info, &c->seg_table, &c->persist_bar, &c->batch_tab, &c->batch_ws, &c->batch_fc, &c->win_ws, &c->flt_ids, &c->flt_birth, &c->flt_len, &c->flt_off, &c->flt_xy,
                        &c->mt_kp_off, &c->mt_q, &c->mt_pts, &c->mt_kp_ind, &c->mt_kp_xy, &c->mt_moff, &c->mt_keys, &c->mt_rows, &c->mt_gid, &c->mt_pairs,
                        &c->lb_state, &c->lb_first, &c->lb_flag, &c->lb_ws, &c->lb_ids, &c->lb_off, &c->lb_frames, &c->lb_xy, &c->lb_labels, &c->gt_flag, &c->kill,
                        &c->db_kp, &c->db_pairs, &c->db_rows, &c->db_ws, &c->sd_ws, &c->dd_ws, &c->dd_comp, &c->qr_ws};
@@ -373,6 +373,13 @@
     PSFM_CHECK_CTX(c);
     if (sort_form) *sort_form = c->fin_sort_form;
     if (offsets_form) *offsets_form = c->fin_offsets_form;
+    return PSFM_OK;
+}
+
+extern "C" psfm_status psfm_ctx_get_finalize_placed(psfm_ctx* c, int* placed)
+{
+    PSFM_CHECK_CTX(c);
+    if (placed) *placed = c->fin_placed;
     return PSFM_OK;
 }
 
@@ -493,6 +500,7 @@
             if ((st = c->handoff.ensure((size_t)dp.nblk * 256 * 24)) != PSFM_OK) return st;
             if ((st = c->seg_info.ensure(sizeof(int) * 2 * (size_t)dp.nblk)) != PSFM_OK) return st;
             if ((st = c->persist_bar.ensure((size_t)(4 * PSFM_NSHARD + 1) * 128)) != PSFM_OK) return st;
+            if ((st = c->place_tab.ensure(psfm_place_table_bytes(dp))) != PSFM_OK) return st;
             if (pipe && (st = pipe->need(n_flows - 1, false, s)) != PSFM_OK) return st;
             bool fallback = false;
             {
diff --git a/particle-sfm_amd/csrc/psfm_finalize.hip b/particle-sfm_amd/csrc/psfm_finalize.hip
--- a/particle-sfm_amd/csrc/psfm_finalize.hip
+++ b/particle-sfm_amd/csrc/psfm_finalize.hip
@@ -6,6 +6,7 @@
 #include "psfm_device.h"
 #include "psfm_finalize_plan.h"
 #include "psfm_internal.h"
+#include "psfm_place.h"
 
 #define PSFM_BLOCK 256
 
@@ -383,13 +384,17 @@
     return PSFM_OK;
 }
 
-static psfm_status psfm_sort_records(psfm_ctx* c, const PsfmFinForm& f, int64_t n, size_t* scan_bytes, hipStream_t s)
+static psfm_status psfm_sort_records(psfm_ctx* c, const PsfmFinForm& f, int64_t n, size_t* scan_bytes, hipStream_t s, bool placed = false)
 {
     psfm_status st;
     PSFM_HIP(rocprim::exclusive_scan(nullptr, *scan_bytes, (int64_t*)nullptr, (int64_t*)nullptr, (int64_t)0,
                                      (size_t)(n + 1), rocprim::plus<int64_t>(), s));
-    c->fin_sort_form = 0; c->fin_offsets_form = 0;
-    if (f.sort_form == 3) {
+    c->fin_sort_form = 0; c->fin_offsets_form = 0; c->fin_placed = 0;
+    if (placed) {
+        int* l_out = c->sort_lanes.as<int>();
+        if ((st = c->sort_tmp.ensure(*scan_bytes)) != PSFM_OK) return st;
+        st = psfm_place_sort(c, c->sort_keys.as<unsigned>(), l_out, c->sort_keys.as<unsigned>() + n, l_out + n, n, s);
+    } else if (f.sort_form == 3) {
         st = f.fmt.use32 ? psfm_rocprim_sort<unsigned>(c, n, f.end_bit, *scan_bytes, s) : psfm_rocprim_sort<unsigned long long>(c, n, f.end_bit, *scan_bytes, s);
     } else {
         int* l_out = c->sort_lanes.as<int>();
@@ -399,6 +404,7 @@
     }
     if (st != PSFM_OK) return st;
     c->fin_sort_form = f.sort_form;
+    c->fin_placed = placed ? 1 : 0;
     return PSFM_OK;
 }
 
@@ -413,11 +419,11 @@
 }
 
 static psfm_status psfm_finalize_sorted(psfm_ctx* c, const PsfmTrackDims& d, const PsfmFinForm& f, int64_t n, int64_t npts, bool delta_log,
-                                        hipStream_t s)
+                                        hipStream_t s, bool placed = false)
 {
     psfm_status st;
     size_t scan_bytes = 0;
-    if ((st = psfm_sort_records(c, f, n, &scan_bytes, s)) != PSFM_OK) return st;
+    if ((st = psfm_sort_records(c, f, n, &scan_bytes, s, placed)) != PSFM_OK) return st;
     if ((st = c->res_birth.ensure(sizeof(int) * n)) != PSFM_OK) return st;
     if ((st = c->res_len.ensure(sizeof(int) * n)) != PSFM_OK) return st;
     if ((st = c->res_off.ensure(sizeof(int64_t) * (n + 1))) != PSFM_OK) return st;
@@ -577,6 +583,11 @@
     if ((st = c->sort_keys.ensure(sizeof(unsigned long long) * n * 2)) != PSFM_OK) return st;
     if ((st = c->sort_lanes.ensure(sizeof(int) * n * 2)) != PSFM_OK) return st;
     const PsfmFinForm f = psfm_form_of(d, n);
+    static const int place_on = getenv("PSFM_FIN_PLACE") ? atoi(getenv("PSFM_FIN_PLACE")) : 1;
+    if (psfm_place_form(1, f, d.n_flows, n, d.cap, place_on)) {
+        if ((st = psfm_place_records(c, d, f, n, s)) != PSFM_OK) return st;
+        return psfm_finalize_sorted(c, d, f, n, npts, true, s, true);
+    }
     const PsfmFinDst dst = psfm_compact_dst(c, f, n);
     hipLaunchKernelGGL(psfm_compact_segments_kernel, dim3((unsigned)nseg), dim3(PSFM_BLOCK), 0, s,
                        c->fin_keys.as<unsigned long long>(), c->fin_lanes.as<int>(), (const int2*)c->seg_info.as<int2>(), d.nblk, d.seg_cap,
diff --git a/particle-sfm_amd/csrc/psfm_internal.h b/particle-sfm_amd/csrc/psfm_internal.h
--- a/particle-sfm_amd/csrc/psfm_internal.h
+++ b/particle-sfm_amd/csrc/psfm_internal.h
@@ -123,6 +123,7 @@
     PsfmBuf seg_info;
     PsfmBuf seg_table;
     PsfmBuf persist_bar;
+    PsfmBuf place_tab;
     int persist_max_blocks = -1;
     int chain_mode = 0;
     bool mb_enable = false;
@@ -134,6 +135,7 @@
     PsfmBuf fin_marks;
     bool fin_marks_clean = false;
     int fin_sort_form = 0, fin_offsets_form = 0;
+    int fin_placed = 0;
     PsfmBuf res_birth, res_len, res_off, res_xy;
     int64_t res_n_traj = 0, res_n_points = 0;
     int res_n_flows = 0;
@@ -286,6 +288,10 @@
 psfm_status psfm_sort_pairs64(psfm_ctx* c, unsigned long long* k_half0, int* v_half0, unsigned long long* k_half1, int* v_half1, int64_t n, unsigned end_bit, hipStream_t s);
 psfm_status psfm_sort_pairs32(psfm_ctx* c, unsigned* k_half0, int* v_half0, unsigned* k_half1, int* v_half1, int64_t n, unsigned end_bit, hipStream_t s);
 psfm_status psfm_finalize_persist(psfm_ctx* c, const PsfmTrackDims& d, bool* fallback, hipStream_t s);
+struct PsfmFinForm;
+size_t psfm_place_table_bytes(const PsfmTrackDims& d);
+psfm_status psfm_place_records(psfm_ctx* c, const PsfmTrackDims& d, const PsfmFinForm& f, int64_t n, hipStream_t s);
+psfm_status psfm_place_sort(psfm_ctx* c, unsigned* k_half0, int* v_half0, const unsigned* k_half1, const int* v_half1, int64_t n, hipStream_t s);
 
 psfm_status psfm_solve_frame_enqueue(psfm_ctx* c, const PsfmTrackDims& d, const float* flow01, const float* flow12,
                                      const float* flow02, const uint8_t* occ02, int frame, int unroll, hipStream_t s);
diff --git a/particle-sfm_amd/csrc/psfm_persist.hip b/particle-sfm_amd/csrc/psfm_persist.hip
--- a/particle-sfm_amd/csrc/psfm_persist.hip
+++ b/particle-sfm_amd/csrc/psfm_persist.hip
@@ -3,8 +3,10 @@
 
 #include "psfm_internal.h"
 #include "psfm_chain.h"
+#include "psfm_place.h"
 
 #define PP_BLOCK 256
+static_assert(PP_BLOCK == PSFM_PLACE_VB, "psfm_place.h takes a virtual block of the loop for 256 grid points");
 #define PP_NW (PP_BLOCK / PSFM_WAVE)
 #define PP_PROBE 8
 #ifndef PP_PRE_WAVES
@@ -38,6 +40,7 @@
 #endif
 #define PP_POOLED (-1)
 #define PP_PEND (-2)
+#define PP_BORN (1 << 30)
 #define PP_DIED (-3)
 
 struct PsfmPersistArgs {
@@ -54,6 +57,7 @@
     int n_flows;
     int nblk;
     PsfmFastDiv gwdiv, rdiv;
+    unsigned long long* bmask; int bm_words;
 };
 #define PP_SURV ((2 * PSFM_NSHARD + 1) * 32)
 
@@ -404,6 +408,7 @@
         const bool pend = bf == PP_PEND;
         if (bf == PP_DIED) bf = PP_PEND;
         const unsigned long long bm = __ballot(birth), am = __ballot(adopted), pm = __ballot(pend);
+        if (birth) npts |= PP_BORN;
         if (lane == 0) { s_births[wave] = __popcll(bm); s_adopt[wave] = __popcll(am); s_pend[wave] = __popcll(pm); }
         if (birth) s_new_g[wave * PSFM_WAVE + psfm_rank_in(bm)] = L;
         if (adopted) s_ad_tid[wave * PSFM_WAVE + psfm_rank_in(am)] = tid;
@@ -625,7 +630,7 @@
         }
         PP_TL(5);
         asm volatile("" : "+s"(t), "+v"(tid));
-        if (npts) s_npts[tid] += npts;
+        if (npts & ~PP_BORN) s_npts[tid] += npts & ~PP_BORN;
         const unsigned long long alm = __ballot(any_alive);
         if (lane == 0 && alm != 0ull) s_alive_any[t & 1] = 1;
         __syncthreads();
@@ -643,9 +648,22 @@
             }
         }
         if (tid == 0 && s_alive_any[t & 1]) { psfm_coh_st(PA->bar + PP_SURV + ((t & 1) * PSFM_NSHARD + PP_SHARD) * 32, (unsigned)(t + 1)); s_alive_any[t & 1] = 0; }
-        if (PA->fc) {
-            const int nf = PA->n_flows, need = t + 3 < nf ? t + 3 : nf;
-            if (!(PP_WHATIF & 16)) for (; fc_next < need; ++fc_next) psfm_fc_slice(fc_next, tid);
+        {
+            const PsfmHotPtr a = psfm_hot();
+            const int fc = a->fc, nf = a->n_flows;
+#ifndef PP_NO_BIRTH_MASKS
+            {
+                const int gw = a->bm_words, per = a->xcd_per, b = PP_BID;
+                unsigned long long* bmask = a->bmask;
+                const unsigned long long born = __ballot((npts & PP_BORN) != 0);
+                const int word = ((per > 0 && b < 8 * per) ? (b & 7) * per + (b >> 3) : b) * (PP_BLOCK / PSFM_WAVE) + (tid / PSFM_WAVE);
+                if ((tid & (PSFM_WAVE - 1)) == 0 && t > 0 && word < gw) bmask[(size_t)t * gw + word] = born;
+            }
+#endif
+            if (fc) {
+                const int need = t + 3 < nf ? t + 3 : nf;
+                if (!(PP_WHATIF & 16)) for (; fc_next < need; ++fc_next) psfm_fc_slice(fc_next, tid);
+            }
         }
         if (!(PP_WHATIF & 2)) asm volatile("s_waitcnt vmcnt(0) lgkmcnt(0)" ::: "memory");
         PP_TL(6);
@@ -773,6 +791,7 @@
     k.fin_keys = c->fin_keys.as<unsigned long long>(); k.fin_lanes = c->fin_lanes.as<int>();
     k.seg_cap = d.seg_cap; k.spill_base = d.nblk * d.seg_cap; k.spill_cap = d.spill_cap;
     k.seg_info = c->seg_info.as<int2>();
+    a.bmask = c->place_tab.as<unsigned long long>(); a.bm_words = psfm_place_words(d.G);
     a.bar = c->persist_bar.as<unsigned>();
     a.n_flows = d.n_flows; a.nblk = d.nblk; k.shift_b = d.shift_b; k.shift_d = d.shift_d;
     a.gwdiv = psfm_fastdiv_make((unsigned)d.GW); a.rdiv = psfm_fastdiv_make((unsigned)d.ratio);
diff --git a/particle-sfm_amd/csrc/psfm_place.h b/particle-sfm_amd/csrc/psfm_place.h
--- /dev/null
+++ b/particle-sfm_amd/csrc/psfm_place.h
@@ -0,0 +1,54 @@
+#pragma once
+#include <hip/hip_runtime.h>
+#include <stdint.h>
+
+#include "psfm_finalize_plan.h"
+
+#define PSFM_PLACE_VB 256
+#define PSFM_PLACE_VB_WORDS 4
+#define PSFM_PLACE_MAX_TIMES 256
+#define PSFM_PLACE_LANE_BITS 24
+
+static inline int psfm_place_form(int persist_ran, const PsfmFinForm& f, int n_flows, int64_t n, int64_t cap, int place_switch)
+{
+    return (place_switch && persist_ran && f.fmt.use32 && f.sort_form == 1 && n_flows + 1 <= PSFM_PLACE_MAX_TIMES && n < (1ll << 31) &&
+            cap <= (1ll << PSFM_PLACE_LANE_BITS)) ? 1 : 0;
+}
+
+PSFM_HD int psfm_place_blocks(int64_t G) { return (int)((G + PSFM_PLACE_VB - 1) / PSFM_PLACE_VB); }
+PSFM_HD int psfm_place_words(int64_t G) { return PSFM_PLACE_VB_WORDS * psfm_place_blocks(G); }
+PSFM_HD int64_t psfm_place_table_words(int n_flows, int64_t G) { return (int64_t)(n_flows + 1) * psfm_place_words(G); }
+PSFM_HD int psfm_place_count(const unsigned long long* bmask, int64_t G, int n_flows, int b, int vb)
+{
+    if (b == 0) { const int64_t r = G - (int64_t)PSFM_PLACE_VB * vb; return r >= PSFM_PLACE_VB ? PSFM_PLACE_VB : (r > 0 ? (int)r : 0); }
+    if (b >= n_flows) return 0;
+    const unsigned long long* w = bmask + (int64_t)b * psfm_place_words(G) + (int64_t)PSFM_PLACE_VB_WORDS * vb;
+    int c = 0;
+    for (int j = 0; j < PSFM_PLACE_VB_WORDS; ++j) c += __builtin_popcountll(w[j]);
+    return c;
+}
+PSFM_HD int psfm_place_ordinal(const unsigned long long* w, int idx)
+{
+    const int q = (idx & (PSFM_PLACE_VB - 1)) >> 6, bit = idx & 63;
+    int k = __builtin_popcountll(w[q] & ((1ull << bit) - 1ull));
+    for (int j = 0; j < PSFM_PLACE_VB_WORDS; ++j) if (j < q) k += __builtin_popcountll(w[j]);
+    return k;
+}
+PSFM_HD int psfm_place_born(const unsigned long long* w, int idx) { return (int)((w[(idx & (PSFM_PLACE_VB - 1)) >> 6] >> (idx & 63)) & 1ull); }
+PSFM_HD int64_t psfm_place_pos(int64_t base, int start, int k) { return base + start + k; }
+PSFM_HD int psfm_place_pack(int lane, int last) { return (int)(((unsigned)last << PSFM_PLACE_LANE_BITS) | (unsigned)lane); }
+PSFM_HD unsigned psfm_place_digit(int packed) { return (unsigned)packed >> PSFM_PLACE_LANE_BITS; }
+PSFM_HD int psfm_place_lane(int packed) { return (int)((unsigned)packed & ((1u << PSFM_PLACE_LANE_BITS) - 1u)); }
+
+static inline void psfm_place_scan_rows(const unsigned long long* bmask, int64_t G, int n_flows, int* start, int* total)
+{
+    const int gb = psfm_place_blocks(G);
+    for (int b = 0; b < n_flows; ++b) {
+        int run = 0;
+        for (int vb = 0; vb < gb; ++vb) {
+            if (b > 0) start[(int64_t)b * gb + vb] = run;
+            run += psfm_place_count(bmask, G, n_flows, b, vb);
+        }
+        total[b] = run;
+    }
+}
diff --git a/particle-sfm_amd/csrc/psfm_place.hip b/particle-sfm_amd/csrc/psfm_place.hip
--- /dev/null
+++ b/particle-sfm_amd/csrc/psfm_place.hip
@@ -0,0 +1,307 @@
+#include <hip/hip_runtime.h>
+#include <stdint.h>
+
+#include "psfm_device.h"
+#include "psfm_internal.h"
+#include "psfm_place.h"
+
+#define PL_BLOCK 256
+#define PL_NW (PL_BLOCK / PSFM_WAVE)
+
+__device__ __forceinline__ int psfm_place_block_scan(int mine, int* s_w, int* sum)
+{
+    const int tid = threadIdx.x, lane = tid & (PSFM_WAVE - 1), wave = tid / PSFM_WAVE;
+    int inc = mine;
+#pragma unroll
+    for (int o = 1; o < PSFM_WAVE; o <<= 1) {
+        const int v = __shfl_up(inc, o);
+        if (lane >= o) inc += v;
+    }
+    if (lane == PSFM_WAVE - 1) s_w[wave] = inc;
+    __syncthreads();
+    int base = 0, tot = 0;
+#pragma unroll
+    for (int w = 0; w < PL_NW; ++w) { const int v = s_w[w]; if (w < wave) base += v; tot += v; }
+    *sum = tot;
+    return base + inc - mine;
+}
+
+__global__ __launch_bounds__(PL_BLOCK) void psfm_place_scan_kernel(const unsigned long long* __restrict__ bmask, int G, int n_flows,
+                                                                   int* __restrict__ start, int* __restrict__ total)
+{
+    __shared__ int s_w[PL_NW];
+    const int b = blockIdx.x, tid = threadIdx.x;
+    if (b == 0) { if (tid == 0) total[0] = G; return; }
+    const int gb = psfm_place_blocks(G);
+    const int per = (gb + PL_BLOCK - 1) / PL_BLOCK;
+    const int v0 = min(tid * per, gb), v1 = min(v0 + per, gb);
+    int mine = 0;
+    for (int v = v0; v < v1; ++v) mine += psfm_place_count(bmask, G, n_flows, b, v);
+    int tot;
+    int run = psfm_place_block_scan(mine, s_w, &tot);
+    int* out = start + (int64_t)b * gb;
+    for (int v = v0; v < v1; ++v) { out[v] = run; run += psfm_place_count(bmask, G, n_flows, b, v); }
+    if (tid == 0) total[b] = tot;
+}
+
+__global__ __launch_bounds__(PL_BLOCK) void psfm_place_records_kernel(
+    const unsigned long long* __restrict__ fin_keys, const int* __restrict__ fin_lanes, const int2* __restrict__ seg_info, int nblk,
+    int seg_cap, const PsfmCounters* __restrict__ ctr, int spill_cap, const unsigned long long* __restrict__ bmask,
+    const int* __restrict__ start, const int* __restrict__ total, int G, int n_flows, PsfmKeyFmt fmt, unsigned* __restrict__ keys,
+    int* __restrict__ vals, int64_t n)
+{
+    __shared__ int s_base[PSFM_PLACE_MAX_TIMES];
+    __shared__ int s_w[PL_NW];
+    const int b = blockIdx.x, tid = threadIdx.x;
+    const int gb = psfm_place_blocks(G), gw = psfm_place_words(G);
+    {
+        int tot;
+        const int mine = tid < n_flows ? total[tid] : 0;
+        s_base[tid] = psfm_place_block_scan(mine, s_w, &tot);
+    }
+    __syncthreads();
+    const int count = b < nblk ? seg_info[b].x : min(ctr->spill_cnt, spill_cap);
+    const long long src = (long long)b * seg_cap;
+    for (int i0 = 0; i0 < count; i0 += 4 * PL_BLOCK) {
+        unsigned long long k[4];
+        int l[4], last[4], bf[4], idx[4], st[4];
+        ulonglong2 m[4][2];
+        bool ok[4];
+#pragma unroll
+        for (int u = 0; u < 4; ++u) {
+            const int i = i0 + u * PL_BLOCK + tid;
+            k[u] = i < count ? fin_keys[src + i] : 0ull;
+            l[u] = i < count ? fin_lanes[src + i] : 0;
+        }
+#pragma unroll
+        for (int u = 0; u < 4; ++u) {
+            const int i = i0 + u * PL_BLOCK + tid;
+            psfm_key64_fields(k[u], fmt.shift_b, fmt.shift_d, &last[u], &bf[u], &idx[u]);
+            ok[u] = i < count && bf[u] < n_flows && last[u] < PSFM_PLACE_MAX_TIMES && idx[u] < G &&
+                    (unsigned)l[u] < (1u << PSFM_PLACE_LANE_BITS);
+            const bool look = ok[u] && bf[u] > 0;
+            const ulonglong2* row = (const ulonglong2*)(bmask + (int64_t)bf[u] * gw + (int64_t)PSFM_PLACE_VB_WORDS * (idx[u] / PSFM_PLACE_VB));
+            m[u][0] = look ? row[0] : make_ulonglong2(0ull, 0ull);
+            m[u][1] = look ? row[1] : make_ulonglong2(0ull, 0ull);
+            st[u] = look ? start[(int64_t)bf[u] * gb + idx[u] / PSFM_PLACE_VB] : 0;
+        }
+#pragma unroll
+        for (int u = 0; u < 4; ++u) {
+            if (!ok[u]) continue;
+            int64_t pos = idx[u];
+            if (bf[u] > 0) {
+                const unsigned long long w[PSFM_PLACE_VB_WORDS] = {m[u][0].x, m[u][0].y, m[u][1].x, m[u][1].y};
+                if (!psfm_place_born(w, idx[u])) continue;
+                pos = psfm_place_pos(s_base[bf[u]], st[u], psfm_place_ordinal(w, idx[u]));
+            }
+            if (pos >= 0 && pos < n) {
+                keys[pos] = psfm_key32(k[u], fmt);
+                vals[pos] = psfm_place_pack(l[u], last[u]);
+            }
+        }
+    }
+}
+
+#define PL_ITEMS 16
+#define PL_TILE (PL_BLOCK * PL_ITEMS)
+#define PL_WSPAN (PL_ITEMS * PSFM_WAVE)
+#define PL_GROUP 8
+#define PL_DIGITS 256
+#define PL_GCHUNK 64
+#define PL_HWAVES 2
+#define PL_HREP 4
+#define PL_HBLOCK (PL_GROUP * PL_HWAVES * PSFM_WAVE)
+#define PL_HITEMS (PL_TILE / (PL_HWAVES * PSFM_WAVE))
+#define PL_PAD (PL_DIGITS - 1)
+
+__device__ __forceinline__ unsigned long long pl_match8(unsigned d)
+{
+    unsigned long long peers = ~0ull;
+#pragma unroll
+    for (int bit = 0; bit < 8; ++bit) {
+        const bool on = (d >> bit) & 1u;
+        const unsigned long long m = __ballot(on);
+        peers &= on ? m : ~m;
+    }
+    return peers;
+}
+
+__global__ __launch_bounds__(PL_HBLOCK) void psfm_place_hist_kernel(const int* __restrict__ vals, int64_t n, unsigned* __restrict__ cnt,
+                                                                    unsigned* __restrict__ grp, int nb)
+{
+    __shared__ unsigned s_h[PL_GROUP][PL_HREP][PL_DIGITS];
+    const int tid = threadIdx.x, lane = tid & (PSFM_WAVE - 1), wave = tid / PSFM_WAVE;
+    for (int q = tid; q < PL_GROUP * PL_HREP * PL_DIGITS; q += PL_HBLOCK) (&s_h[0][0][0])[q] = 0u;
+    const int t = wave / PL_HWAVES, part = wave % PL_HWAVES;
+    const int b = blockIdx.x * PL_GROUP + t;
+    const int64_t tile0 = (int64_t)b * PL_TILE;
+    const int nv = b < nb ? (int)(n - tile0 < PL_TILE ? n - tile0 : PL_TILE) : 0;
+    int k[PL_HITEMS];
+#pragma unroll
+    for (int i = 0; i < PL_HITEMS; ++i) {
+        const int off = (part * PL_HITEMS + i) * PSFM_WAVE + lane;
+        k[i] = off < nv ? vals[tile0 + off] : 0;
+    }
+    __syncthreads();
+#pragma unroll
+    for (int i = 0; i < PL_HITEMS; ++i) {
+        const int off = (part * PL_HITEMS + i) * PSFM_WAVE + lane;
+        const bool ok = off < nv;
+        const unsigned d = psfm_place_digit(k[i]);
+        const unsigned long long valid = __ballot(ok);
+        const unsigned d0 = (unsigned)__builtin_amdgcn_readfirstlane((int)d);
+        if (__ballot(ok && d == d0) == valid) {
+            if (lane == 0 && valid) atomicAdd(&s_h[t][0][d0], (unsigned)__popcll(valid));
+        } else if (ok) {
+            atomicAdd(&s_h[t][lane & (PL_HREP - 1)][d], 1u);
+        }
+    }
+    __syncthreads();
+    if (tid < PL_DIGITS) {
+        unsigned run = 0;
+#pragma unroll
+        for (int q = 0; q < PL_GROUP; ++q) {
+            unsigned c = 0;
+#pragma unroll
+            for (int rep = 0; rep < PL_HREP; ++rep) c += s_h[q][rep][tid];
+            if (blockIdx.x * PL_GROUP + q < nb) cnt[(int64_t)(blockIdx.x * PL_GROUP + q) * PL_DIGITS + tid] = run;
+            run += c;
+        }
+        grp[blockIdx.x * PL_DIGITS + tid] = run;
+    }
+}
+
+__global__ __launch_bounds__(PL_BLOCK) void psfm_place_scatter_kernel(const unsigned* __restrict__ kin, const int* __restrict__ vin,
+                                                                      unsigned* __restrict__ kout, int* __restrict__ vout, int64_t n,
+                                                                      const unsigned* __restrict__ cnt, const unsigned* __restrict__ grp,
+                                                                      int ngrp)
+{
+    __shared__ unsigned s_k[PL_TILE];
+    __shared__ int s_v[PL_TILE];
+    __shared__ unsigned s_wc[PL_NW][PL_DIGITS];
+    __shared__ int s_delta[PL_DIGITS];
+    __shared__ unsigned s_wsum[2][PL_NW];
+    const int tid = threadIdx.x, lane = tid & (PSFM_WAVE - 1), wave = tid / PSFM_WAVE;
+    const int b = blockIdx.x;
+    const int64_t tile0 = (int64_t)b * PL_TILE;
+    const int nv = (int)(n - tile0 < PL_TILE ? n - tile0 : PL_TILE);
+#pragma unroll
+    for (int w = 0; w < PL_NW; ++w) s_wc[w][tid] = 0u;
+    unsigned k[PL_ITEMS];
+    int v[PL_ITEMS];
+#pragma unroll
+    for (int i = 0; i < PL_ITEMS; ++i) {
+        const int off = wave * PL_WSPAN + i * PSFM_WAVE + lane;
+        const bool ok = off < nv;
+        k[i] = ok ? kin[tile0 + off] : 0u;
+        v[i] = ok ? vin[tile0 + off] : psfm_place_pack(0, PL_PAD);
+    }
+    unsigned before = cnt[(int64_t)b * PL_DIGITS + tid], all = 0;
+    {
+        const int g = b / PL_GROUP;
+        for (int q0 = 0; q0 < ngrp; q0 += PL_GCHUNK) {
+            unsigned row[PL_GCHUNK];
+#pragma unroll
+            for (int u = 0; u < PL_GCHUNK; ++u) row[u] = q0 + u < ngrp ? grp[(q0 + u) * PL_DIGITS + tid] : 0u;
+#pragma unroll
+            for (int u = 0; u < PL_GCHUNK; ++u) { all += row[u]; if (q0 + u < g) before += row[u]; }
+        }
+    }
+    __syncthreads();
+    unsigned r[PL_ITEMS];
+    {
+        const unsigned long long lower = (1ull << lane) - 1ull;
+#pragma unroll
+        for (int i = 0; i < PL_ITEMS; ++i) {
+            const unsigned d = psfm_place_digit(v[i]);
+            const unsigned long long peers = pl_match8(d);
+            const unsigned old = s_wc[wave][d];
+            const unsigned long long below = peers & lower;
+            r[i] = old + (unsigned)__popcll(below);
+            if (below == 0ull) s_wc[wave][d] = old + (unsigned)__popcll(peers);
+            __builtin_amdgcn_wave_barrier();
+        }
+    }
+    __syncthreads();
+    {
+        unsigned c[PL_NW], mine = 0;
+#pragma unroll
+        for (int w = 0; w < PL_NW; ++w) { c[w] = s_wc[w][tid]; mine += c[w]; }
+        unsigned inc_t = mine, inc_a = all;
+#pragma unroll
+        for (int o = 1; o < PSFM_WAVE; o <<= 1) {
+            const unsigned a = __shfl_up(inc_t, o), g2 = __shfl_up(inc_a, o);
+            if (lane >= o) { inc_t += a; inc_a += g2; }
+        }
+        if (lane == PSFM_WAVE - 1) { s_wsum[0][wave] = inc_t; s_wsum[1][wave] = inc_a; }
+        __syncthreads();
+        unsigned base_t = 0, base_a = 0;
+#pragma unroll
+        for (int w = 0; w < PL_NW; ++w) if (w < wave) { base_t += s_wsum[0][w]; base_a += s_wsum[1][w]; }
+        const unsigned dstart = base_t + inc_t - mine;
+        const unsigned gstart = base_a + inc_a - all;
+        unsigned run = dstart;
+#pragma unroll
+        for (int w = 0; w < PL_NW; ++w) { s_wc[w][tid] = run; run += c[w]; }
+        s_delta[tid] = (int)(gstart + before) - (int)dstart;
+    }
+    __syncthreads();
+#pragma unroll
+    for (int i = 0; i < PL_ITEMS; ++i) {
+        const unsigned q = s_wc[wave][psfm_place_digit(v[i])] + r[i];
+        s_k[q] = k[i];
+        s_v[q] = v[i];
+    }
+    __syncthreads();
+#pragma unroll
+    for (int j = 0; j < PL_ITEMS; ++j) {
+        const int q = j * PL_BLOCK + tid;
+        if (q < nv) {
+            const int val = s_v[q];
+            const int64_t pos = (int64_t)s_delta[psfm_place_digit(val)] + q;
+            kout[pos] = s_k[q];
+            vout[pos] = psfm_place_lane(val);
+        }
+    }
+}
+
+static int* psfm_place_starts(psfm_ctx* c, const PsfmTrackDims& d) { return (int*)(c->place_tab.as<unsigned long long>() + psfm_place_table_words(d.n_flows, d.G)); }
+
+psfm_status psfm_place_records(psfm_ctx* c, const PsfmTrackDims& d, const PsfmFinForm& f, int64_t n, hipStream_t s)
+{
+    const unsigned long long* bmask = c->place_tab.as<unsigned long long>();
+    int* start = psfm_place_starts(c, d);
+    int* total = start + (int64_t)(d.n_flows + 1) * psfm_place_blocks(d.G);
+    hipLaunchKernelGGL(psfm_place_scan_kernel, dim3((unsigned)d.n_flows), dim3(PL_BLOCK), 0, s, bmask, (int)d.G, d.n_flows, start, total);
+    hipLaunchKernelGGL(psfm_place_records_kernel, dim3((unsigned)(d.nblk + 1)), dim3(PL_BLOCK), 0, s,
+                       (const unsigned long long*)c->fin_keys.as<unsigned long long>(), (const int*)c->fin_lanes.as<int>(),
+                       (const int2*)c->seg_info.as<int2>(), d.nblk, d.seg_cap, (const PsfmCounters*)c->counters.as<PsfmCounters>(), d.spill_cap,
+                       bmask, (const int*)start, (const int*)total, (int)d.G, d.n_flows, f.fmt,
+                       c->sort_keys.as<unsigned>() + n, c->sort_lanes.as<int>() + n, n);
+    PSFM_HIP(hipGetLastError());
+    return PSFM_OK;
+}
+
+size_t psfm_place_table_bytes(const PsfmTrackDims& d)
+{
+    return sizeof(unsigned long long) * (size_t)psfm_place_table_words(d.n_flows, d.G) +
+           sizeof(int) * ((size_t)(d.n_flows + 1) * psfm_place_blocks(d.G) + PSFM_PLACE_MAX_TIMES);
+}
+
+psfm_status psfm_place_sort(psfm_ctx* c, unsigned* k_half0, int* v_half0, const unsigned* k_half1, const int* v_half1, int64_t n, hipStream_t s)
+{
+    if (n <= 0) return PSFM_OK;
+    const int64_t nb = (n + PL_TILE - 1) / PL_TILE;
+    const int64_t ngrp = (nb + PL_GROUP - 1) / PL_GROUP;
+    const size_t cnt_bytes = sizeof(unsigned) * PL_DIGITS * (size_t)nb;
+    const size_t grp_bytes = sizeof(unsigned) * PL_DIGITS * (size_t)ngrp;
+    psfm_status st = c->sort_tmp.ensure(cnt_bytes + grp_bytes);
+    if (st != PSFM_OK) return st;
+    unsigned* cnt = c->sort_tmp.as<unsigned>();
+    unsigned* grp = (unsigned*)((char*)c->sort_tmp.p + cnt_bytes);
+    hipLaunchKernelGGL(psfm_place_hist_kernel, dim3((unsigned)ngrp), dim3(PL_HBLOCK), 0, s, v_half1, n, cnt, grp, (int)nb);
+    hipLaunchKernelGGL(psfm_place_scatter_kernel, dim3((unsigned)nb), dim3(PL_BLOCK), 0, s, k_half1, v_half1, k_half0, v_half0, n,
+                       (const unsigned*)cnt, (const unsigned*)grp, (int)ngrp);
+    PSFM_HIP(hipGetLastError());
+    return PSFM_OK;
+}
diff --git a/particle-sfm_amd/point_trajectory/_hip.py b/particle-sfm_amd/point_trajectory/_hip.py
--- a/particle-sfm_amd/point_trajectory/_hip.py
+++ b/particle-sfm_amd/point_trajectory/_hip.py
@@ -18,7 +18,7 @@
     "psfm_shard_solve_writeback", "psfm_shard_solve_record", "psfm_shard_finish", "psfm_result_keys",
     "psfm_shard_solve_control_async", "psfm_shard_window_state", "psfm_shard_peek_stall", "psfm_shard_frame",
     "psfm_shard_solve_control_chain_async", "psfm_shard_solve_poll", "psfm_shard_solve_local", "psfm_shard_solve_redo_local", "psfm_connect_batch", "psfm_solver_launches", "psfm_ctx_set_resident_budget", "psfm_resident_capacity", "psfm_load_flo_stack",
-    "psfm_path_consistency_eval", "psfm_sort_records", "psfm_sort_records64", "psfm_ctx_get_finalize_forms",
+    "psfm_path_consistency_eval", "psfm_sort_records", "psfm_sort_records64", "psfm_ctx_get_finalize_forms", "psfm_ctx_get_finalize_placed",
     "psfm_shard_peer_area", "psfm_shard_peer_epoch", "psfm_shard_peer_open", "psfm_shard_peer_connect", "psfm_shard_solve_blocks", "psfm_shard_solve_peer",
     "psfm_labels_begin", "psfm_labels_merge_window", "psfm_labels_finish", "psfm_labels_device", "psfm_labels_copy", "psfm_labels_to_matches",
     "psfm_traj_augment", "psfm_traj_encode_weight_count", "psfm_traj_encode",
@@ -87,6 +87,7 @@
     L.psfm_sort_records.argtypes = [vp, vp, vp, i64, i32, vp]
     L.psfm_sort_records64.argtypes = [vp, vp, vp, i64, i32, vp]
     L.psfm_ctx_get_finalize_forms.argtypes = [vp, ctypes.POINTER(ctypes.c_int32), ctypes.POINTER(ctypes.c_int32)]
+    L.psfm_ctx_get_finalize_placed.argtypes = [vp, ctypes.POINTER(ctypes.c_int32)]
     L.psfm_track.argtypes = [vp, vp, vp, vp, vp, i32, i32, i32, i32, ctypes.POINTER(TrackInfo), vp]
     L.psfm_connect.argtypes = [vp, vp, vp, vp, vp, i32, i32, i32, f32, i32, vp, vp, ctypes.POINTER(TrackInfo), vp]
     L.psfm_connect_batch.argtypes = [ctypes.POINTER(vp), i32, ctypes.POINTER(vp), ctypes.POINTER(vp), ctypes.POINTER(vp), ctypes.POINTER(vp),
@@ -227,6 +228,11 @@
         check(lib().psfm_ctx_get_finalize_forms(self._h, ctypes.byref(a), ctypes.byref(b)))
         return {"sort": int(a.value), "offsets": int(b.value)}
 
+    def finalize_placed(self):
+        a = ctypes.c_int32()
+        check(lib().psfm_ctx_get_finalize_placed(self._h, ctypes.byref(a)))
+        return int(a.value)
+
     def set_sparse_depth(self, budget_bytes=1 << 30, timing=False):
         check(lib().psfm_ctx_set_sparse_depth(self._h, int(budget_bytes), int(bool(timing))))
 
```

After: 22.40 billion trajectory-points/s (median of 6 runs). 1.6% higher.
